# pmgbergen/porepy

Hardware: AMD Instinct MI355X
Metric: cells/sec MPFA assemble+solve, 3D unstructured grid (higher is better)
Workload: dtype f64

## Files before the change

include/porefv.h:

```cpp
#ifndef POREFV_H
#define POREFV_H

#include <stddef.h>
#include <stdint.h>

#ifdef __cplusplus
extern "C" {
#endif

typedef struct pfv_ctx pfv_ctx;

typedef enum {
  PFV_OK = 0,
  PFV_ERR_SINGULAR = 1,
  PFV_ERR_CELL_SHAPE = 2,
  PFV_ERR_HIP = 3,
  PFV_ERR_ARGUMENT = 4,
  PFV_ERR_UNSUPPORTED = 5,
  PFV_ERR_NOT_CONVERGED = 6
} pfv_status;

enum {
  PFV_MAT_FLUX = 0,
  PFV_MAT_BOUND_FLUX = 1,
  PFV_MAT_BOUND_PRESSURE_CELL = 2,
  PFV_MAT_BOUND_PRESSURE_FACE = 3,
  PFV_MAT_VECTOR_SOURCE = 4,
  PFV_MAT_BOUND_PRESSURE_VECTOR_SOURCE = 5,
  PFV_MAT_SYSTEM = 6,
  PFV_MAT_STRESS = 7,
  PFV_MAT_BOUND_STRESS = 8,
  PFV_MAT_BOUND_DISPLACEMENT_CELL = 9,
  PFV_MAT_BOUND_DISPLACEMENT_FACE = 10,
  PFV_MAT_MECH_SYSTEM = 11,
  PFV_MAT_USER_SYSTEM = 12,
  PFV_MAT_FLUX_JACOBIAN = 13,
  PFV_MAT_UPWIND = 14,
  PFV_MAT_UPWIND_RHS_DIR = 15,
  PFV_MAT_UPWIND_RHS_NEU = 16,
  PFV_MAT_TRANSPORT_SYSTEM = 17,
  PFV_MAT_ADVDIFF_SYSTEM = 18,
  PFV_NUM_MATS = 19
};

enum { PFV_BC_DIR = 1, PFV_BC_NEU = 2, PFV_BC_ROB = 4, PFV_BC_INTERNAL = 8 };

enum { PFV_SOLVE_CG = 0, PFV_SOLVE_BICGSTAB = 1, PFV_SOLVE_GMRES = 2 };

enum { PFV_PRECOND_JACOBI = 0, PFV_PRECOND_AMG = 1, PFV_PRECOND_BLOCK = 2,
       PFV_PRECOND_AMG_NNS = 3,
       PFV_PRECOND_SWEEP = 4     };

enum {
  PFV_FLUXFN_LINEAR = 0,
  PFV_FLUXFN_COREY = 1,
  PFV_FLUXFN_TABLE = 2
};

enum {
  PFV_DISCR_REBUILD_TOPOLOGY = 1,
  PFV_DISCR_SKIP_VECTOR_SOURCE = 2
};

typedef struct {
  int32_t iterations;
  int32_t converged;
  double rel_residual;
  double solve_ms;
} pfv_solve_info;

typedef struct {
  double topology_ms;
  double symbolic_ms;
  double node_ms;
  double face_ms;
  double assemble_ms;
  double solve_ms;
  double bytes_written_outputs;
  int64_t num_nodes, num_sub_half_faces, sum_block_sq, max_block;
  double amg_setup_ms;
  double amg_operator_complexity;
  int64_t amg_levels, amg_coarsest_rows;
  double discretize_ms;
  int64_t solve_renumbered;
  double node_flops;
  int64_t node_table_doubles;
  int64_t amg_maps_reused;
  int64_t amg_level0_nnz;
  double amg_filter_theta;
  int64_t win_reused;
  int64_t amg_filter_layout;
  int64_t solve_launches;
  int64_t amg_setup_launches;
  int64_t node_redo;
  int64_t symbolic_reused;
  int64_t amg_stale_rematches;
  int64_t mpsa_contrast_regions;
  double mpsa_max_contrast;
  int64_t assemble_positions_kept;
  int64_t pipeline_runs;
  int64_t amg_nns_modes;
  double face_flux_ms;
  double upwind_ms;
  double transport_assemble_ms;
  double transport_advance_ms;
  int64_t transport_iterations;
  int64_t transport_gmres_retries;
  double advdiff_assemble_ms;
  double advdiff_advance_ms;
  int64_t advdiff_iterations;
  int64_t advdiff_precond_fallbacks;
  int64_t advdiff_gmres_retries;
  int64_t sweep_levels;
  int64_t sweep_core_cells;
  int64_t sweep_launches;
  double sweep_order_ms;
  int64_t sweep_direct_steps;
  int64_t sweep_direct_fallbacks;
  int64_t transport_multi_components;
  int64_t transport_multi_direct_steps;
  int64_t transport_multi_fallback_components;
  double transport_nl_ms;
  int64_t transport_nl_steps;
  int64_t transport_nl_core_iterations;
  int64_t transport_nl_components;
  double transport_react_ms;
  int64_t transport_react_steps;
  int64_t transport_react_core_iterations;
  int64_t transport_react_components;
  double transport_adjoint_ms;
  int64_t transport_adjoint_steps;
  int64_t transport_adjoint_core_iterations;
} pfv_stats;

pfv_status pfv_create(int device, pfv_ctx** out);
void pfv_destroy(pfv_ctx* h);
const char* pfv_last_error(pfv_ctx* h);
int pfv_is_device_build(void);

pfv_status pfv_set_grid(pfv_ctx* h, int nd, int64_t nc, int64_t nf, int64_t nn,
                        const double* nodes, const int32_t* cf_indptr,
                        const int32_t* cf_indices, const int8_t* cf_sign,
                        const int32_t* fn_indptr, const int32_t* fn_indices,
                        const double* face_normals, const double* face_centers,
                        const double* cell_centers, const double* face_areas);

pfv_status pfv_mpfa_set_params(pfv_ctx* h, const double* perm_33n, const uint8_t* bc_flags,
                               const double* robin_weight, double eta,
                               const double* eta_subface);

pfv_status pfv_mpfa_set_permeability(pfv_ctx* h, const double* perm_33n);

#define PFV_AD_WANT_FLUX_JACOBIAN 1u
pfv_status pfv_mpfa_ad_flux_system(pfv_ctx* h, const double* p, const double* dk_dp, const double* bc_values,
                                   const double* vector_source, const double* source, double* flux_out,
                                   uint32_t flags);

pfv_status pfv_mpfa_set_subface_bc(pfv_ctx* h, const uint8_t* bc_flags_sub, const double* robin_weight_sub);

pfv_status pfv_mpfa_discretize(pfv_ctx* h, uint32_t flags);

pfv_status pfv_tpfa_discretize(pfv_ctx* h, int vector_source_dim);

pfv_status pfv_tpfa_transmissibility_ad(pfv_ctx* h, const double* perm_33n, double* t_face, double* dt_dk);

pfv_status pfv_mpfa_discretize_faces(pfv_ctx* h, uint32_t flags, int64_t n_faces,
                                     const int32_t* faces, int keep_other_rows);

pfv_status pfv_matrix_info(pfv_ctx* h, int which, int64_t* nrows, int64_t* ncols,
                           int64_t* nnz);
pfv_status pfv_get_matrix(pfv_ctx* h, int which, int32_t* indptr, int32_t* indices,
                          double* data);
pfv_status pfv_device_memory(pfv_ctx* h, int64_t* free_bytes, int64_t* total_bytes);
pfv_status pfv_host_alloc(size_t bytes, void** out);
void pfv_host_free(void* p);
pfv_status pfv_active_size(pfv_ctx* h, int64_t* n);
pfv_status pfv_get_matrix_rows(pfv_ctx* h, int which, int64_t n_rows, const int32_t* rows, int32_t* out_indptr,
                               int32_t* out_indices, double* out_data);

pfv_status pfv_mpfa_assemble(pfv_ctx* h, const double* bc_values, const double* vector_source,
                             const double* source);
pfv_status pfv_get_rhs(pfv_ctx* h, double* b);

pfv_status pfv_spmv(pfv_ctx* h, int which, const double* x, double* y);

enum {
  PFV_BIOT_SCALAR_GRADIENT = 0,
  PFV_BIOT_DISPLACEMENT_DIVERGENCE = 1,
  PFV_BIOT_BOUNDARY_DISPLACEMENT_DIVERGENCE = 2,
  PFV_BIOT_CONSISTENCY = 3,
  PFV_BIOT_BOUND_DISPLACEMENT_PRESSURE = 4,
  PFV_BIOT_NUM_TERMS = 5
};
pfv_status pfv_biot_set_alphas(pfv_ctx* h, int nalpha, const double* alpha_k33n);
pfv_status pfv_biot_discretize_faces(pfv_ctx* h, uint32_t flags, int64_t n_faces, const int32_t* faces,
                                     int64_t n_cells, const int32_t* cells, int keep_other_rows);

pfv_status pfv_biot_discretize(pfv_ctx* h, uint32_t flags);
pfv_status pfv_biot_matrix_info(pfv_ctx* h, int term, int64_t* nrows, int64_t* ncols, int64_t* nnz);
pfv_status pfv_biot_get_matrix(pfv_ctx* h, int term, int key, int32_t* indptr, int32_t* indices,
                               double* data);

pfv_status pfv_set_system(pfv_ctx* h, int64_t n, const int32_t* indptr, const int32_t* indices,
                          const double* data, const double* rhs);

pfv_status pfv_set_periodic(pfv_ctx* h, const int32_t* native_cell, const double* shift);

pfv_status pfv_set_vectors_on_device(pfv_ctx* h, int on);

pfv_status pfv_set_preconditioner(pfv_ctx* h, int kind);

pfv_status pfv_sweep_info(pfv_ctx* h, int64_t info[4], int32_t* level, int32_t* order);

pfv_status pfv_set_near_null_space(pfv_ctx* h, int bs, int k, const double* B);

pfv_status pfv_amg_nns_level(pfv_ctx* h, int level, int64_t* info, int32_t* agg, double* P, double* B, double* Bc,
                             int32_t* indptr, int32_t* indices, double* val);

pfv_status pfv_amg_level(pfv_ctx* h, int level, int64_t* info, double* params, int32_t* sys_indptr, int32_t* sys_indices,
                         double* sys_val, int32_t* a_indptr, int32_t* a_indices, double* a_val, int32_t* op_indptr,
                         int32_t* op_indices, double* op_val, double* dinv, int32_t* agg, int32_t* mptr, int32_t* mem,
                         double* dense);

pfv_status pfv_set_block_preconditioner(pfv_ctx* h, int64_t n_blocks, const int64_t* block_ptr, int gauss_seidel);

pfv_status pfv_solve(pfv_ctx* h, int method, double rtol, int maxit, int restart,
                     const double* x0, double* x, pfv_solve_info* info);

pfv_status pfv_mpsa_set_params(pfv_ctx* h, const double* stiffness_99n, const double* cell_volumes,
                               const uint8_t* bc_dir_bits, const uint8_t* bc_neu_bits, double eta);
pfv_status pfv_mpsa_set_subface_eta(pfv_ctx* h, const double* eta_subface);
pfv_status pfv_mpsa_set_reconstruction_eta(pfv_ctx* h, int on, double hf_eta);
pfv_status pfv_mpsa_set_reconstruction_eta_subface(pfv_ctx* h, const double* hf_eta_subface);
pfv_status pfv_mpsa_set_robin(pfv_ctx* h, const uint8_t* bc_rob_bits, const double* robin_weight_ddn);
pfv_status pfv_mpsa_set_basis(pfv_ctx* h, const double* basis_ddn);

pfv_status pfv_mpsa_set_subface_bc(pfv_ctx* h, const uint8_t* bc_dir_bits_sub, const uint8_t* bc_neu_bits_sub,
                                   const uint8_t* bc_rob_bits_sub, const double* robin_weight_dds);
pfv_status pfv_mpsa_set_subface_basis(pfv_ctx* h, const double* basis_dds);

pfv_status pfv_mpsa_discretize(pfv_ctx* h, uint32_t flags);

pfv_status pfv_mpsa_discretize_faces(pfv_ctx* h, uint32_t flags, int64_t n_faces,
                                     const int32_t* faces, int keep_other_rows);
pfv_status pfv_mpsa_assemble(pfv_ctx* h, const double* bc_values, const double* source);

pfv_status pfv_mpfa_face_flux(pfv_ctx* h, const double* p, const double* bc_values, const double* vector_source,
                              double* q_out);
pfv_status pfv_upwind_set_bc(pfv_ctx* h, const uint8_t* bc_flags);
pfv_status pfv_upwind_discretize(pfv_ctx* h, const double* q, int num_components);
pfv_status pfv_upwind_assemble(pfv_ctx* h, const double* q, const double* bc_values, const double* accumulation,
                               const double* c_old, const double* source, double* bound_rhs_out);
pfv_status pfv_transport_advance(pfv_ctx* h, int n_steps, int method, double rtol, int maxit, double* c,
                                 int32_t* steps_done, pfv_solve_info* last);
pfv_status pfv_transport_advance_multi(pfv_ctx* h, const double* q, int n_comp, const double* bc_values,
                                       const double* accumulation, const double* source, int n_steps, int method,
                                       double rtol, int maxit, double* c, int32_t* steps_done, pfv_solve_info* last);
pfv_status pfv_transport_advance_nl(pfv_ctx* h, const double* q, int fluxfn_kind, const double* fluxfn_params,
                                    int n_params, const double* bc_values, const double* accumulation,
                                    const double* source, const double* sink, int n_steps, double rtol, int maxit,
                                    double* s, int32_t* steps_done, pfv_solve_info* last);
pfv_status pfv_transport_advance_nl_multi(pfv_ctx* h, const double* q, int fluxfn_kind, const double* fluxfn_params,
                                          int n_params, const double* bc_values, const double* accumulation,
                                          const double* source, const double* sink, int k, const double* c_bc_values,
                                          const double* sorption, const double* c_source, int n_steps, double rtol,
                                          int maxit, double* s, double* c, int32_t* steps_done, pfv_solve_info* last);

pfv_status pfv_transport_advance_react(pfv_ctx* h, const double* q, int k, const double* bc_values,
                                       const double* accumulation, const double* source, const double* mobility,
                                       const double* rate, const double* rate_weight, int n_steps, double rtol,
                                       int maxit, double* c, int32_t* steps_done, pfv_solve_info* last);

pfv_status pfv_transport_adjoint_multi(pfv_ctx* h, const double* q, int n_comp, const double* bc_values,
                                       const double* accumulation, int n_steps, int64_t n_obs, const int32_t* obs_cells,
                                       const double* loads, const double* states, double rtol, int maxit,
                                       double* grad_c0, double* grad_source, double* grad_bc_values,
                                       double* grad_accumulation, double* grad_flux, int32_t* steps_done,
                                       pfv_solve_info* last);

pfv_status pfv_advdiff_assemble(pfv_ctx* h, const double* q, double flux_scale, const double* bc_values,
                                const double* accumulation, const double* c_old, const double* source,
                                double* bound_rhs_out);
pfv_status pfv_advdiff_advance(pfv_ctx* h, int n_steps, int method, double rtol, int maxit, double* c,
                               int32_t* steps_done, pfv_solve_info* last);
pfv_status pfv_advdiff_face_flux(pfv_ctx* h, const double* c, double* out);
// ... 74 lines not shown
```

porepy_amd/_lib.py:

```python
from __future__ import annotations

import ctypes as C
import os

import numpy as np

_HERE = os.path.dirname(os.path.abspath(__file__))
DEFAULT_LIBRARY = os.path.join(_HERE, "csrc", "libporefv_hip.so")

MAT_FLUX, MAT_BOUND_FLUX, MAT_BOUND_PRESSURE_CELL, MAT_BOUND_PRESSURE_FACE = 0, 1, 2, 3
MAT_VECTOR_SOURCE, MAT_BOUND_PRESSURE_VECTOR_SOURCE, MAT_SYSTEM = 4, 5, 6
MAT_STRESS, MAT_BOUND_STRESS, MAT_BOUND_DISPLACEMENT_CELL, MAT_BOUND_DISPLACEMENT_FACE, MAT_MECH_SYSTEM = 7, 8, 9, 10, 11
MAT_USER_SYSTEM = 12
MAT_FLUX_JACOBIAN = 13
MAT_UPWIND, MAT_UPWIND_RHS_DIR, MAT_UPWIND_RHS_NEU, MAT_TRANSPORT_SYSTEM = 14, 15, 16, 17
MAT_ADVDIFF_SYSTEM = 18
BC_DIR, BC_NEU, BC_ROB, BC_INTERNAL = 1, 2, 4, 8
SOLVE_CG, SOLVE_BICGSTAB, SOLVE_GMRES = 0, 1, 2
PRECOND_JACOBI, PRECOND_AMG, PRECOND_BLOCK, PRECOND_AMG_NNS, PRECOND_SWEEP = 0, 1, 2, 3, 4
FLUXFN_LINEAR, FLUXFN_COREY, FLUXFN_TABLE = 0, 1, 2
DISCR_REBUILD_TOPOLOGY, DISCR_SKIP_VECTOR_SOURCE = 1, 2

STATUS_NAMES = {
    0: "ok", 1: "singular local system", 2: "unsupported cell shape", 3: "HIP error",
    4: "bad argument", 5: "unsupported size/feature", 6: "not converged",
}

EXPORTS = [
    "pfv_create", "pfv_destroy", "pfv_last_error", "pfv_is_device_build", "pfv_set_grid",
    "pfv_mpfa_set_params", "pfv_mpfa_discretize", "pfv_matrix_info", "pfv_get_matrix",
    "pfv_mpfa_assemble", "pfv_get_rhs", "pfv_spmv", "pfv_solve", "pfv_spmv_device",
    "pfv_get_device_rhs", "pfv_sync", "pfv_get_stats", "pfv_time_kernel", "pfv_debug_copy",
    "pfv_spmv_device_rows", "pfv_copy_device_vector", "pfv_set_stream",
    "pfv_mpsa_set_params", "pfv_mpsa_discretize", "pfv_mpsa_assemble",
    "pfv_mpfa_discretize_faces", "pfv_set_system", "pfv_tpfa_discretize", "pfv_mpsa_discretize_faces", "pfv_set_preconditioner", "pfv_amg_setup", "pfv_amg_setup_sharded", "pfv_amg_apply_device", "pfv_csr_from_host", "pfv_csr_from_matrix", "pfv_csr_block_diag", "pfv_csr_matmul", "pfv_csr_axpby", "pfv_csr_transpose", "pfv_csr_bmat", "pfv_csr_scale", "pfv_csr_divide", "pfv_csr_spmv", "pfv_csr_spmv_device", "pfv_csr_info", "pfv_csr_get", "pfv_csr_set_system", "pfv_csr_free", "pfv_reset_stream", "pfv_mpsa_set_robin", "pfv_mpsa_set_basis", "pfv_mpfa_set_subface_bc", "pfv_mpsa_set_subface_bc", "pfv_mpsa_set_subface_basis",
    "pfv_biot_set_alphas", "pfv_biot_discretize", "pfv_biot_matrix_info", "pfv_biot_get_matrix",
    "pfv_set_vectors_on_device", "pfv_set_periodic", "pfv_biot_discretize_faces", "pfv_solve_sharded", "pfv_tpfa_transmissibility_ad",
    "pfv_get_matrix_rows", "pfv_active_size", "pfv_device_memory",
    "pfv_rccl_unique_id", "pfv_rccl_comm_create", "pfv_rccl_set_halo_plan", "pfv_rccl_hooks", "pfv_rccl_stats",
    "pfv_rccl_last_error", "pfv_rccl_comm_destroy", "pfv_mpfa_ad_flux_system", "pfv_host_alloc", "pfv_host_free",
    "pfv_mpsa_set_subface_eta", "pfv_mpsa_set_reconstruction_eta", "pfv_mpsa_set_reconstruction_eta_subface", "pfv_get_stats_n", "pfv_set_block_preconditioner",
    "pfv_mpfa_set_permeability", "pfv_set_near_null_space", "pfv_amg_nns_level", "pfv_amg_level",
    "pfv_mpfa_face_flux", "pfv_upwind_set_bc", "pfv_upwind_discretize", "pfv_upwind_assemble", "pfv_transport_advance",
    "pfv_advdiff_assemble", "pfv_advdiff_advance", "pfv_advdiff_face_flux", "pfv_resident_flux",
    "pfv_sweep_info", "pfv_transport_advance_multi", "pfv_transport_advance_nl", "pfv_transport_advance_nl_multi",
    "pfv_transport_advance_react", "pfv_transport_adjoint_multi",
]


class SolveInfo(C.Structure):
    _fields_ = [("iterations", C.c_int32), ("converged", C.c_int32),
                ("rel_residual", C.c_double), ("solve_ms", C.c_double)]


class Stats(C.Structure):
    _fields_ = [("topology_ms", C.c_double), ("symbolic_ms", C.c_double), ("node_ms", C.c_double),
                ("face_ms", C.c_double), ("assemble_ms", C.c_double), ("solve_ms", C.c_double),
                ("bytes_written_outputs", C.c_double), ("num_nodes", C.c_int64),
                ("num_sub_half_faces", C.c_int64), ("sum_block_sq", C.c_int64),
                ("max_block", C.c_int64), ("amg_setup_ms", C.c_double),
                ("amg_operator_complexity", C.c_double), ("amg_levels", C.c_int64),
                ("amg_coarsest_rows", C.c_int64), ("discretize_ms", C.c_double), ("solve_renumbered", C.c_int64),
                ("node_flops", C.c_double), ("node_table_doubles", C.c_int64),
                ("amg_maps_reused", C.c_int64), ("amg_level0_nnz", C.c_int64), ("amg_filter_theta", C.c_double),
                ("win_reused", C.c_int64), ("amg_filter_layout", C.c_int64),
                ("solve_launches", C.c_int64), ("amg_setup_launches", C.c_int64), ("node_redo", C.c_int64),
                ("symbolic_reused", C.c_int64), ("amg_stale_rematches", C.c_int64),
                ("mpsa_contrast_regions", C.c_int64), ("mpsa_max_contrast", C.c_double), ("assemble_positions_kept", C.c_int64),
                ("pipeline_runs", C.c_int64), ("amg_nns_modes", C.c_int64),
                ("face_flux_ms", C.c_double), ("upwind_ms", C.c_double), ("transport_assemble_ms", C.c_double),
                ("transport_advance_ms", C.c_double), ("transport_iterations", C.c_int64),
                ("transport_gmres_retries", C.c_int64),
                ("advdiff_assemble_ms", C.c_double), ("advdiff_advance_ms", C.c_double),
                ("advdiff_iterations", C.c_int64), ("advdiff_precond_fallbacks", C.c_int64),
                ("advdiff_gmres_retries", C.c_int64),
                ("sweep_levels", C.c_int64), ("sweep_core_cells", C.c_int64), ("sweep_launches", C.c_int64),
                ("sweep_order_ms", C.c_double), ("sweep_direct_steps", C.c_int64),
                ("sweep_direct_fallbacks", C.c_int64),
                ("transport_multi_components", C.c_int64), ("transport_multi_direct_steps", C.c_int64),
                ("transport_multi_fallback_components", C.c_int64),
                ("transport_nl_ms", C.c_double), ("transport_nl_steps", C.c_int64),
                ("transport_nl_core_iterations", C.c_int64), ("transport_nl_components", C.c_int64),
                ("transport_react_ms", C.c_double), ("transport_react_steps", C.c_int64),
                ("transport_react_core_iterations", C.c_int64), ("transport_react_components", C.c_int64),
                ("transport_adjoint_ms", C.c_double), ("transport_adjoint_steps", C.c_int64),
                ("transport_adjoint_core_iterations", C.c_int64)]

    def as_dict(self):
        return {n: getattr(self, n) for n, _ in self._fields_}


HALO_FN = C.CFUNCTYPE(C.c_int, C.c_void_p, C.c_void_p, C.c_void_p)
ALLREDUCE_FN = C.CFUNCTYPE(C.c_int, C.c_void_p, C.c_void_p, C.c_int, C.c_void_p)


SENDRECV_FN = C.CFUNCTYPE(C.c_int, C.c_void_p, C.c_int, C.POINTER(C.c_int32), C.c_void_p, C.POINTER(C.c_int64),
                          C.c_void_p, C.POINTER(C.c_int64), C.c_void_p)
ALLGATHER_FN = C.CFUNCTYPE(C.c_int, C.c_void_p, C.c_void_p, C.c_void_p, C.c_int64, C.c_void_p)


class ShardHooks(C.Structure):
    _fields_ = [("exchange_halo", HALO_FN), ("allreduce_sum", ALLREDUCE_FN), ("user", C.c_void_p),
                ("sendrecv", SENDRECV_FN), ("allgather", ALLGATHER_FN)]


class PorefvError(RuntimeError):
    def __init__(self, status: int, message: str):
        super().__init__(f"porefv status {status} ({STATUS_NAMES.get(status, '?')}): {message}")
        self.status = status
        self.message = message


_dp = C.POINTER(C.c_double)
_ip = C.POINTER(C.c_int32)
_bp = C.POINTER(C.c_int8)
_up = C.POINTER(C.c_uint8)
_lp = C.POINTER(C.c_int64)
_h = C.c_void_p


def _bind(lib: C.CDLL) -> C.CDLL:
    lib.pfv_create.argtypes = [C.c_int, C.POINTER(_h)]
    lib.pfv_create.restype = C.c_int
    lib.pfv_destroy.argtypes = [_h]
    lib.pfv_destroy.restype = None
    lib.pfv_last_error.argtypes = [_h]
    lib.pfv_last_error.restype = C.c_char_p
    lib.pfv_is_device_build.argtypes = []
    lib.pfv_is_device_build.restype = C.c_int
    lib.pfv_set_grid.argtypes = [_h, C.c_int, C.c_int64, C.c_int64, C.c_int64, _dp, _ip, _ip, _bp,
                                 _ip, _ip, _dp, _dp, _dp, _dp]
    lib.pfv_set_grid.restype = C.c_int
    lib.pfv_mpfa_set_params.argtypes = [_h, _dp, _up, _dp, C.c_double, _dp]
    lib.pfv_mpfa_set_params.restype = C.c_int
    lib.pfv_mpfa_set_permeability.argtypes = [_h, _dp]
    lib.pfv_mpfa_set_permeability.restype = C.c_int
    lib.pfv_mpfa_discretize.argtypes = [_h, C.c_uint32]
    lib.pfv_mpfa_discretize.restype = C.c_int
    lib.pfv_mpfa_discretize_faces.argtypes = [_h, C.c_uint32, C.c_int64, _ip, C.c_int]
    lib.pfv_mpfa_discretize_faces.restype = C.c_int
    lib.pfv_mpsa_discretize_faces.argtypes = [_h, C.c_uint32, C.c_int64, _ip, C.c_int]
    lib.pfv_mpsa_discretize_faces.restype = C.c_int
    lib.pfv_biot_set_alphas.argtypes = [_h, C.c_int, _dp]
    lib.pfv_biot_set_alphas.restype = C.c_int
    lib.pfv_biot_discretize.argtypes = [_h, C.c_uint32]
    lib.pfv_biot_discretize.restype = C.c_int
    lib.pfv_biot_matrix_info.argtypes = [_h, C.c_int, _lp, _lp, _lp]
    lib.pfv_biot_matrix_info.restype = C.c_int
    lib.pfv_biot_get_matrix.argtypes = [_h, C.c_int, C.c_int, _ip, _ip, _dp]
    lib.pfv_biot_get_matrix.restype = C.c_int
    lib.pfv_mpfa_set_subface_bc.argtypes = [_h, _up, _dp]
    lib.pfv_mpfa_set_subface_bc.restype = C.c_int
    lib.pfv_mpsa_set_basis.argtypes = [_h, _dp]
    lib.pfv_mpsa_set_basis.restype = C.c_int
    lib.pfv_mpsa_set_subface_bc.argtypes = [_h, _up, _up, _up, _dp]
    lib.pfv_mpsa_set_subface_bc.restype = C.c_int
    lib.pfv_mpsa_set_subface_basis.argtypes = [_h, _dp]
    lib.pfv_mpsa_set_subface_basis.restype = C.c_int
    lib.pfv_mpsa_set_robin.argtypes = [_h, _up, _dp]
    lib.pfv_mpsa_set_robin.restype = C.c_int
    lib.pfv_mpsa_set_subface_eta.argtypes = [_h, _dp]
    lib.pfv_mpsa_set_subface_eta.restype = C.c_int
    lib.pfv_mpsa_set_reconstruction_eta.argtypes = [_h, C.c_int, C.c_double]
    lib.pfv_mpsa_set_reconstruction_eta.restype = C.c_int
    lib.pfv_mpsa_set_reconstruction_eta_subface.argtypes = [_h, _dp]
    lib.pfv_mpsa_set_reconstruction_eta_subface.restype = C.c_int
    lib.pfv_reset_stream.argtypes = [_h]
    lib.pfv_reset_stream.restype = C.c_int
    lib.pfv_amg_setup.argtypes = [_h, C.c_int64]
    lib.pfv_amg_setup.restype = C.c_int
    lib.pfv_amg_setup_sharded.argtypes = [_h, C.c_int64, C.POINTER(ShardHooks), C.c_int, C.c_int, C.c_int, _ip, _lp, _ip,
                                          _lp, _ip]
    lib.pfv_amg_setup_sharded.restype = C.c_int
    lib.pfv_csr_from_host.argtypes = [_h, C.c_int64, C.c_int64, _ip, _ip, _dp, C.POINTER(_h)]
    lib.pfv_csr_from_matrix.argtypes = [_h, _h, C.c_int, C.POINTER(_h)]
    lib.pfv_csr_block_diag.argtypes = [_h, C.c_int, C.POINTER(_h), C.POINTER(_h)]
    lib.pfv_csr_matmul.argtypes = [_h, _h, _h, C.POINTER(_h)]
    lib.pfv_csr_axpby.argtypes = [_h, C.c_double, _h, C.c_double, _h, C.POINTER(_h)]
    lib.pfv_csr_transpose.argtypes = [_h, _h, C.POINTER(_h)]
    lib.pfv_csr_bmat.argtypes = [_h, C.c_int, C.c_int, C.POINTER(_h), _lp, _lp, C.POINTER(_h)]
    lib.pfv_csr_scale.argtypes = [_h, _dp, _dp]
    lib.pfv_csr_divide.argtypes = [_h, C.c_double]
    lib.pfv_csr_divide.restype = C.c_int
    lib.pfv_csr_spmv.argtypes = [_h, _dp, _dp]
    lib.pfv_csr_spmv_device.argtypes = [_h, C.c_void_p, C.c_void_p]
    lib.pfv_csr_info.argtypes = [_h, _lp, _lp, _lp]
    lib.pfv_csr_get.argtypes = [_h, _ip, _ip, _dp]
    lib.pfv_csr_set_system.argtypes = [_h, _h, C.c_void_p, C.c_int]
    for name in ("from_host", "from_matrix", "block_diag", "matmul", "axpby", "transpose", "bmat", "scale", "spmv", "spmv_device", "info", "get",
                 "set_system"):
        getattr(lib, "pfv_csr_" + name).restype = C.c_int
    lib.pfv_csr_free.argtypes = [_h]
    lib.pfv_csr_free.restype = None
    lib.pfv_amg_apply_device.argtypes = [_h, C.c_void_p, C.c_void_p]
    lib.pfv_amg_apply_device.restype = C.c_int
    lib.pfv_biot_discretize_faces.argtypes = [_h, C.c_uint32, C.c_int64, _ip, C.c_int64, _ip, C.c_int]
    lib.pfv_biot_discretize_faces.restype = C.c_int
    lib.pfv_set_periodic.argtypes = [_h, C.POINTER(C.c_int32), _dp]
    lib.pfv_set_periodic.restype = C.c_int
    lib.pfv_set_vectors_on_device.argtypes = [_h, C.c_int]
    lib.pfv_set_vectors_on_device.restype = C.c_int
    lib.pfv_set_preconditioner.argtypes = [_h, C.c_int]
    lib.pfv_set_preconditioner.restype = C.c_int
    lib.pfv_tpfa_discretize.argtypes = [_h, C.c_int]
    lib.pfv_tpfa_discretize.restype = C.c_int
    lib.pfv_set_system.argtypes = [_h, C.c_int64, _ip, _ip, _dp, _dp]
    lib.pfv_set_system.restype = C.c_int
    lib.pfv_matrix_info.argtypes = [_h, C.c_int, _lp, _lp, _lp]
    lib.pfv_matrix_info.restype = C.c_int
    lib.pfv_get_matrix.argtypes = [_h, C.c_int, _ip, _ip, _dp]
    lib.pfv_get_matrix.restype = C.c_int
    lib.pfv_mpfa_assemble.argtypes = [_h, _dp, _dp, _dp]
    lib.pfv_mpfa_assemble.restype = C.c_int
    lib.pfv_get_rhs.argtypes = [_h, _dp]
    lib.pfv_get_rhs.restype = C.c_int
    lib.pfv_spmv.argtypes = [_h, C.c_int, _dp, _dp]
    lib.pfv_spmv.restype = C.c_int
    lib.pfv_solve.argtypes = [_h, C.c_int, C.c_double, C.c_int, C.c_int, _dp, _dp, C.POINTER(SolveInfo)]
    lib.pfv_solve.restype = C.c_int
    lib.pfv_spmv_device.argtypes = [_h, C.c_int, C.c_void_p, C.c_void_p]
    lib.pfv_spmv_device.restype = C.c_int
    lib.pfv_get_device_rhs.argtypes = [_h, C.POINTER(C.c_void_p), C.POINTER(C.c_void_p)]
    lib.pfv_get_device_rhs.restype = C.c_int
    lib.pfv_sync.argtypes = [_h]
    lib.pfv_sync.restype = C.c_int
    lib.pfv_get_stats.argtypes = [_h, C.POINTER(Stats)]
    lib.pfv_get_stats.restype = C.c_int
    lib.pfv_set_block_preconditioner.argtypes = [_h, C.c_int64, C.POINTER(C.c_int64), C.c_int]
    lib.pfv_set_block_preconditioner.restype = C.c_int
    lib.pfv_set_near_null_space.argtypes = [_h, C.c_int, C.c_int, _dp]
    lib.pfv_set_near_null_space.restype = C.c_int
    lib.pfv_amg_nns_level.argtypes = [_h, C.c_int, _lp, _ip, _dp, _dp, _dp, _ip, _ip, _dp]
    lib.pfv_amg_nns_level.restype = C.c_int
    lib.pfv_amg_level.argtypes = [_h, C.c_int, _lp, _dp, _ip, _ip, _dp, _ip, _ip, _dp, _ip, _ip, _dp, _dp, _ip, _ip, _ip,
                                  _dp]
    lib.pfv_amg_level.restype = C.c_int
    lib.pfv_get_stats_n.argtypes = [_h, C.c_void_p, C.c_size_t]
    lib.pfv_get_stats_n.restype = C.c_int
    lib.pfv_time_kernel.argtypes = [_h, C.c_int, C.c_int, _dp]
# ... 1343 lines not shown
```

porepy_amd/csrc/amg.inc:

```

namespace pfv {

constexpr int kAmgDenseMax = 1024;
constexpr int kAmgCoarseTargetDefault = 160;
constexpr int kAmgMaxLevels = 14;
constexpr int64_t kAmgWTopRows = 600000;
constexpr int kAmgFilterPermilBlock = 50;
constexpr int kAmgFilterPermil = 30;
constexpr int kAmgRounds = 4;
constexpr int kAmgPasses = 3;
constexpr int kAmgGentleCells = 400000;
constexpr int kGalEpl = 8;
constexpr int kGalMaxMembers = 16;
constexpr int64_t kAmgGatherRowsDefault = 32768;

struct AmgSwitches {
  int bs = 1;
  bool omega_auto = false;
  bool safe_rows = true;
  double omega = 0.95, alpha = 1.5;
  int omega_power_steps = 10;
  double omega_sigma = 1.8;
  int passes = kAmgPasses;
  bool passes_coarse_set = false;
  int passes_coarse_raw = -1;
  int rounds = kAmgRounds, rounds_raw = kAmgRounds;
  int strength_neg = 0;
  bool fp32 = true;
  double filter_theta = 0.0;
  int coarse_target = kAmgCoarseTargetDefault;
  bool gamma_set = false;
  int gamma_raw = 0;
  int gamma_levels = 1;
  int64_t fuse_rows = 30000;
  bool fuse_cycle = true;
  bool restrict_lanes = true;
  bool reuse = true, reuse_dist = true, reuse_rebuilt = true;
  int reuse_dist_min_rows = 500000;
  bool members_reuse = true, sizes_reuse = true;
  bool filter_smooth = true, rowmax_reuse = true, filter_layout_reuse = true, skip_moved_digest = true;
  bool galerkin_batched = true, filter_unroll = true, dense_lds = true;
  int64_t gather_rows = kAmgGatherRowsDefault;
};

static AmgSwitches amg_read_switches(int bs) {
  auto given = [](const char* name, int& v) {
    const char* e = std::getenv(name);
    if (e) v = std::atoi(e);
    return e != nullptr;
  };
  auto on = [](const char* name, int dflt) { return env_int(name, dflt) != 0; };
  AmgSwitches w;
  w.bs = bs;
  w.safe_rows = on("PFV_AMG_SAFE_ROWS", bs == 1 ? 1 : 0);
  int omega_pct = w.safe_rows ? 95 : 80;
  w.omega_auto = !given("PFV_AMG_OMEGA_PCT", omega_pct) && on("PFV_AMG_OMEGA_AUTO", 0);
  w.omega = 0.01 * omega_pct;
  w.alpha = 0.01 * env_int("PFV_AMG_ALPHA_PCT", 150);
  w.omega_power_steps = std::max(2, std::min(30, env_int("PFV_AMG_OMEGA_POWER_STEPS", 10)));
  w.omega_sigma = 0.01 * env_int("PFV_AMG_OMEGA_RHO_PCT", 180);
  w.passes = std::max(1, std::min(6, env_int("PFV_AMG_PASSES", kAmgPasses)));
  w.passes_coarse_set = given("PFV_AMG_PASSES_COARSE", w.passes_coarse_raw);
  w.rounds_raw = env_int("PFV_AMG_ROUNDS", kAmgRounds);
  w.rounds = std::max(1, std::min(12, w.rounds_raw));
  w.strength_neg = env_int("PFV_AMG_STRENGTH_NEG", 0);
  w.fp32 = on("PFV_AMG_FP32", 1);
  w.filter_theta = 0.001 * env_int(bs == 1 ? "PFV_AMG_FILTER_PERMIL" : "PFV_AMG_FILTER_PERMIL_BLOCK",
                                   bs == 1 ? kAmgFilterPermil : kAmgFilterPermilBlock);
  w.coarse_target = std::max(1, std::min(kAmgDenseMax, env_int("PFV_AMG_COARSE_TARGET", kAmgCoarseTargetDefault)));
  w.gamma_set = given("PFV_AMG_GAMMA", w.gamma_raw);
  w.gamma_levels = env_int("PFV_AMG_GAMMA_LEVELS", 1);
  w.fuse_rows = env_int("PFV_AMG_FUSE_ROWS", 30000);
  w.fuse_cycle = on("PFV_AMG_FUSE_CYCLE", 1);
  w.restrict_lanes = on("PFV_AMG_RESTRICT_LANES", bs == 1 ? 1 : 0);
  w.reuse = on("PFV_AMG_REUSE", 1);
  w.reuse_dist = on("PFV_AMG_REUSE_DIST", 1);
  w.reuse_rebuilt = on("PFV_AMG_REUSE_REBUILT", 1);
  w.reuse_dist_min_rows = env_int("PFV_AMG_REUSE_DIST_MIN_ROWS", 500000);
  w.members_reuse = on("PFV_AMG_MEMBERS_REUSE", 1);
  w.sizes_reuse = on("PFV_AMG_SIZES_REUSE", 1);
  w.filter_smooth = on("PFV_AMG_FILTER_SMOOTH", 1);
  w.rowmax_reuse = on("PFV_AMG_ROWMAX_REUSE", 1);
  w.filter_layout_reuse = on("PFV_AMG_FILTER_LAYOUT_REUSE", 1);
  w.skip_moved_digest = on("PFV_AMG_SKIP_MOVED_DIGEST", 1);
  w.galerkin_batched = on("PFV_AMG_GALERKIN_BATCHED", 1);
  w.filter_unroll = on("PFV_AMG_FILTER_UNROLL", 1);
  w.dense_lds = on("PFV_AMG_DENSE_LDS", 1);
  w.gather_rows = std::max<int64_t>(1, env_int("PFV_AMG_GATHER_ROWS", (int)kAmgGatherRowsDefault));
  return w;
}

static int64_t amg_maps_cfg(const AmgSwitches& w) {
  return ((((int64_t)w.passes * 16 + w.rounds_raw) * 16 + w.passes_coarse_raw + 1) * 4 + w.strength_neg) * 65536 +
         w.coarse_target * 8 + w.bs + (int64_t)(1000.0 * w.filter_theta + 0.5) * (int64_t(1) << 40);
}
static int amg_maps_tag(const AmgSwitches& w) { return w.rounds_raw * 64 + w.passes_coarse_raw + 1; }

struct AmgLevel {
  int64_t n = 0;
  int64_t m = 0;
  const CsrPattern* P = nullptr;
  const double* val = nullptr;
  CsrPattern P_own;
  Buf<double> val_own;
  Buf<float> val32;
  const float* v32 = nullptr;
  WinCsr win_own;
  const WinCsr* win = nullptr;
  Buf<double> dinv;
  Buf<int32_t> agg;
  Buf<int32_t> mptr, mem;
  int64_t nc_cells = 0;
  Buf<int32_t> pmap[6];
  int64_t pmap_n[6] = {0, 0, 0, 0, 0, 0};
  int pmap_count = 0;
  Buf<int32_t> pmp[6], pme[6];
  bool members_kept = false;
  Buf<double> x, b, t;
  Buf<double> r2, x2;
  Buf<double> u;
  double omega = 0.8;
  double rho = 0.0;
};

struct AmgWork {
  Buf<int32_t> match, pick, join, lead, a1, mp, me, cap, cnt, tcol, vin;
  Buf<uint32_t> kin, kout;
  Buf<int64_t> pos, tptr, cptr;
  Buf<double> tval, dense_work;
  Buf<int32_t> piv;
  Buf<unsigned long long> csum;
  CsrPattern P[2];
  Buf<double> V[2], D[2];
};

struct AmgPlan {
  int n_peers = 0;
  std::vector<int32_t> peers;
  std::vector<int64_t> send_ptr, recv_ptr;
  std::vector<int32_t> h_send_idx, h_recv_pos;
  Buf<int32_t> send_idx, recv_pos;
  int64_t n_send = 0, n_recv = 0;
  int64_t n_own = 0, n_halo = 0;
  std::vector<int32_t> halo_peer, halo_owner_id;
};
struct Amg;
struct AmgDist {
  ~AmgDist() {
    rows0.indptr.p = nullptr;
    rows0.indices.p = nullptr;
  }
  CsrPattern rows0;
  pfv_shard_hooks hooks{};
  int rank = 0, world = 1;
  std::vector<std::unique_ptr<AmgPlan>> plan;
  size_t kgather = 0;
  Buf<double> sbuf, rbuf, gid;
  Buf<int32_t> aext, itmp, chalo;
  std::unique_ptr<Amg> glob;
  std::vector<int64_t> gn, goff;
  int64_t gN = 0, gnmax = 0;
  Buf<int64_t> gn_d, goff_d, cnt_s, cnt_r;
  Buf<double> gsend, grecv, gb, gx, gV, gval_s, gval_r;
  Buf<int32_t> glen_s, glen_r, gcol_s, gcol_r, hal_gcell;
  CsrPattern gT, gP;
  Buf<double> gTV, gD;
  Buf<int32_t> gagg, gmp, gme;
  int64_t exchanges = 0, allgathers = 0;
  int64_t global_rows0 = 0, global_rows_level = 0;
};

struct Amg {
  Amg();
  ~Amg();
  std::unique_ptr<AmgDist> dist;
  bool no_filter = false;
  int64_t finest_cells_parent = 0;
  std::vector<std::unique_ptr<AmgLevel>> lev;
  size_t nlev = 0;
  AmgWork wk;
  int bs = 1;
  AmgSwitches sw;
  int passes = kAmgPasses;
  double omega = 0.8, alpha = 1.5;
  bool omega_auto = true;
  Buf<double> pw_a, pw_b, pw_zero, pw_part;
  Buf<double> dense;
  unsigned long long filt_layout_for = 0;
  bool filt_layout_stable = false;
  CsrPattern filtP;
  Buf<double> filtV;
  double filter_theta = 0.0;
  int64_t filt_nnz = 0;
  bool filter_level0 = false;
  WinCsr filt_win;
  struct GalSizes { int64_t ncr, annz, nnz; int maxcap; };
  std::vector<GalSizes> gal_sizes;
  unsigned long long gal_for_sum = 0;
  bool gal_use = false;
  size_t gal_k = 0;
  unsigned long long filt_win_sum = 0;
  bool maps_ok = false, reused = false;
  int64_t maps_n = -1, maps_nnz = -1, maps_cfg = 0;
  unsigned long long maps_sum = 0, maps_epoch = 0;
  int maps_tag = 0;
  int iters_fresh = -1;
  int method_fresh = -1;
  double rtol_fresh = 0.0;
  int64_t stale_rematches = 0;
  void note_iterations(int iterations, double rtol, int method, bool converged) {
    if (!valid) return;
    if (!reused) {
      iters_fresh = converged ? iterations : -1;
      rtol_fresh = rtol;
      method_fresh = method;
    } else if (iters_fresh > 0 && rtol == rtol_fresh && method == method_fresh &&
               (!converged || (double)iterations > 1.3 * (double)iters_fresh + 1.0)) {
      maps_ok = false;
      ++stale_rematches;
    }
  }
  bool dense_ok = false;
  bool restrict_lanes = true;
  bool valid = false;
  int gamma = 2, gamma_levels = 1;
  int coarse_target = 0;
  int64_t fuse_rows = 0;
  bool fuse_cycle = true;
  bool fp32 = true;
  double setup_ms = 0.0, op_complexity = 0.0;
  const CsrPattern* sysP = nullptr;
  const double* sysV = nullptr;
};

struct AmgPath {
  bool small = false;
  bool twice = false;
  bool fuse_up = false;
  bool fuse_big = false;
  bool second = false;
};
static AmgPath amg_level_path(const Amg& amg, size_t l) {
  AmgPath p;
  if (l + 1 >= amg.nlev) return p;
  const AmgLevel& L = *amg.lev[l];
  p.small = L.n <= amg.fuse_rows && !(L.win && L.win->ok);
  p.twice = amg.gamma == 2 && l >= 1 && (int)l <= amg.gamma_levels;
  p.fuse_up = p.small && l >= 1 && !p.twice;
  p.fuse_big = amg.fuse_cycle && !p.small && l >= 1;
  p.second = amg.gamma == 2 && (int)l < amg.gamma_levels && l + 2 < amg.nlev;
  return p;
}

inline Amg::Amg() = default;
inline Amg::~Amg() = default;
static bool amg_gal_cached(Amg* amg, int64_t ncr, int64_t annz, int* maxcap, int64_t* nnz) {
  if (!amg || !amg->gal_use || amg->gal_k >= amg->gal_sizes.size()) return false;
  const Amg::GalSizes& g = amg->gal_sizes[amg->gal_k];
  if (g.ncr != ncr || g.annz != annz) {
    amg->gal_use = false;
    amg->gal_sizes.resize(amg->gal_k);
    return false;
  }
  *maxcap = g.maxcap;
  *nnz = g.nnz;
  ++amg->gal_k;
  return true;
}
static void amg_gal_record(Amg* amg, int64_t ncr, int64_t annz, int maxcap, int64_t nnz) {
  if (!amg) return;
  if (amg->gal_k < amg->gal_sizes.size()) amg->gal_sizes.resize(amg->gal_k);
  amg->gal_sizes.push_back(Amg::GalSizes{ncr, annz, nnz, maxcap});
  amg->gal_k = amg->gal_sizes.size();
}

struct AmgGraph {
  const int32_t* ip;
  const int32_t* ix;
  const double* val;
  int bs;
  int neg_only;
  PFV_HD int nblk(int64_t i) const { return (ip[i * bs + 1] - ip[i * bs]) / bs; }
  PFV_HD int col(int64_t i, int k) const { return ix[ip[i * bs] + k * bs] / bs; }
  PFV_HD double w(int64_t i, int k) const {
    double s = 0.0;
    for (int a = 0; a < bs; ++a) {
      const double v = val[ip[i * bs + a] + k * bs + a];
      s += neg_only ? (v < 0.0 ? -v : 0.0) : fabs(v);
    }
    return s;
  }
};

PFV_HD inline uint32_t amg_edge_hash(int64_t i, int64_t j) {
  uint64_t a = (uint64_t)(i < j ? i : j), b = (uint64_t)(i < j ? j : i);
  uint64_t z = a * 0x9E3779B97F4A7C15ull + b + 0x7F4A7C15ull;
  z = (z ^ (z >> 30)) * 0xBF58476D1CE4E5B9ull;
  z = (z ^ (z >> 27)) * 0x94D049BB133111EBull;
  return (uint32_t)(z >> 32);
}

static void amg_pick_pass(pfv_ctx_impl& c, const AmgGraph g, int64_t nb, const int32_t* match, int want_matched,
                          int32_t* out) {
  stream_t s = c.stream;
  const size_t lds_pick = 16 * (8 + 4 + 4) + 16;
  wave_for<16>(s, nb, lds_pick, PFV_LAMBDA(const WaveCtx& w) {
    const int64_t i = w.item;
    if (match[i] >= 0) {
      if (w.lane0()) out[i] = -1;
      return;
    }
    double* cw = reinterpret_cast<double*>(w.lds);
    uint32_t* ch = reinterpret_cast<uint32_t*>(cw + 16);
    int32_t* cj = reinterpret_cast<int32_t*>(ch + 16);
    double bw = 0.0;
    uint32_t bh = 0;
    int best = -1;
    const int m = g.nblk(i);
    PFV_LANES(k, m) {
      const int j = g.col(i, k);
      const bool eligible = (j != i) && j < nb && ((match[j] >= 0) == (want_matched != 0));
      if (eligible) {
        const double wt = g.w(i, k);
        if (wt > 0.0 && !(wt < bw)) {
          const uint32_t h = amg_edge_hash(i, j);
          if (wt > bw || h > bh) { bw = wt; bh = h; best = j; }
        }
      }
    }
    cw[w.lane] = bw;
    ch[w.lane] = bh;
    cj[w.lane] = best;
    w.sync();
    if (w.lane0()) {
      for (int l = 1; l < w.width; ++l) {
        if (cj[l] >= 0 && (cw[l] > bw || (cw[l] == bw && ch[l] > bh))) { bw = cw[l]; bh = ch[l]; best = cj[l]; }
      }
      out[i] = best;
    }
    w.sync();
  });
}

static int64_t amg_pairwise(pfv_ctx_impl& c, const AmgSwitches& sw, AmgWork& wk, const CsrPattern& P, const double* val,
                            int bs, Buf<int32_t>& agg_out) {
  stream_t s = c.stream;
  const int64_t nb = P.nrows / bs;
  AmgGraph g{P.indptr, P.indices, val, bs, sw.strength_neg};
  int32_t* match = wk.match.ensure(nb);
  int32_t* pick = wk.pick.ensure(nb);
  int32_t* join = wk.join.ensure(nb);
  int32_t* lead = wk.lead.ensure(nb + 1);
  int64_t* pos = wk.pos.ensure(nb + 1);
  parallel_for(s, nb, PFV_LAMBDA(int64_t i) { match[i] = -1; });
  for (int round = 0; round < sw.rounds; ++round) {
    amg_pick_pass(c, g, nb, match, 0, pick);
    parallel_for(s, nb, PFV_LAMBDA(int64_t i) {
      const int p = pick[i];
      if (p >= 0 && pick[p] == (int32_t)i) match[i] = p;
    });
  }
  amg_pick_pass(c, g, nb, match, 1, join);
  parallel_for(s, nb, PFV_LAMBDA(int64_t i) {
    lead[i] = (match[i] >= 0) ? ((int32_t)i < match[i] ? 1 : 0) : (join[i] < 0 ? 1 : 0);
  });
  exclusive_scan<int32_t, int64_t>(s, c.scratch, lead, pos, (size_t)nb);
  const int64_t nagg = read_scalar<int64_t>(s, pos + nb);
  int32_t* agg = agg_out.ensure(nb);
  parallel_for(s, nb, PFV_LAMBDA(int64_t i) {
    int l;
    if (match[i] >= 0) l = (int32_t)i < match[i] ? (int32_t)i : match[i];
    else if (join[i] >= 0) l = join[i] < match[join[i]] ? join[i] : match[join[i]];
    else l = (int32_t)i;
    agg[i] = (int32_t)pos[l];
  });
  return nagg;
}

static void amg_members(pfv_ctx_impl& c, AmgWork& wk, const int32_t* agg, int64_t nb, int64_t nagg,
                        Buf<int32_t>& mptr_, Buf<int32_t>& mem_) {
  stream_t s = c.stream;
  uint32_t* k = wk.kin.ensure(nb);
  uint32_t* ko = wk.kout.ensure(nb);
  int32_t* v = wk.vin.ensure(nb);
  int32_t* mem = mem_.ensure(nb);
  int32_t* mptr = mptr_.ensure(nagg + 1);
  parallel_for(s, nb, PFV_LAMBDA(int64_t i) {
    k[i] = (uint32_t)agg[i];
    v[i] = (int32_t)i;
  });
  int bits = 1;
  while ((int64_t(1) << bits) < nagg) ++bits;
  sort_pairs(s, c.scratch, k, ko, v, mem, (size_t)nb, bits);
  parallel_for(s, nagg + 1, PFV_LAMBDA(int64_t I) {
    mptr[I] = (int32_t)lower_bound_idx<uint32_t>(ko, (int)nb, (uint32_t)I);
  });
}

struct Amg;
static bool amg_gal_cached(Amg* amg, int64_t ncr, int64_t annz, int* maxcap, int64_t* nnz);
static void amg_gal_record(Amg* amg, int64_t ncr, int64_t annz, int maxcap, int64_t nnz);
static void amg_galerkin(pfv_ctx_impl& c, const AmgSwitches& sw, AmgWork& wk, const CsrPattern& A, const double* val,
                         int bs, const int32_t* agg, const int32_t* mptr, const int32_t* mem, int64_t nagg, CsrPattern& Ac,
                         Buf<double>& valc, Buf<double>& dinvc, Amg* sizes = nullptr) {
  stream_t s = c.stream;
  const int64_t ncr = nagg * bs;
  const int32_t* ip = A.indptr;
  const int32_t* ix = A.indices;
  int32_t* cap = wk.cap.ensure(ncr + 1);
  int32_t* cnt = wk.cnt.ensure(ncr + 1);
  int64_t* tptr = wk.tptr.ensure(ncr + 1);
  int64_t* cptr = wk.cptr.ensure(ncr + 1);
  int32_t* st = c.status.ensure(16);
  be_memset(st + 8, 0, sizeof(int32_t) * 2, s);
  parallel_for(s, ncr, PFV_LAMBDA(int64_t R) {
    const int64_t I = R / bs;
    const int a = (int)(R - I * bs);
    int m = 0;
    for (int q = mptr[I]; q < mptr[I + 1]; ++q) {
      const int64_t r = (int64_t)mem[q] * bs + a;
      m += ip[r + 1] - ip[r];
    }
    cap[R] = m;
    track_max_i32(st + 8, m);
  });
  exclusive_scan<int32_t, int64_t>(s, c.scratch, cap, tptr, (size_t)ncr);
  int maxcap_c = 0;
  int64_t nnz_c = 0;
  const bool known = amg_gal_cached(sizes, ncr, A.nnz, &maxcap_c, &nnz_c);
  const int maxcap = known ? maxcap_c : read_scalar<int32_t>(s, st + 8);
  const int64_t ttot = A.nnz;
  if (maxcap > 4096) throw Error(PFV_ERR_UNSUPPORTED, "AMG: more than 4096 entries feed one coarse row");
  int32_t* tcol = wk.tcol.ensure(std::max<int64_t>(ttot, 1));
  double* tval = wk.tval.ensure(std::max<int64_t>(ttot, 1));
  double* dinv = dinvc.ensure(std::max<int64_t>(ncr, 1));
  be_memset(dinv, 0, sizeof(double) * (size_t)ncr, s);
  const int capL = std::max(maxcap, 1);
  const int G = capL <= 64 ? 16 : (capL <= 160 ? 32 : 64);
  int capP = 2;
  while (capP < capL) capP <<= 1;
  const int nw = capP / 64 + 1;
  const size_t lds = 8 * (size_t)capP + 8 * (size_t)capL + 8 * (size_t)nw + 4 * (2 * kGalMaxMembers + 1) + 64;
  const bool batched = capL <= kGalEpl * G && sw.galerkin_batched;
  wave_for_g(G, s, ncr, lds, PFV_LAMBDA(const WaveCtx& w) {
    const int64_t R = w.item;
    const int64_t I = R / bs;
    const int a = (int)(R - I * bs);
    unsigned long long* key = reinterpret_cast<unsigned long long*>(w.lds);
    double* v0 = reinterpret_cast<double*>(key + capP);
    unsigned long long* mask = reinterpret_cast<unsigned long long*>(v0 + capL);
    int m = 0;
    const int q0 = mptr[I], nm = mptr[I + 1] - q0;
    if (batched && nm <= kGalMaxMembers && cap[R] <= kGalEpl * w.width) {
      int32_t* mp0 = reinterpret_cast<int32_t*>(mask + nw);
      int32_t* mof = mp0 + kGalMaxMembers;
      PFV_LANES(q, nm) {
        const int64_t r = (int64_t)mem[q0 + q] * bs + a;
        mp0[q] = ip[r];
        mof[q + 1] = ip[r + 1] - ip[r];
      }
      w.sync();
      if (w.lane0()) {
        mof[0] = 0;
        for (int q = 0; q < nm; ++q) mof[q + 1] += mof[q];
      }
      w.sync();
      m = mof[nm];
      int cidx[kGalEpl];
      double vv[kGalEpl];
#pragma unroll
      for (int k = 0; k < kGalEpl; ++k) {
        const int e = w.lane + k * w.width;
        cidx[k] = -1;
        vv[k] = 0.0;
        if (e < m) {
          int q = 0;
          while (q + 1 < nm && e >= mof[q + 1]) ++q;
          const int src = mp0[q] + (e - mof[q]);
          cidx[k] = ix[src];
          vv[k] = val[src];
        }
      }
      int kcs[kGalEpl];
#pragma unroll
      for (int k = 0; k < kGalEpl; ++k) {
        kcs[k] = 0;
        if (cidx[k] >= 0) {
          const int cj = cidx[k] / bs;
          kcs[k] = agg[cj] * bs + (cidx[k] - cj * bs);
        }
      }
#pragma unroll
      for (int k = 0; k < kGalEpl; ++k) {
        const int e = w.lane + k * w.width;
        if (cidx[k] >= 0) {
          key[e] = ((unsigned long long)(unsigned)kcs[k] << 32) | (unsigned)e;
          v0[e] = vv[k];
        }
      }
    } else {
      for (int q = q0; q < q0 + nm; ++q) {
        const int64_t r = (int64_t)mem[q] * bs + a;
        const int p0 = ip[r], len = ip[r + 1] - p0;
        PFV_LANES(t, len) {
          const int cidx = ix[p0 + t];
          const int cj = cidx / bs;
          const unsigned long long kc = (unsigned long long)(unsigned)(agg[cj] * bs + (cidx - cj * bs));
          key[m + t] = (kc << 32) | (unsigned)(m + t);
          v0[m + t] = val[p0 + t];
        }
        m += len;
      }
    }
    int P2 = 2;
    while (P2 < m) P2 <<= 1;
    PFV_LANES(t, P2 - m) key[m + t] = ~0ull;
    PFV_LANES(i, P2 / 64 + 1) mask[i] = 0ull;
    w.sync();
    for (int k = 2; k <= P2; k <<= 1) {
      for (int j = k >> 1; j > 0; j >>= 1) {
        PFV_LANES(t, P2 >> 1) {
          const int lo = ((t & ~(j - 1)) << 1) | (t & (j - 1));
          const int hi = lo | j;
          const bool up = (lo & k) == 0;
          const unsigned long long x = key[lo], y = key[hi];
          if ((x > y) == up) {
            key[lo] = y;
            key[hi] = x;
          }
        }
        w.sync();
      }
    }
    PFV_LANES(e, m) {
      if (e == 0 || (key[e] >> 32) != (key[e - 1] >> 32)) atomic_or_u64(mask + (e >> 6), 1ull << (e & 63));
    }
    w.sync();
    int total = 0;
    for (int i = 0; i < m / 64 + 1; ++i) total += popcount64(mask[i]);
    const int64_t t0 = tptr[R];
    PFV_LANES(e, m) {
      const unsigned long long word = mask[e >> 6];
      if ((word >> (e & 63)) & 1ull) {
        int posn = popcount64(word & ((1ull << (e & 63)) - 1ull));
        for (int i = 0; i < (e >> 6); ++i) posn += popcount64(mask[i]);
        const unsigned long long kc = key[e] >> 32;
        double sum = v0[(unsigned)key[e]];
        for (int t = e + 1; t < m && (key[t] >> 32) == kc; ++t) sum += v0[(unsigned)key[t]];
        tcol[t0 + posn] = (int32_t)kc;
        tval[t0 + posn] = sum;
        if ((int64_t)kc == R) dinv[R] = sum != 0.0 ? 1.0 / sum : 0.0;
      }
    }
    if (w.lane0()) cnt[R] = total;
    w.sync();
  });
  exclusive_scan<int32_t, int64_t>(s, c.scratch, cnt, cptr, (size_t)ncr);
  const int64_t nnz = known ? nnz_c : read_scalar<int64_t>(s, cptr + ncr);
  if (!known) amg_gal_record(sizes, ncr, A.nnz, maxcap, nnz);
  if (nnz >= (int64_t(1) << 31)) throw Error(PFV_ERR_UNSUPPORTED, "AMG: coarse matrix with more than 2^31 entries");
  Ac.nrows = Ac.ncols = ncr;
  Ac.nnz = nnz;
  int32_t* cp = Ac.indptr.ensure(ncr + 1);
  int32_t* cx = Ac.indices.ensure(std::max<int64_t>(nnz, 1));
  double* cv = valc.ensure(std::max<int64_t>(nnz, 1));
  parallel_for(s, ncr + 1, PFV_LAMBDA(int64_t R) { cp[R] = (int32_t)cptr[R]; });
  wave_for<16>(s, ncr, 16, PFV_LAMBDA(const WaveCtx& w) {
    const int64_t R = w.item;
    const int64_t t0 = tptr[R], o = cptr[R];
    PFV_LANES(t, cnt[R]) {
      cx[o + t] = tcol[t0 + t];
      cv[o + t] = tval[t0 + t];
    }
  });
  Ac.max_row = maxcap;
}

static void amg_diag_inverse(pfv_ctx_impl& c, const CsrPattern& P, const double* val, double* dinv) {
  const int32_t* ip = P.indptr;
  const int32_t* ix = P.indices;
  parallel_for(c.stream, P.nrows, PFV_LAMBDA(int64_t r) {
    double d = 0.0;
    for (int e = ip[r]; e < ip[r + 1]; ++e)
      if (ix[e] == r) d += val[e];
    dinv[r] = d != 0.0 ? 1.0 / d : 0.0;
  });
}

static void amg_swap_pattern(CsrPattern& a, CsrPattern& b) {
  std::swap(a.nrows, b.nrows);
  std::swap(a.ncols, b.ncols);
  std::swap(a.nnz, b.nnz);
  std::swap(a.max_row, b.max_row);
  a.indptr.swap(b.indptr);
  a.indices.swap(b.indices);
}

static unsigned long long amg_pattern_checksum(pfv_ctx_impl& c, AmgWork& wk, const CsrPattern& P) {
  if (&P == &c.pat_A && c.pat_A_checksum != 0 && c.have_symbolic) return c.pat_A_checksum;
  return read_scalar<unsigned long long>(c.stream, launch_pattern_checksum(c, wk.csum, P));
}

struct AmgBlockStrength {
  const int32_t* ip;
  const double* val;
  int bs;
  PFV_HD double operator()(int64_t r, int kb) const {
    const int64_t i = r / bs;
    double sw = 0.0;
    for (int a = 0; a < bs; ++a) sw += fabs(val[ip[i * bs + a] + kb * bs + a]);
    return sw;
  }
};

#ifndef PFV_EMULATE
constexpr int kFilterUnroll = 5;

static void amg_filter_count_scalar(stream_t s, int64_t n, const int32_t* ip, const int32_t* ix, const double* val,
                                    const double* rmax, double theta, int32_t* cnt) {
  wave_for<16>(s, n, 16, PFV_LAMBDA(const WaveCtx& w) {
    const int64_t r = w.item;
    const int p0 = ip[r], nb = ip[r + 1] - p0;
    const double mi = rmax[r];
    int kept = 0;
    for (int c0 = 0; c0 < nb; c0 += kFilterUnroll * 16) {
      int cj[kFilterUnroll];
      double v[kFilterUnroll], rm[kFilterUnroll];
#pragma unroll
      for (int u = 0; u < kFilterUnroll; ++u) {
        const int kb = c0 + u * 16 + w.lane;
        const bool live = kb < nb;
        cj[u] = live ? ix[p0 + kb] : -1;
        v[u] = live ? val[p0 + kb] : 0.0;
      }
#pragma unroll
      for (int u = 0; u < kFilterUnroll; ++u) rm[u] = cj[u] >= 0 ? rmax[cj[u]] : 0.0;
#pragma unroll
      for (int u = 0; u < kFilterUnroll; ++u)
        if (cj[u] >= 0 && (cj[u] == (int32_t)r || fabs(v[u]) >= theta * fmin(mi, rm[u]))) ++kept;
    }
    kept += __shfl_xor(kept, 8, 16);
    kept += __shfl_xor(kept, 4, 16);
    kept += __shfl_xor(kept, 2, 16);
    kept += __shfl_xor(kept, 1, 16);
    if (w.lane0()) cnt[r] = kept;
  });
}

static void amg_filter_compact_scalar(stream_t s, int64_t n, const int32_t* ip, const int32_t* ix, const double* val,
                                      const double* rmax, double theta, const int32_t* fp, int32_t* fx, double* fv,
                                      double* dinv_out, bool spec, int32_t* bad) {
  wave_for<16>(s, n, 16 * sizeof(double) + 16, PFV_LAMBDA(const WaveCtx& w) {
    const int64_t r = w.item;
    double* lump = reinterpret_cast<double*>(w.lds);
    const int p0 = ip[r], nb = ip[r + 1] - p0;
    const double mi = rmax[r];
    double mylump = 0.0;
    int base = fp[r];
    const int room = fp[r + 1];
    int od = -1;
    double dv = 0.0;
    const int sh = (int)threadIdx.x & 48;
    for (int c0 = 0; c0 < nb; c0 += kFilterUnroll * 16) {
      int cj[kFilterUnroll];
      double v[kFilterUnroll], rm[kFilterUnroll];
#pragma unroll
      for (int u = 0; u < kFilterUnroll; ++u) {
        const int kb = c0 + u * 16 + w.lane;
        const bool live = kb < nb;
        cj[u] = live ? ix[p0 + kb] : -1;
        v[u] = live ? val[p0 + kb] : 0.0;
      }
#pragma unroll
      for (int u = 0; u < kFilterUnroll; ++u) rm[u] = cj[u] >= 0 ? rmax[cj[u]] : 0.0;
#pragma unroll
      for (int u = 0; u < kFilterUnroll; ++u) {
        if (c0 + u * 16 >= nb) break;
        const bool live = cj[u] >= 0;
        const bool isdiag = cj[u] == (int32_t)r;
        bool keep = live && (isdiag || fabs(v[u]) >= theta * fmin(mi, rm[u]));
        if (live && !keep) mylump += v[u];
        const unsigned long long m = __ballot(keep);
        const unsigned m16 = (unsigned)((m >> sh) & 0xffffu);
        const int before = __popc(m16 & ((1u << w.lane) - 1u));
        const int total = __popc(m16);
        if (keep && spec && base + before + 1 > room) {
          atomic_max_i32(bad, 1);
          keep = false;
        }
        if (keep) {
          const int o = base + before;
          fx[o] = cj[u];
          fv[o] = v[u];
          if (isdiag) { od = o; dv = v[u]; }
        }
        base += total;
      }
    }
    lump[w.lane] = mylump;
    w.lsync();
    if (spec && w.lane0() && base != room) atomic_max_i32(bad, 1);
    const unsigned long long has = __ballot(od >= 0);
    const bool any_diag = ((has >> sh) & 0xffffull) != 0ull;
    if (od >= 0) {
      double sum = 0.0;
      for (int l = 0; l < 16; ++l) sum += lump[l];
      const double d = dv + sum;
      fv[od] = d;
      if (dinv_out) dinv_out[r] = d != 0.0 ? 1.0 / d : 0.0;
    } else if (!any_diag && w.lane0() && dinv_out) {
      dinv_out[r] = 0.0;
    }
    w.lsync();
  });
}
#endif

static void amg_filter(pfv_ctx_impl& c, const AmgSwitches& sw, const CsrPattern& A, const double* val, double theta,
                       CsrPattern& F, Buf<double>& FV, AmgWork& wk, int bs = 1,
// ... 41 lines not shown
#endif
  if (!spec) {
#ifndef PFV_EMULATE
  if (fast) amg_filter_count_scalar(s, n, ip, ix, val, rmax, theta, cnt);
  else
#endif
  wave_for<16>(s, n, 16 * sizeof(int32_t) + 16, PFV_LAMBDA(const WaveCtx& w) {
    const int64_t r = w.item;
    const int64_t i = r / bs;
    int32_t* ct = reinterpret_cast<int32_t*>(w.lds);
    const int p0 = ip[r], nb = (ip[r + 1] - p0) / bs;
    const double mi = rmax[r];
    int kept = 0;
    PFV_LANES(kb, nb) {
      const int cj = ix[p0 + kb * bs] / bs;
      if (cj == (int32_t)i || strength(r, kb) >= theta * fmin(mi, rmax[(int64_t)cj * bs])) ++kept;
    }
#ifndef PFV_EMULATE
    (void)ct;
    kept += __shfl_xor(kept, 8, 16);
    kept += __shfl_xor(kept, 4, 16);
    kept += __shfl_xor(kept, 2, 16);
    kept += __shfl_xor(kept, 1, 16);
    if (w.lane0()) cnt[r] = kept * bs;
#else
    ct[w.lane] = kept;
    w.lsync();
    if (w.lane0()) {
      int tot = 0;
      for (int l = 0; l < w.width; ++l) tot += ct[l];
      cnt[r] = tot * bs;
    }
    w.lsync();
#endif
  });
  exclusive_scan<int32_t, int64_t>(s, c.scratch, cnt, pos, (size_t)n);
  }
  const bool compare = !spec && layout_unchanged != nullptr && F.nrows == n && F.nnz > 0 && F.indptr.p != nullptr;
  if (!spec) {
    be_memset(pos + n + 1, 0, sizeof(int64_t), s);
    if (compare) {
      const int32_t* old = F.indptr.p;
      parallel_for(s, n, PFV_LAMBDA(int64_t r) {
        if (old[r + 1] - old[r] != cnt[r]) pos[n + 1] = 1;
      });
    }
  }
  int64_t tail[2] = {F.nnz, 0};
  if (!spec) be_d2h(tail, pos + n, 2 * sizeof(int64_t), s);
  if (layout_unchanged) *layout_unchanged = spec || (compare && tail[1] == 0 && tail[0] == F.nnz);
  const int64_t nnz = tail[0];
  F.nrows = n;
  F.ncols = A.ncols;
  F.nnz = nnz;
  F.max_row = A.max_row;
  int32_t* fp = F.indptr.ensure(n + 1);
  int32_t* fx = F.indices.ensure(std::max<int64_t>(nnz, 1));
  double* fv = FV.ensure(std::max<int64_t>(nnz, 1));
  if (!spec) parallel_for(s, n + 1, PFV_LAMBDA(int64_t q) { fp[q] = (int32_t)pos[q]; });
#ifndef PFV_EMULATE
  if (fast) amg_filter_compact_scalar(s, n, ip, ix, val, rmax, theta, fp, fx, fv, dinv_out, spec, bad);
  else
#endif
  wave_for<16>(s, n, (16 + 1) * kMaxBs * sizeof(double) + 20 * sizeof(int32_t) + 16, PFV_LAMBDA(const WaveCtx& w) {
    const int64_t r = w.item;
    const int64_t i = r / bs;
    double* lump = reinterpret_cast<double*>(w.lds);
    double* dblk = lump + 16 * kMaxBs;
    int32_t* flag = reinterpret_cast<int32_t*>(dblk + kMaxBs);
    const int p0 = ip[r], nb = (ip[r + 1] - p0) / bs;
    const double mi = rmax[r];
    if (w.lane0()) flag[16] = -1;
    w.lsync();
    double mylump[kMaxBs];
    for (int b = 0; b < kMaxBs; ++b) mylump[b] = 0.0;
    int base = fp[r];
    for (int c0 = 0; c0 < nb; c0 += w.width) {
      const int kb = c0 + w.lane;
      bool keep = false;
      const bool live = kb < nb;
      bool isdiag = false;
      if (live) {
        const int cj = ix[p0 + kb * bs] / bs;
        isdiag = cj == (int32_t)i;
        keep = isdiag || strength(r, kb) >= theta * fmin(mi, rmax[(int64_t)cj * bs]);
        if (!keep)
          for (int b = 0; b < bs; ++b) mylump[b] += val[p0 + kb * bs + b];
      }
      int before = 0, total = 0;
#ifndef PFV_EMULATE
      {
        const unsigned long long m = __ballot(keep);
        const unsigned m16 = (unsigned)((m >> (((int)threadIdx.x & 48))) & 0xffffu);
        before = __popc(m16 & ((1u << w.lane) - 1u));
        total = __popc(m16);
      }
#else
      flag[w.lane] = keep ? 1 : 0;
      w.lsync();
      for (int l = 0; l < w.width; ++l) {
        const int fl = flag[l];
        if (l < w.lane) before += fl;
        total += fl;
      }
#endif
      if (keep && spec && base + (before + 1) * bs > fp[r + 1]) {
        atomic_max_i32(bad, 1);
        keep = false;
      }
      if (keep) {
        const int o = base + before * bs;
        for (int b = 0; b < bs; ++b) {
          fx[o + b] = ix[p0 + kb * bs + b];
          fv[o + b] = val[p0 + kb * bs + b];
        }
        if (isdiag) {
          flag[16] = o;
          for (int b = 0; b < bs; ++b) dblk[b] = val[p0 + kb * bs + b];
        }
      }
      base += total * bs;
      w.lsync();
    }
    for (int b = 0; b < bs; ++b) lump[w.lane * kMaxBs + b] = mylump[b];
    w.lsync();
    if (spec && w.lane0() && base != fp[r + 1]) atomic_max_i32(bad, 1);
    if (w.lane0()) {
      const int od = flag[16];
      if (od >= 0) {
        for (int b = 0; b < bs; ++b) {
          double sum = 0.0;
          for (int l = 0; l < w.width; ++l) sum += lump[l * kMaxBs + b];
          const double dv = dblk[b] + sum;
          fv[od + b] = dv;
          if (dinv_out && b == (int)(r - i * bs)) dinv_out[r] = dv != 0.0 ? 1.0 / dv : 0.0;
        }
      } else if (dinv_out) {
        dinv_out[r] = 0.0;
      }
    }
    w.lsync();
  });
  c.stats.amg_filter_layout = spec ? 1 : 0;
  if (spec && read_scalar<int32_t>(s, bad) != 0) {
    amg_filter(c, sw, A, val, theta, F, FV, wk, bs, fill_halo, rmax_given, dinv_out, false, nullptr);
    c.stats.amg_filter_layout = 2;
    if (layout_unchanged) *layout_unchanged = false;
  }
}

static void amg_estimate_omegas(pfv_ctx_impl& c, Amg& amg);
static void amg_spmv(pfv_ctx_impl& c, const Amg& amg, const AmgLevel& L, const double* x, double* y,
                     const double* smooth_b);
static double* amg_cycle(pfv_ctx_impl& c, Amg& amg, size_t l, const double* b, double* x, bool x_is_presmoothed = false,
                         int visit = 0);
static void amg_setup(pfv_ctx_impl& c, Amg& amg, const CsrPattern& A, const double* val, int bs,
                      const double* diag = nullptr, const WinCsr* win0 = nullptr);
static void amg_restrict(pfv_ctx_impl& c, const Amg& amg, const AmgLevel& L, const AmgLevel& Ln, const double* b,
                         const double* t, bool next_smooths);

static void amg_safeguard_rows(pfv_ctx_impl& c, const CsrPattern& P, const double* val, double* dinv) {
  const int32_t* ip = P.indptr;
  const int32_t* ix = P.indices;
  wave_for<16>(c.stream, P.nrows, 16 * sizeof(double) + 16, PFV_LAMBDA(const WaveCtx& w) {
    const int64_t r = w.item;
    double* sh = reinterpret_cast<double*>(w.lds);
    const int p0 = ip[r], len = ip[r + 1] - p0;
    double off = 0.0;
    PFV_LANES(k, len) {
      if (ix[p0 + k] != (int32_t)r) off += fabs(val[p0 + k]);
    }
    sh[w.lane] = off;
    w.lsync();
    if (w.lane0()) {
      double sum = 0.0;
      for (int l = 0; l < w.width; ++l) sum += sh[l];
      const double di = dinv[r];
      const double ri = sum * fabs(di);
      if (ri > 1.0 && ri < 1.0e300) dinv[r] = di * 2.0 / (1.0 + ri);
    }
    w.lsync();
  });
}

#include "amg_dist.inc"

static bool amg_dense_invert(pfv_ctx_impl& c, const AmgSwitches& sw, AmgWork& wk, const CsrPattern& P, const double* v,
                             Buf<double>& dense) {
  stream_t s = c.stream;
  const int n = (int)P.nrows, ld = n | 1;
  double* D = wk.dense_work.ensure((size_t)n * ld + 3 * (size_t)n);
  double* rsc = D + (size_t)n * ld + 2 * (size_t)n;
  int32_t* ipiv = wk.piv.ensure(n + 4);
  const int32_t* ip = P.indptr;
  const int32_t* ix = P.indices;
  be_memset(D, 0, sizeof(double) * ((size_t)n * ld + 3 * (size_t)n), s);
  parallel_for(s, n, PFV_LAMBDA(int64_t r) {
    double sum = 0.0;
    for (int e = ip[r]; e < ip[r + 1]; ++e) sum += fabs(v[e]);
    const double sc = (sum > 0.0 && sum < 1.0e300) ? 1.0 / sum : 1.0;
    rsc[r] = sc;
    for (int e = ip[r]; e < ip[r + 1]; ++e) D[(size_t)r * ld + ix[e]] += v[e] * sc;
  });
  int32_t* st = c.status.ensure(16);
  be_memset(st, 0, sizeof(int32_t), s);
  auto invert = PFV_LAMBDA(const WaveCtx& w) {
    NodeLds G;
    G.A = D;
    G.rowk = D + (size_t)n * ld;
    G.colk = G.rowk + n;
    G.ipiv = ipiv;
    node_gj_lds(w, G, n, ld, 0, st);
  };
  const size_t lds_need = sizeof(double) * ((size_t)n * ld + 2 * (size_t)n) + 64;
  auto invert_lds = PFV_LAMBDA(const WaveCtx& w) {
    double* A = reinterpret_cast<double*>(w.lds);
    PFV_LANES(q, n * ld) A[q] = D[q];
    w.sync();
    NodeLds G;
    G.A = A;
    G.rowk = A + (size_t)n * ld;
    G.colk = G.rowk + n;
    G.ipiv = ipiv;
    node_gj_lds(w, G, n, ld, 0, st);
    w.sync();
    PFV_LANES(q, n * ld) D[q] = A[q];
    w.sync();
  };
  if (lds_need <= 150 * 1024 && sw.dense_lds) {
    if (n > 128) block_for<1024>(s, 1, lds_need, invert_lds);
    else block_for<256>(s, 1, lds_need, invert_lds);
  } else if (n > 128) block_for<1024>(s, 1, 0, invert);
  else block_for<256>(s, 1, 0, invert);
  if (read_scalar<int32_t>(s, st) == 0) {
    double* inv = dense.ensure((size_t)n * n);
    parallel_for(s, (int64_t)n * n, PFV_LAMBDA(int64_t q) {
      const int64_t r = q / n, cc = q - r * n;
      inv[q] = D[(size_t)r * ld + cc] * rsc[cc];
    });
    return true;
  }
  return false;
}

static void amg_dense_apply(pfv_ctx_impl& c, const double* inv, int64_t n, const double* b, double* x) {
  wave_for(c.stream, n, 64 * sizeof(double) + 16, PFV_LAMBDA(const WaveCtx& w) {
    double* sh = reinterpret_cast<double*>(w.lds);
    const int64_t r = w.item;
    double a = 0.0;
    PFV_LANES(j, (int)n) a += inv[r * n + j] * b[j];
    sh[w.lane] = a;
    w.sync();
    if (w.lane0()) {
      double sum = 0.0;
      for (int j = 0; j < w.width; ++j) sum += sh[j];
      x[r] = sum;
    }
    w.sync();
  });
}


static AmgLevel& amg_level(Amg& amg, size_t l) {
  while (amg.lev.size() <= l) amg.lev.push_back(std::make_unique<AmgLevel>());
  return *amg.lev[l];
}

static bool amg_decide_reuse(pfv_ctx_impl& c, Amg& amg, const CsrPattern& A, unsigned long long& csum) {
  const AmgSwitches& w = amg.sw;
  AmgDist* D = amg.dist.get();
  csum = 0;
  bool mine = false;
  if (w.reuse && (!D || w.reuse_dist)) {
    csum = amg_pattern_checksum(c, amg.wk, A);
    mine = amg.maps_ok && amg.maps_n == A.nrows && amg.maps_nnz == A.nnz && amg.maps_cfg == amg_maps_cfg(w) &&
           amg.maps_sum == csum &&
           (amg.maps_epoch == c.symbolic_epoch || w.reuse_rebuilt) &&
           (!D || (A.nrows >= w.reuse_dist_min_rows && amg.maps_tag == amg_maps_tag(w)));
  }
  return D ? amg_dist_vote(c, *D, A.nrows, mine) : mine;
}

static void amg_check_full_blocks(pfv_ctx_impl& c, const CsrPattern& A, int bs) {
  stream_t s = c.stream;
  const int32_t* ip = A.indptr;
  int32_t* st = c.status.ensure(16);
  be_memset(st + 10, 0, sizeof(int32_t), s);
  parallel_for(s, A.nrows / bs, PFV_LAMBDA(int64_t i) {
    const int len = ip[i * bs + 1] - ip[i * bs];
    bool bad = (len % bs) != 0;
    for (int a = 1; a < bs; ++a) bad = bad || (ip[i * bs + a + 1] - ip[i * bs + a]) != len;
    if (bad) atomic_max_i32(st + 10, 1);
  });
  if (read_scalar<int32_t>(s, st + 10))
    throw Error(PFV_ERR_UNSUPPORTED, "AMG: the matrix is not made of full blocks of the given block size");
}

static unsigned long long amg_setup_level0(pfv_ctx_impl& c, Amg& amg, const CsrPattern& A, const double* val,
                                           const double* diag, const WinCsr* win0, unsigned long long csum) {
  stream_t s = c.stream;
  const AmgSwitches& w = amg.sw;
  AmgDist* D = amg.dist.get();
  const int bs = amg.bs;
  AmgLevel& L0 = amg_level(amg, 0);
  L0.n = A.nrows;
  L0.m = std::max(A.ncols, A.nrows);
  L0.P = &A;
  L0.val = val;
  L0.win = win0;
  amg.filt_nnz = 0;
  amg.filter_level0 = amg.filter_theta > 0.0 && w.filter_smooth;
  if (!amg.filter_level0) {
    double* dv = L0.dinv.ensure(L0.n);
    if (diag) {
      parallel_for(s, L0.n, PFV_LAMBDA(int64_t i) { dv[i] = diag[i] != 0.0 ? 1.0 / diag[i] : 0.0; });
    } else {
      amg_diag_inverse(c, A, val, dv);
    }
    return csum;
  }
  const double* rmax_given = (c.sys_rowmax_for == val && A.nrows == c.nc && w.rowmax_reuse) ? c.sys_rowmax.p : nullptr;
  const bool same_pattern = !D && csum != 0 && amg.filt_layout_for == csum;
  const bool same_layout = same_pattern && amg.filt_layout_stable && w.filter_layout_reuse;
  if (!same_pattern) amg.filtP.nrows = 0;
  bool unchanged = false;
  amg_filter(c, w, A, val, amg.filter_theta, amg.filtP, amg.filtV, amg.wk, bs, amg_fill_halo0(c, D, bs), rmax_given,
             L0.dinv.ensure(L0.n), same_layout, &unchanged);
  amg.filt_layout_stable = unchanged;
  amg.filt_layout_for = D ? 0ull : csum;
  amg.filt_nnz = amg.filtP.nnz;
  L0.P = &amg.filtP;
  L0.val = amg.filtV.p;
  L0.win = nullptr;
  if (amg.filtP.nnz < 200000) return 0ull;
  const bool moved = same_pattern && !unchanged && w.skip_moved_digest;
  const unsigned long long fsum = (env_int("PFV_WIN_REUSE", 1) != 0 && !moved)
                                      ? read_scalar<unsigned long long>(s, launch_pattern_checksum(c, amg.wk.csum, amg.filtP))
                                      : 0ull;
  const bool keep = fsum != 0 && amg.filt_win.ok && amg.filt_win_sum == fsum && amg.filt_win.nrows == amg.filtP.nrows &&
                    amg.filt_win.nnz == amg.filtP.nnz && env_int("PFV_SPMV_WINDOW", 1) != 0;
  if (!keep) {
    if (!(win0 && win_derive(c, amg.filtP, *win0, amg.filt_win))) win_build(c, amg.filtP, amg.filt_win);
    amg.filt_win_sum = amg.filt_win.ok ? fsum : 0ull;
  }
  L0.win = &amg.filt_win;
  return fsum;
}

static void amg_level_buffers(pfv_ctx_impl& c, const Amg& amg, AmgLevel& L, size_t l) {
  if (l > 0) {
    L.x.ensure(L.m);
    L.b.ensure(L.n);
  }
  L.t.ensure(L.m);
  L.v32 = nullptr;
  if (amg.fp32) {
    float* v32 = L.val32.ensure(L.P->nnz);
    const double* v64 = L.val;
    parallel_for(c.stream, L.P->nnz, PFV_LAMBDA(int64_t e) { v32[e] = (float)v64[e]; });
    L.v32 = v32;
  }
  L.nc_cells = 0;
}

static int amg_coarsen_level(pfv_ctx_impl& c, Amg& amg, size_t l, bool reuse) {
  stream_t s = c.stream;
  const AmgSwitches& w = amg.sw;
  AmgWork& wk = amg.wk;
  AmgDist* D = amg.dist.get();
  const int bs = amg.bs;
  AmgLevel& L = *amg.lev[l];
  const int64_t cells = L.n / bs;
  const CsrPattern* curP = L.P;
  const double* curV = L.val;
  if (l == 0 && amg.filter_theta > 0.0 && !amg.filter_level0) {
    amg_filter(c, w, *L.P, L.val, amg.filter_theta, amg.filtP, amg.filtV, wk, bs, amg_fill_halo0(c, D, bs));
    amg.filt_nnz = amg.filtP.nnz;
    curP = &amg.filtP;
    curV = amg.filtV.p;
  }
  int32_t* aggL = L.agg.ensure(cells);
  int64_t cur_cells = cells;
  int slot = -1;
  const int64_t finest_cells = amg.finest_cells_parent > 0 ? amg.finest_cells_parent
                                                            : (D ? D->global_rows0 : amg.lev[0]->n) / bs;
  const int coarse_default = finest_cells >= kAmgGentleCells ? std::min(2, amg.passes) : amg.passes;
  const int passes_here = (l == 0 && amg.finest_cells_parent <= 0)
                              ? amg.passes
                              : std::max(1, std::min(6, w.passes_coarse_set ? w.passes_coarse_raw : coarse_default));
  if (!reuse) L.pmap_count = 0;
  if (!reuse) L.members_kept = false;
  const bool members_reuse = reuse && L.members_kept && w.members_reuse;
  for (int pass = 0; pass < (reuse ? L.pmap_count : passes_here); ++pass) {
    int64_t nagg;
    if (reuse) {
      nagg = L.pmap_n[pass];
    } else {
      nagg = amg_pairwise(c, w, wk, *curP, curV, bs, wk.a1);
      if (nagg >= cur_cells) break;
      be_d2d(L.pmap[pass].ensure(cur_cells), wk.a1.p, sizeof(int32_t) * (size_t)cur_cells, s);
      L.pmap_n[pass] = nagg;
      L.pmap_count = pass + 1;
    }
    const int32_t* a1p = L.pmap[pass].p;
    if (!members_reuse) amg_members(c, wk, a1p, cur_cells, nagg, L.pmp[pass], L.pme[pass]);
    const int nslot = slot < 0 ? 0 : 1 - slot;
    const int32_t* amap = D ? amg_dist_extend_map(c, *D, l, a1p, cur_cells, nagg) : a1p;
    amg_galerkin(c, w, wk, *curP, curV, bs, amap, L.pmp[pass], L.pme[pass], nagg, wk.P[nslot], wk.V[nslot], wk.D[nslot],
                 D ? nullptr : &amg);
    if (D) wk.P[nslot].ncols = (nagg + D->plan[l]->n_halo) * bs;
    if (members_reuse) {
    } else if (slot < 0) {
      parallel_for(s, cells, PFV_LAMBDA(int64_t i) { aggL[i] = a1p[i]; });
    } else {
      parallel_for(s, cells, PFV_LAMBDA(int64_t i) { aggL[i] = a1p[aggL[i]]; });
    }
    slot = nslot;
    curP = &wk.P[slot];
    curV = wk.V[slot].p;
    cur_cells = nagg;
    if (nagg * bs <= w.coarse_target) break;
  }
  if (D && slot < 0) {
    amg_dist_identity_level(c, amg, *D, l, *curP, curV, aggL, cells);
    slot = 0;
  }
  if (!D && (slot < 0 || cur_cells > 0.85 * cells)) return -1;
  L.nc_cells = cur_cells;
  if (!(members_reuse && L.pmap_count > 0)) amg_members(c, wk, aggL, cells, cur_cells, L.mptr, L.mem);
  L.members_kept = L.pmap_count > 0;
  return slot;
}

static void amg_setup_finish(pfv_ctx_impl& c, Amg& amg, const CsrPattern& A, double nnz_sum, unsigned long long csum,
                             unsigned long long level0_sum) {
  const AmgSwitches& w = amg.sw;
  AmgDist* D = amg.dist.get();
  AmgLevel& Lc = *amg.lev[amg.nlev - 1];
  if (D) {
    amg_build_global(c, amg, *D, Lc, *D->plan[amg.nlev - 1]);
  } else if (Lc.n <= kAmgDenseMax) {
    amg.dense_ok = amg_dense_invert(c, w, amg.wk, *Lc.P, Lc.val, amg.dense);
  }
  amg.op_complexity = nnz_sum / (double)A.nnz;
  for (size_t k = 0; k < amg.nlev; ++k) {
    amg.lev[k]->omega = amg.omega;
    amg.lev[k]->rho = 0.0;
  }
  if (w.safe_rows) {
    for (size_t k = 0; k < amg.nlev; ++k) {
      AmgLevel& Lk = *amg.lev[k];
      if (k + 1 < amg.nlev || !amg.dense_ok) amg_safeguard_rows(c, *Lk.P, Lk.val, Lk.dinv);
    }
  }
  if (amg.omega_auto && !D) amg_estimate_omegas(c, amg);
  amg.valid = true;
  if (env_int("PFV_DEBUG_AMG", 0)) {
    std::fprintf(stderr, "amg_setup: filter theta %.3f (nnz %lld -> %lld), levels:", amg.filter_theta, (long long)A.nnz,
                 (long long)amg.filt_nnz);
    for (size_t k = 0; k < amg.nlev; ++k)
      std::fprintf(stderr, " %lld/%lld(w%.3f)", (long long)amg.lev[k]->n, (long long)amg.lev[k]->P->nnz, amg.lev[k]->omega);
    std::fprintf(stderr, " reuse %d\n", (int)amg.reused);
  }
  amg.gal_for_sum = D ? 0ull : level0_sum;
  if (w.reuse && (!D || csum != 0)) {
    amg.maps_ok = true;
    amg.maps_n = A.nrows;
    amg.maps_nnz = A.nnz;
    amg.maps_cfg = amg_maps_cfg(w);
    amg.maps_sum = csum;
    amg.maps_epoch = c.symbolic_epoch;
    amg.maps_tag = amg_maps_tag(w);
  }
}

static void amg_setup(pfv_ctx_impl& c, Amg& amg, const CsrPattern& A, const double* val, int bs,
                      const double* diag, const WinCsr* win0) {
  stream_t s = c.stream;
  Timer tm;
  tm.start(s);
  AmgDist* D = amg.dist.get();
  amg.bs = bs;
  amg.valid = amg.dense_ok = false;
  amg.sysP = &A;
  amg.sysV = val;
  if (A.nrows % bs) throw Error(PFV_ERR_ARGUMENT, "AMG: system size is not a multiple of the block size");
  AmgSwitches& w = amg.sw = amg_read_switches(bs);
  if (amg.no_filter) w.filter_theta = 0.0;
  if (amg.coarse_target > 0) w.coarse_target = std::min(kAmgDenseMax, amg.coarse_target);
  amg.omega_auto = w.omega_auto;
  amg.omega = w.omega;
  amg.alpha = w.alpha;
  amg.passes = w.passes;
  amg.fp32 = w.fp32;
  amg.filter_theta = w.filter_theta;
  amg.gamma_levels = w.gamma_levels;
  amg.fuse_rows = w.fuse_rows;
  amg.fuse_cycle = w.fuse_cycle;
  amg.restrict_lanes = w.restrict_lanes;
  unsigned long long csum = 0;
  const bool reuse = amg_decide_reuse(c, amg, A, csum);
  const int64_t rows_for_shape = D ? D->global_rows0 / D->world : A.nrows;
  amg.gamma = std::max(1, std::min(2, w.gamma_set ? w.gamma_raw : (rows_for_shape >= kAmgWTopRows ? 2 : 1)));
  amg.maps_ok = false;
  amg.reused = reuse;
  if (bs > 1) amg_check_full_blocks(c, A, bs);
  unsigned long long level0_sum = amg_setup_level0(c, amg, A, val, diag, win0, csum);
  amg.gal_use = reuse && !D && level0_sum != 0 && amg.gal_for_sum == level0_sum && w.sizes_reuse;
  amg.gal_k = 0;
  if (!amg.gal_use) amg.gal_sizes.clear();
  double nnz_sum = 0.0;
  size_t l = 0;
  while (true) {
    AmgLevel& L = amg_level(amg, l);
    nnz_sum += (double)L.P->nnz;
    amg_level_buffers(c, amg, L, l);
    if (D ? (l >= 1 && l == D->kgather) : (L.n <= w.coarse_target || (int)l + 1 >= kAmgMaxLevels)) break;
    const int slot = amg_coarsen_level(c, amg, l, reuse);
    if (slot < 0) break;
    AmgLevel& Ln = amg_level(amg, l + 1);
    Ln.n = L.nc_cells * bs;
    amg_swap_pattern(Ln.P_own, amg.wk.P[slot]);
    Ln.val_own.swap(amg.wk.V[slot]);
    Ln.dinv.swap(amg.wk.D[slot]);
    Ln.P = &Ln.P_own;
    Ln.val = Ln.val_own.p;
    Ln.win = nullptr;
    Ln.m = Ln.n;
    if (D) {
      amg_dist_rename_halo(c, *D, l, L.agg, L.nc_cells, bs, Ln);
      amg_dist_decide_gather(c, *D, l, Ln.n, w.gather_rows);
    }
    if (Ln.n > w.coarse_target && Ln.P_own.nnz >= 200000) {
      win_build(c, Ln.P_own, Ln.win_own);
      Ln.win = &Ln.win_own;
    }
    ++l;
  }
  amg.nlev = l + 1;
  amg_setup_finish(c, amg, A, nnz_sum, csum, level0_sum);
  amg.setup_ms = tm.stop(s);
}


#ifndef PFV_EMULATE
template <int L, int U, class VT, int MODE>
__global__ void __launch_bounds__(256) k_amg_spmv(int64_t nrows, const int32_t* __restrict__ indptr,
                                                  const int32_t* __restrict__ indices,
                                                  const VT* __restrict__ val, const double* __restrict__ x,
                                                  double* __restrict__ y, const double* __restrict__ b,
                                                  const double* __restrict__ dinv, double omega, const SpmvFuse F) {
  const int lane = threadIdx.x % L;
  const int64_t row = (int64_t)blockIdx.x * (256 / L) + threadIdx.x / L;
  if (row >= nrows) return;
  const int a = indptr[row], e = indptr[row + 1];
  double sum = 0.0;
  for (int p = a + lane; p < e; p += L * U) {
    int col[U];
    double v[U];
#pragma unroll
    for (int u = 0; u < U; ++u) {
      const int pp = p + u * L;
      const bool ok = pp < e;
      const int pc = ok ? pp : a;
      col[u] = indices[pc];
      const double vv = (double)val[pc];
      v[u] = ok ? vv : 0.0;
    }
#pragma unroll
    for (int u = 0; u < U; ++u) sum += v[u] * (MODE == 4 ? spmv_prolonged(F, x, col[u]) : x[col[u]]);
  }
#pragma unroll
  for (int o = L / 2; o > 0; o >>= 1) sum += __shfl_down(sum, o, L);
  if (lane == 0) {
    if (MODE == 1) y[row] = x[row] + omega * dinv[row] * (b[row] - sum);
    else if (MODE == 4) y[row] = spmv_prolonged(F, x, row) + omega * dinv[row] * (b[row] - sum);
    else if (MODE == 5) {
      const double res = b[row] - sum;
      y[row] = res;
      F.y2[row] = omega * dinv[row] * res;
    } else y[row] = sum;
  }
}
template <int L, class VT, int MODE>
static void launch_amg_spmv(stream_t s, int U, int64_t nrows, const int32_t* ip, const int32_t* ix, const VT* val,
                            const double* x, double* y, const double* b, const double* dinv, double omega,
                            const SpmvFuse& F) {
  const unsigned blocks = (unsigned)((nrows + 256 / L - 1) / (256 / L));
  if (U <= 2)
    PFV_LAUNCH(HIP_KERNEL_NAME(k_amg_spmv<L, 2, VT, MODE>), dim3(blocks), dim3(256), 0, s, nrows, ip, ix,
                       val, x, y, b, dinv, omega, F);
  else if (U <= 4)
    PFV_LAUNCH(HIP_KERNEL_NAME(k_amg_spmv<L, 4, VT, MODE>), dim3(blocks), dim3(256), 0, s, nrows, ip, ix,
                       val, x, y, b, dinv, omega, F);
  else
    PFV_LAUNCH(HIP_KERNEL_NAME(k_amg_spmv<L, 6, VT, MODE>), dim3(blocks), dim3(256), 0, s, nrows, ip, ix,
                       val, x, y, b, dinv, omega, F);
}
#endif

template <class VT, int MODE>
static void amg_spmv_t(pfv_ctx_impl& c, const CsrPattern& P, const VT* val, const double* x, double* y,
                       const double* b, const double* dinv, double omega, const SpmvFuse& F = SpmvFuse{}) {
  stream_t s = c.stream;
  const int64_t nrows = P.nrows;
  if (nrows == 0) return;
  const int32_t* ip = P.indptr;
  const int32_t* ix = P.indices;
#ifdef PFV_EMULATE
  parallel_for(s, nrows, PFV_LAMBDA(int64_t r) {
    double sum = 0.0;
    for (int p = ip[r]; p < ip[r + 1]; ++p) sum += (double)val[p] * (MODE == 4 ? spmv_prolonged(F, x, ix[p]) : x[ix[p]]);
    if (MODE == 1) y[r] = x[r] + omega * dinv[r] * (b[r] - sum);
    else if (MODE == 4) y[r] = spmv_prolonged(F, x, r) + omega * dinv[r] * (b[r] - sum);
    else if (MODE == 5) {
      const double res = b[r] - sum;
      y[r] = res;
      F.y2[r] = omega * dinv[r] * res;
    } else y[r] = sum;
  });
#else
  const double avg = (double)P.nnz / (double)nrows;
  const int L = avg <= 20 ? 8 : (avg <= 160 ? 16 : 32);
  const int U = std::max(1, std::min(6, (int)std::ceil(1.1 * avg / L)));
  if (L == 8) launch_amg_spmv<8, VT, MODE>(s, U, nrows, ip, ix, val, x, y, b, dinv, omega, F);
  else if (L == 16) launch_amg_spmv<16, VT, MODE>(s, U, nrows, ip, ix, val, x, y, b, dinv, omega, F);
  else launch_amg_spmv<32, VT, MODE>(s, U, nrows, ip, ix, val, x, y, b, dinv, omega, F);
  PFV_HIP_CHECK(hipGetLastError());
#endif
}
static void amg_spmv(pfv_ctx_impl& c, const Amg& amg, const AmgLevel& L, const double* x, double* y,
                     const double* smooth_b) {
  const double* dinv = L.dinv;
#ifndef PFV_EMULATE
  if (L.win && L.win->ok) {
    Reduce R{};
    if (L.v32) {
      if (smooth_b) spmv_win<float, 1>(c, *L.P, *L.win, L.v32, x, y, smooth_b, dinv, L.omega, R);
      else spmv_win<float, 0>(c, *L.P, *L.win, L.v32, x, y, nullptr, nullptr, 0.0, R);
    } else {
      if (smooth_b) spmv_win<double, 1>(c, *L.P, *L.win, L.val, x, y, smooth_b, dinv, L.omega, R);
      else spmv_win<double, 0>(c, *L.P, *L.win, L.val, x, y, nullptr, nullptr, 0.0, R);
    }
    return;
  }
#endif
  if (L.v32) {
    if (smooth_b) amg_spmv_t<float, 1>(c, *L.P, L.v32, x, y, smooth_b, dinv, L.omega);
    else amg_spmv_t<float, 0>(c, *L.P, L.v32, x, y, nullptr, nullptr, 0.0);
  } else {
    if (smooth_b) amg_spmv_t<double, 1>(c, *L.P, L.val, x, y, smooth_b, dinv, L.omega);
    else amg_spmv_t<double, 0>(c, *L.P, L.val, x, y, nullptr, nullptr, 0.0);
  }
}
template <int MODE>
static void amg_spmv_fused(pfv_ctx_impl& c, const AmgLevel& L, const double* x, double* y, const double* b,
                           const SpmvFuse& F) {
  const double* dinv = L.dinv;
#ifndef PFV_EMULATE
  if (L.win && L.win->ok) {
    Reduce R{};
    if (L.v32) spmv_win<float, MODE>(c, *L.P, *L.win, L.v32, x, y, b, dinv, L.omega, R, nullptr, 0, F);
// ... 57 lines not shown
        double a = 0.0, b = 0.0;
        for (int j = 0; j < 64; ++j) { a += p1[j]; b += p2[j]; }
        part[w.item] = a;
        part[kChunks + w.item] = b;
      }
      w.sync();
    });
    double* o = out + 2 * nest;
    parallel_for(s, 1, PFV_LAMBDA(int64_t) {
      double a = 0.0, b = 0.0;
      for (int j = 0; j < kChunks; ++j) { a += part[j]; b += part[kChunks + j]; }
      o[0] = a;
      o[1] = b;
    });
    ++nest;
  }
  if (nest == 0) return;
  std::vector<double> h(2 * nest);
  be_d2h(h.data(), out, sizeof(double) * 2 * nest, s);
  size_t k = 0;
  for (size_t l = 0; l < amg.nlev; ++l) {
    AmgLevel& L = *amg.lev[l];
    const bool smooths = l + 1 < amg.nlev || !amg.dense_ok;
    if (!smooths) continue;
    const double a = h[2 * k], b = h[2 * k + 1];
    ++k;
    double rho = (b > 0.0 && a > 0.0 && a < 1.0e300) ? std::sqrt(a / b) + 1.0 : 0.0;
    if (!(rho > 0.5)) rho = 0.0;
    L.rho = rho;
    if (rho > 0.0) L.omega = std::min(1.0, sigma / rho);
  }
}

template <class VT>
static void amg_restrict_residual(pfv_ctx_impl& c, const Amg& amg, const AmgLevel& L, const AmgLevel& Ln, const VT* val,
                                  const double* b, const double* x, bool next_smooths) {
  stream_t s = c.stream;
  const int bs = amg.bs;
  const double omega = Ln.omega;
  const int32_t* ip = L.P->indptr;
  const int32_t* ix = L.P->indices;
  const int32_t* mptr = L.mptr;
  const int32_t* mem = L.mem;
  double* bc = Ln.b;
  double* xn = Ln.x;
  const double* dn = Ln.dinv;
  wave_for<64>(s, Ln.n, 64 * sizeof(double) + 16, PFV_LAMBDA(const WaveCtx& w) {
    double* sh = reinterpret_cast<double*>(w.lds);
    const int64_t R = w.item;
    const int64_t I = R / bs;
    const int a = (int)(R - I * bs);
    const int q0 = mptr[I], nm = mptr[I + 1] - q0;
    constexpr int SUB = 8;
    double part = 0.0;
    for (int t = w.lane; t < nm * SUB; t += w.width) {
      const int q = t / SUB, sl = t - q * SUB;
      const int64_t r = (int64_t)mem[q0 + q] * bs + a;
      double sum = 0.0;
      for (int p = ip[r] + sl; p < ip[r + 1]; p += SUB) sum += (double)val[p] * x[ix[p]];
      part += (sl == 0 ? b[r] : 0.0) - sum;
    }
    sh[w.lane] = part;
    w.lsync();
    if (w.lane0()) {
      double sum = 0.0;
      for (int j = 0; j < w.width; ++j) sum += sh[j];
      bc[R] = sum;
      if (next_smooths) xn[R] = omega * dn[R] * sum;
    }
    w.lsync();
  });
}
template <class VT>
static void amg_prolong_smooth(pfv_ctx_impl& c, const Amg& amg, const AmgLevel& L, const VT* val, const double* b,
                               const double* x, const double* xc, double* y) {
  stream_t s = c.stream;
  const int bs = amg.bs;
  const double omega = L.omega, alpha = amg.alpha;
  const int32_t* ip = L.P->indptr;
  const int32_t* ix = L.P->indices;
  const int32_t* agg = L.agg;
  const double* dinv = L.dinv;
  wave_for<16>(s, L.n, 16 * sizeof(double) + 16, PFV_LAMBDA(const WaveCtx& w) {
    double* sh = reinterpret_cast<double*>(w.lds);
    const int64_t r = w.item;
    const int p0 = ip[r], len = ip[r + 1] - p0;
    double part = 0.0;
    PFV_LANES(k, len) {
      const int cc = ix[p0 + k];
      const int ci = cc / bs;
      part += (double)val[p0 + k] * (x[cc] + alpha * xc[(int64_t)agg[ci] * bs + (cc - ci * bs)]);
    }
    sh[w.lane] = part;
    w.lsync();
    if (w.lane0()) {
      double sum = 0.0;
      for (int j = 0; j < w.width; ++j) sum += sh[j];
      const int64_t i = r / bs;
      const double tr = x[r] + alpha * xc[(int64_t)agg[i] * bs + (r - i * bs)];
      y[r] = tr + omega * dinv[r] * (b[r] - sum);
    }
    w.lsync();
  });
}

static void amg_restrict(pfv_ctx_impl& c, const Amg& amg, const AmgLevel& L, const AmgLevel& Ln, const double* b,
                         const double* t, bool next_smooths) {
  stream_t s = c.stream;
  const int bs = amg.bs;
  const double omega_n = Ln.omega;
  {
    const int32_t* mptr = L.mptr;
    const int32_t* mem = L.mem;
    double* bc = Ln.b;
    double* xn = Ln.x;
    const double* dn = Ln.dinv;
    if (!amg.restrict_lanes) {
      parallel_for(s, Ln.n, PFV_LAMBDA(int64_t R) {
        const int64_t I = R / bs;
        const int a = (int)(R - I * bs);
        double sum = 0.0;
        for (int q = mptr[I]; q < mptr[I + 1]; ++q) {
          const int64_t r = (int64_t)mem[q] * bs + a;
          sum += b[r] - t[r];
        }
        bc[R] = sum;
        if (next_smooths) xn[R] = omega_n * dn[R] * sum;
      });
    } else
    wave_for<8>(s, Ln.n, 8 * sizeof(double) + 16, PFV_LAMBDA(const WaveCtx& w) {
      double* sh = reinterpret_cast<double*>(w.lds);
      const int64_t R = w.item;
      const int64_t I = R / bs;
      const int a = (int)(R - I * bs);
      const int q0 = mptr[I], nm = mptr[I + 1] - q0;
      double part = 0.0;
      PFV_LANES(q, nm) {
        const int64_t r = (int64_t)mem[q0 + q] * bs + a;
        part += b[r] - t[r];
      }
      sh[w.lane] = part;
      w.lsync();
      if (w.lane0()) {
        double sum = 0.0;
        for (int j = 0; j < w.width; ++j) sum += sh[j];
        bc[R] = sum;
        if (next_smooths) xn[R] = omega_n * dn[R] * sum;
      }
      w.lsync();
    });
  }
}

static double* amg_cycle(pfv_ctx_impl& c, Amg& amg, size_t l, const double* b, double* x, bool x_is_presmoothed,
                         int visit) {
  stream_t s = c.stream;
  AmgLevel& L = *amg.lev[l];
  const int64_t n = L.n;
  const double omega = L.omega, alpha = amg.alpha;
  const double* dinv = L.dinv;
  double* t = L.t;
  if (l + 1 == amg.nlev) {
    if (amg.dense_ok) {
      amg_dense_apply(c, amg.dense, n, b, x);
    } else {
      parallel_for(s, n, PFV_LAMBDA(int64_t i) { x[i] = omega * dinv[i] * b[i]; });
      for (int sweep = 0; sweep < 2; ++sweep) {
        amg_spmv(c, amg, L, x, t, b);
        amg_spmv(c, amg, L, t, x, b);
      }
    }
    return x;
  }
  AmgLevel& Ln = *amg.lev[l + 1];
  const int bs = amg.bs;
  const double omega_n = Ln.omega;
  const AmgPath path = amg_level_path(amg, l);
  const bool small = path.small;
  const bool twice = path.twice;
  const bool fuse_up = path.fuse_up;
  const bool fuse_big = path.fuse_big;
  if (!x_is_presmoothed) parallel_for(s, n, PFV_LAMBDA(int64_t i) { x[i] = omega * dinv[i] * b[i]; });
  const bool next_smooths = l + 2 < amg.nlev;
  if (small) {
    if (L.v32) amg_restrict_residual<float>(c, amg, L, Ln, L.v32, b, x, next_smooths);
    else amg_restrict_residual<double>(c, amg, L, Ln, L.val, b, x, next_smooths);
  } else {
    amg_spmv(c, amg, L, x, t, nullptr);
    amg_restrict(c, amg, L, Ln, b, t, next_smooths);
  }
  double* xc = amg_cycle(c, amg, l + 1, Ln.b, Ln.x, next_smooths, 0);
  const double* xc2 = nullptr;
  if (path.second) {
    double* r2 = Ln.r2.ensure(Ln.n);
    double* x2 = Ln.x2.ensure(Ln.n);
    const double* bcn = Ln.b;
    const double* x2r;
    if (amg.fuse_cycle) {
      SpmvFuse F;
      F.y2 = x2;
      amg_spmv_fused<5>(c, Ln, xc, r2, bcn, F);
      x2r = amg_cycle(c, amg, l + 1, r2, x2, true, 1);
    } else {
      double* tn = Ln.t;
      amg_spmv(c, amg, Ln, xc, tn, nullptr);
      parallel_for(s, Ln.n, PFV_LAMBDA(int64_t i) { r2[i] = bcn[i] - tn[i]; });
      x2r = amg_cycle(c, amg, l + 1, r2, x2, false, 1);
    }
    if (amg.fuse_cycle && !fuse_up) xc2 = x2r;
    else parallel_for(s, Ln.n, PFV_LAMBDA(int64_t i) { xc[i] += x2r[i]; });
  }
  if (fuse_up) {
    if (L.v32) amg_prolong_smooth<float>(c, amg, L, L.v32, b, x, xc, t);
    else amg_prolong_smooth<double>(c, amg, L, L.val, b, x, xc, t);
    return t;
  }
  if (fuse_big) {
    double* out = (twice && visit == 0) ? L.u.ensure(n) : t;
    SpmvFuse F;
    F.xc = xc;
    F.xc2 = xc2;
    F.agg = L.agg;
    F.bs = bs;
    F.alpha = alpha;
    amg_spmv_fused<4>(c, L, x, out, b, F);
    return out;
  }
  {
    const int32_t* agg = L.agg;
    parallel_for(s, n, PFV_LAMBDA(int64_t r) {
      const int64_t i = r / bs;
      const int64_t a = (int64_t)agg[i] * bs + (r - i * bs);
      t[r] = x[r] + alpha * (xc2 ? xc[a] + xc2[a] : xc[a]);
    });
  }
  amg_spmv(c, amg, L, t, x, b);
  return x;
}

struct BlockPc {
  struct Blk {
    int64_t p0 = 0, p1 = 0;
    CsrPattern P;
    Buf<double> val, diag;
    std::unique_ptr<Amg> amg;
  };
  std::vector<int64_t> ptr;
  std::vector<std::unique_ptr<Blk>> blk;
  bool gs = true;
  const double* for_val = nullptr;
  Buf<double> tmp;
  double setup_ms = 0.0;
};

static void blockpc_extract(pfv_ctx_impl& c, const CsrPattern& P, const double* val, BlockPc::Blk& B) {
  stream_t s = c.stream;
  const int64_t p0 = B.p0, n = B.p1 - B.p0;
  const int32_t* ip = P.indptr;
  const int32_t* ix = P.indices;
  Buf<int32_t> len;
  Buf<int64_t> pos;
  int32_t* ln = len.ensure(n + 1);
  int64_t* ps = pos.ensure(n + 1);
  const int64_t p1 = B.p1;
  parallel_for(s, n, PFV_LAMBDA(int64_t r) {
    int m = 0;
    for (int e = ip[p0 + r]; e < ip[p0 + r + 1]; ++e) m += (ix[e] >= p0 && ix[e] < p1) ? 1 : 0;
    ln[r] = m;
  });
  exclusive_scan<int32_t, int64_t>(s, c.scratch, ln, ps, (size_t)n);
  const int64_t nnz = read_scalar<int64_t>(s, ps + n);
  if (nnz >= (int64_t(1) << 31)) throw Error(PFV_ERR_UNSUPPORTED, "block with more than 2^31 entries");
  B.P.nrows = B.P.ncols = n;
  B.P.nnz = nnz;
  int32_t* bip = B.P.indptr.ensure(n + 1);
  int32_t* bix = B.P.indices.ensure(std::max<int64_t>(nnz, 1));
  double* bv = B.val.ensure(std::max<int64_t>(nnz, 1));
  double* bd = B.diag.ensure(n);
  int32_t* st = c.status.ensure(16);
  be_memset(st + 11, 0, sizeof(int32_t), s);
  parallel_for(s, n + 1, PFV_LAMBDA(int64_t r) { bip[r] = (int32_t)ps[r]; });
  parallel_for(s, n, PFV_LAMBDA(int64_t r) {
    int64_t o = ps[r];
    double d = 0.0;
    for (int e = ip[p0 + r]; e < ip[p0 + r + 1]; ++e) {
      const int cc = ix[e];
      if (cc >= p0 && cc < p1) {
        bix[o] = (int32_t)(cc - p0);
        bv[o] = val[e];
        if (cc == p0 + r) d = val[e];
        ++o;
      }
    }
    bd[r] = d;
    if (!(d != 0.0)) atomic_max_i32(st + 11, 1);
  });
  if (read_scalar<int32_t>(s, st + 11))
    throw Error(PFV_ERR_ARGUMENT, "block preconditioner: a diagonal entry is zero (permute the rows first: "
                                  "porepy_amd.solvers.match_rows)");
  B.P.max_row = 0;
}

static void blockpc_setup(pfv_ctx_impl& c, BlockPc& M, const CsrPattern& P, const double* val) {
  Timer tm;
  tm.start(c.stream);
  const size_t nb = M.ptr.size() - 1;
  while (M.blk.size() < nb) M.blk.push_back(std::make_unique<BlockPc::Blk>());
  M.blk.resize(nb);
  for (size_t k = 0; k < nb; ++k) {
    BlockPc::Blk& B = *M.blk[k];
    B.p0 = M.ptr[k];
    B.p1 = M.ptr[k + 1];
    blockpc_extract(c, P, val, B);
    if (!B.amg) B.amg = std::make_unique<Amg>();
    B.amg->valid = false;
    B.amg->coarse_target = kAmgDenseMax;
    amg_setup(c, *B.amg, B.P, B.val, 1, B.diag, nullptr);
  }
  M.for_val = val;
  M.setup_ms = tm.stop(c.stream);
}

static void blockpc_apply(pfv_ctx_impl& c, BlockPc& M, const CsrPattern& P, const double* val, int64_t n,
                          const double* in, double* out) {
  stream_t s = c.stream;
  const int32_t* ip = P.indptr;
  const int32_t* ix = P.indices;
  double* t = M.tmp.ensure(n);
  for (size_t k = 0; k < M.blk.size(); ++k) {
    BlockPc::Blk& B = *M.blk[k];
    const int64_t p0 = B.p0, nk = B.p1 - B.p0;
    const double* rhs = in + p0;
    if (M.gs && k > 0) {
      parallel_for(s, nk, PFV_LAMBDA(int64_t r) {
        double sum = 0.0;
        for (int e = ip[p0 + r]; e < ip[p0 + r + 1]; ++e) {
          const int cc = ix[e];
          if (cc >= p0) break;
          sum += val[e] * out[cc];
        }
        t[p0 + r] = in[p0 + r] - sum;
      });
      rhs = t + p0;
    }
    double* z = amg_cycle(c, *B.amg, 0, rhs, out + p0);
    if (z != out + p0) be_d2d(out + p0, z, sizeof(double) * (size_t)nk, s);
  }
}

struct AmgNns;
static void amg_nns_cycle(pfv_ctx_impl& c, AmgNns& H, size_t l, const double* b, double* x);
struct Sweep;
static void sweep_apply(pfv_ctx_impl& c, const Sweep& sw, const CsrPattern& P, const double* val, const double* diag,
                        const double* in, double* out);
struct Precond {
  Amg* amg = nullptr;
  const Sweep* sweep = nullptr;
  AmgNns* nns = nullptr;
  const double* diag = nullptr;
  BlockPc* blocks = nullptr;
  const CsrPattern* P = nullptr;
  const double* val = nullptr;
};
static void precond_apply(pfv_ctx_impl& c, const Precond& M, int64_t n, const double* in, double* out) {
  if (M.sweep) {
    sweep_apply(c, *M.sweep, *M.P, M.val, M.diag, in, out);
  } else if (M.blocks) {
    blockpc_apply(c, *M.blocks, *M.P, M.val, n, in, out);
  } else if (M.nns) {
    amg_nns_cycle(c, *M.nns, 0, in, out);
  } else if (M.amg && M.amg->dist) {
    amg_apply_dist(c, *M.amg, in, out);
  } else if (M.amg) {
    amg_cycle(c, *M.amg, 0, in, out);
  } else {
    const double* d = M.diag;
    parallel_for(c.stream, n, PFV_LAMBDA(int64_t i) { out[i] = in[i] / d[i]; });
  }
}

}
```

porepy_amd/csrc/backend.h:

```cpp
#pragma once

#include <algorithm>
#include <atomic>
#include <chrono>
#include <cmath>
#include <cstdint>
#include <cstdio>
#include <cstdlib>
#include <cstring>
#include <numeric>
#include <stdexcept>
#include <string>
#include <type_traits>
#include <unordered_map>
#include <vector>

#ifdef PFV_EMULATE
#define PFV_HD
#define PFV_FN inline
#define PFV_LAMBDA [=]
#else
#include <hip/hip_runtime.h>
#include <rocprim/rocprim.hpp>
#define PFV_HD __host__ __device__
#define PFV_FN __host__ __device__ __attribute__((always_inline)) inline
#define PFV_LAMBDA [=] __device__
#define PFV_LAUNCH(kernel, ...)                  \
  do {                                           \
    ::pfv::launch_counter().fetch_add(1, std::memory_order_relaxed); \
    hipLaunchKernelGGL((kernel), __VA_ARGS__);   \
  } while (0)
#endif
#define PFV_LANES(i, n) for (int i = w.lane; i < (int)(n); i += w.width)

namespace pfv {

struct Error : std::runtime_error {
  int status;
  Error(int s, const std::string& m) : std::runtime_error(m), status(s) {}
};

constexpr int kWave = 64;

inline std::atomic<long long>& launch_counter() {
  static std::atomic<long long> c{0};
  return c;
}

#ifndef PFV_EMULATE
#define PFV_HIP_CHECK(expr)                                                              \
  do {                                                                                   \
    hipError_t e_ = (expr);                                                              \
    if (e_ != hipSuccess)                                                                \
      throw ::pfv::Error(3, std::string(#expr) + ": " + hipGetErrorString(e_));          \
  } while (0)
using stream_t = hipStream_t;
#else
using stream_t = int;
#endif

inline void* raw_malloc(size_t bytes) {
#ifdef PFV_EMULATE
  void* p = std::malloc(bytes);
  if (!p) throw Error(3, "host emulation: out of memory");
  return p;
#else
  void* p = nullptr;
  PFV_HIP_CHECK(hipMalloc(&p, bytes));
  return p;
#endif
}
inline void raw_free(void* p) {
#ifdef PFV_EMULATE
  std::free(p);
#else
  (void)hipFree(p);
#endif
}

struct MemPool {
  struct Blk { void* p; size_t bytes; };
  std::vector<Blk> free_list;
  std::unordered_map<void*, size_t> live;
  size_t cached = 0;
  static constexpr size_t kMaxCached = size_t(48) << 30;
  void* take(size_t bytes) {
    size_t best = (size_t)-1, best_bytes = (size_t)-1;
    for (size_t i = 0; i < free_list.size(); ++i) {
      const size_t b = free_list[i].bytes;
      if (b >= bytes && b <= 2 * bytes + (size_t(1) << 16) && b < best_bytes) { best = i; best_bytes = b; }
    }
    void* p;
    if (best != (size_t)-1) {
      p = free_list[best].p;
      cached -= best_bytes;
      free_list[best] = free_list.back();
      free_list.pop_back();
      live[p] = best_bytes;
    } else {
      p = raw_malloc(bytes);
      live[p] = bytes;
    }
    return p;
  }
  bool give(void* p) {
    auto it = live.find(p);
    if (it == live.end()) return false;
    const size_t b = it->second;
    live.erase(it);
    if (cached + b > kMaxCached) raw_free(p);
    else { free_list.push_back({p, b}); cached += b; }
    return true;
  }
  void trim() {
    for (auto& b : free_list) raw_free(b.p);
    free_list.clear();
    cached = 0;
  }
  ~MemPool() { trim(); }
};
inline thread_local MemPool* tls_pool = nullptr;
struct PoolScope {
  MemPool* prev;
  explicit PoolScope(MemPool* p) : prev(tls_pool) { tls_pool = p; }
  ~PoolScope() { tls_pool = prev; }
};

inline void* be_malloc(size_t bytes) {
  if (bytes == 0) bytes = 8;
  return tls_pool ? tls_pool->take(bytes) : raw_malloc(bytes);
}
inline void be_free(void* p) {
  if (!p) return;
  if (tls_pool && tls_pool->give(p)) return;
  raw_free(p);
}
#ifndef PFV_EMULATE
inline bool spin_wait_enabled() {
  static const bool on = [] {
    const char* e = std::getenv("PFV_SPIN_WAIT");
    return !(e && std::atoi(e) == 0);
  }();
  return on;
}
inline int env_int_early(const char* name, int dflt) {
  const char* e = std::getenv(name);
  return e ? std::atoi(e) : dflt;
}
inline void wait_stream(stream_t s) {
  if (!spin_wait_enabled()) {
    PFV_HIP_CHECK(hipStreamSynchronize(s));
    return;
  }
  for (;;) {
    const hipError_t e = hipStreamQuery(s);
    if (e == hipSuccess) return;
    if (e != hipErrorNotReady) PFV_HIP_CHECK(e);
  }
}
inline void* pinned_scratch() {
  thread_local void* p = nullptr;
  if (!p) PFV_HIP_CHECK(hipHostMalloc(&p, 4096, hipHostMallocDefault));
  return p;
}
#endif
inline void be_h2d(void* dst, const void* src, size_t bytes, stream_t s) {
  if (!bytes) return;
#ifdef PFV_EMULATE
  (void)s;
  std::memcpy(dst, src, bytes);
#else
  PFV_HIP_CHECK(hipMemcpyAsync(dst, src, bytes, hipMemcpyHostToDevice, s));
  wait_stream(s);
#endif
}
inline void be_d2h(void* dst, const void* src, size_t bytes, stream_t s) {
  if (!bytes) return;
#ifdef PFV_EMULATE
  (void)s;
  std::memcpy(dst, src, bytes);
#else
  if (bytes <= 4096 && spin_wait_enabled()) {
    void* p = pinned_scratch();
    PFV_HIP_CHECK(hipMemcpyAsync(p, src, bytes, hipMemcpyDeviceToHost, s));
    wait_stream(s);
    std::memcpy(dst, p, bytes);
    return;
  }
  if (bytes >= (size_t(8) << 20) && env_int_early("PFV_PINNED_COPIES", 0) != 0) {
    constexpr size_t kChunk = size_t(16) << 20;
    thread_local char* stage[2] = {nullptr, nullptr};
    thread_local hipEvent_t ev[2] = {nullptr, nullptr};
    for (int i = 0; i < 2; ++i) {
      if (!stage[i]) {
        PFV_HIP_CHECK(hipHostMalloc(reinterpret_cast<void**>(&stage[i]), kChunk, hipHostMallocDefault));
        PFV_HIP_CHECK(hipEventCreateWithFlags(&ev[i], hipEventDisableTiming));
      }
    }
    const char* sp = static_cast<const char*>(src);
    char* dp = static_cast<char*>(dst);
    const size_t nchunk = (bytes + kChunk - 1) / kChunk;
    auto issue = [&](size_t k) {
      const size_t off = k * kChunk, len = std::min(kChunk, bytes - off);
      PFV_HIP_CHECK(hipMemcpyAsync(stage[k & 1], sp + off, len, hipMemcpyDeviceToHost, s));
      PFV_HIP_CHECK(hipEventRecord(ev[k & 1], s));
    };
    issue(0);
    for (size_t k = 0; k < nchunk; ++k) {
      if (k + 1 < nchunk) issue(k + 1);
      for (;;) {
        const hipError_t e = hipEventQuery(ev[k & 1]);
        if (e == hipSuccess) break;
        if (e != hipErrorNotReady) PFV_HIP_CHECK(e);
      }
      const size_t off = k * kChunk, len = std::min(kChunk, bytes - off);
      std::memcpy(dp + off, stage[k & 1], len);
    }
    return;
  }
  PFV_HIP_CHECK(hipMemcpyAsync(dst, src, bytes, hipMemcpyDeviceToHost, s));
  wait_stream(s);
#endif
}
inline void be_d2d(void* dst, const void* src, size_t bytes, stream_t s) {
  if (!bytes) return;
#ifdef PFV_EMULATE
  (void)s;
  std::memmove(dst, src, bytes);
#else
  PFV_HIP_CHECK(hipMemcpyAsync(dst, src, bytes, hipMemcpyDeviceToDevice, s));
#endif
}
inline void be_memset(void* dst, int value, size_t bytes, stream_t s) {
  if (!bytes) return;
#ifdef PFV_EMULATE
  (void)s;
  std::memset(dst, value, bytes);
#else
  PFV_HIP_CHECK(hipMemsetAsync(dst, value, bytes, s));
#endif
}
inline void be_sync(stream_t s) {
#ifdef PFV_EMULATE
  (void)s;
#else
  wait_stream(s);
#endif
}

template <class T>
struct Buf {
  T* p = nullptr;
  size_t cap = 0;
  Buf() = default;
  Buf(const Buf&) = delete;
  Buf& operator=(const Buf&) = delete;
  ~Buf() { be_free(p); }
  T* ensure(size_t n) {
    if (n > cap) {
      const size_t room = std::min(cap / 8, (size_t(64) << 20) / sizeof(T));
      size_t want = cap > 0 ? std::max(n, cap + room) : n;
      be_free(p);
      p = nullptr;
      cap = 0;
      if (want > n) {
        try {
          p = static_cast<T*>(be_malloc(want * sizeof(T)));
        } catch (const Error&) {
          p = nullptr;
          want = n;
        }
      }
      if (!p) p = static_cast<T*>(be_malloc(want * sizeof(T)));
      cap = want;
    }
    return p;
  }
  void release() {
    be_free(p);
    p = nullptr;
    cap = 0;
  }
  void swap(Buf& o) {
    std::swap(p, o.p);
    std::swap(cap, o.cap);
  }
  operator T*() const { return p; }
};

struct Timer {
#ifdef PFV_EMULATE
  std::chrono::steady_clock::time_point t0;
  void start(stream_t) { t0 = std::chrono::steady_clock::now(); }
  double stop(stream_t) {
    return std::chrono::duration<double, std::milli>(std::chrono::steady_clock::now() - t0).count();
  }
#else
  hipEvent_t a = nullptr, b = nullptr;
  Timer() {
    (void)hipEventCreate(&a);
    (void)hipEventCreate(&b);
  }
  ~Timer() {
    if (a) (void)hipEventDestroy(a);
    if (b) (void)hipEventDestroy(b);
  }
  Timer(const Timer&) = delete;
  void start(stream_t s) { PFV_HIP_CHECK(hipEventRecord(a, s)); }
  double stop(stream_t s) {
    PFV_HIP_CHECK(hipEventRecord(b, s));
    if (spin_wait_enabled()) {
      for (;;) {
        const hipError_t e = hipEventQuery(b);
        if (e == hipSuccess) break;
        if (e != hipErrorNotReady) PFV_HIP_CHECK(e);
      }
    } else {
      PFV_HIP_CHECK(hipEventSynchronize(b));
    }
    float ms = 0.f;
    PFV_HIP_CHECK(hipEventElapsedTime(&ms, a, b));
    return ms;
  }
  void mark(stream_t s) { PFV_HIP_CHECK(hipEventRecord(b, s)); }
  double elapsed_after_sync() {
    PFV_HIP_CHECK(hipEventSynchronize(b));
    float ms = 0.f;
    PFV_HIP_CHECK(hipEventElapsedTime(&ms, a, b));
    return ms;
  }
#endif
};

#ifndef PFV_EMULATE
struct StreamFork {
  stream_t main, side;
  hipEvent_t e0 = nullptr, e1 = nullptr;
  bool joined = false;
  StreamFork(stream_t m, stream_t sd) : main(m), side(sd) {
    PFV_HIP_CHECK(hipEventCreateWithFlags(&e0, hipEventDisableTiming));
    PFV_HIP_CHECK(hipEventCreateWithFlags(&e1, hipEventDisableTiming));
    PFV_HIP_CHECK(hipEventRecord(e0, main));
    PFV_HIP_CHECK(hipStreamWaitEvent(side, e0, 0));
  }
  void join() {
    PFV_HIP_CHECK(hipEventRecord(e1, side));
    PFV_HIP_CHECK(hipStreamWaitEvent(main, e1, 0));
    joined = true;
  }
  ~StreamFork() {
    if (!joined) (void)hipStreamSynchronize(side);
    if (e0) (void)hipEventDestroy(e0);
    if (e1) (void)hipEventDestroy(e1);
  }
  StreamFork(const StreamFork&) = delete;
};
#endif

struct WaveCtx {
  int64_t item;
  char* lds;
  int lane;
  int width;
  char* red;
#ifdef PFV_EMULATE
  bool lane0() const { return true; }
  void sync() const {}
  void lsync() const {}
  int argmax_abs(const double* base, int stride, int lo, int hi, double* best) const {
    double b = -1.0;
    int p = lo;
    for (int i = lo; i < hi; ++i) {
      const double a = std::fabs(base[(size_t)i * stride]);
      if (a > b) { b = a; p = i; }
    }
    *best = b;
    return p;
  }
#else
  __device__ bool lane0() const { return lane == 0; }
  __device__ void sync() const { __syncthreads(); }
  __device__ void lsync() const {
    if (width > 64) {
      __syncthreads();
    } else {
      __builtin_amdgcn_fence(__ATOMIC_SEQ_CST, "wavefront");
      __builtin_amdgcn_wave_barrier();
    }
  }
  __device__ int argmax_abs(const double* base, int stride, int lo, int hi, double* best) const {
    double b = -1.0;
    int p = 0x7fffffff;
    for (int i = lo + lane; i < hi; i += width) {
      const double a = fabs(base[(size_t)i * stride]);
      if (a > b) { b = a; p = i; }
    }
    const int w = width < 64 ? width : 64;
// ... 137 lines not shown

template <class F>
inline void wave_for_g(int G, stream_t s, int64_t n, size_t lds_bytes, F f) {
  if (G <= 16) wave_for<16>(s, n, lds_bytes, f);
  else if (G <= 32) wave_for<32>(s, n, lds_bytes, f);
  else wave_for<64>(s, n, lds_bytes, f);
}

template <class F>
inline void wave_for_xcd(stream_t s, int64_t n, size_t lds_bytes, F f) {
#ifdef PFV_EMULATE
  wave_for<64>(s, n, lds_bytes, f);
#else
  if (n < 4096) {
    wave_for<64>(s, n, lds_bytes, f);
    return;
  }
  lds_bytes = (lds_bytes + 15) & ~size_t(15);
  if (lds_bytes > 160 * 1024) throw Error(5, "work item needs more than 160 KiB of LDS");
  int64_t blocks = n > 256 * 64 ? 256 * 64 : ((n + 7) & ~int64_t(7));
  if (lds_bytes > 48 * 1024) {
    PFV_HIP_CHECK(hipFuncSetAttribute(reinterpret_cast<const void*>(&k_wave_for_xcd<64, F>),
                                      hipFuncAttributeMaxDynamicSharedMemorySize, (int)lds_bytes));
  }
  PFV_LAUNCH(HIP_KERNEL_NAME(k_wave_for_xcd<64, F>), dim3((unsigned)blocks), dim3(64), lds_bytes, s, n,
                     lds_bytes, f);
  PFV_HIP_CHECK(hipGetLastError());
#endif
}
inline int env_int(const char* name, int dflt) {
  const char* e = std::getenv(name);
  return e ? std::atoi(e) : dflt;
}

#ifndef PFV_EMULATE
template <int T, class F>
__global__ void __launch_bounds__(T) k_block_for(int64_t n, size_t lds_bytes, F f) {
  extern __shared__ __attribute__((aligned(16))) char pfv_lds[];
  for (int64_t b = blockIdx.x; b < n; b += gridDim.x) {
    WaveCtx w{b, pfv_lds, (int)threadIdx.x, T, pfv_lds + lds_bytes};
    f(w);
    __syncthreads();
  }
}
#endif
#ifndef PFV_EMULATE
template <int T, class F>
__global__ void __launch_bounds__(T) k_block_for_global(int64_t n, size_t bytes, char* scratch, F f) {
  extern __shared__ __attribute__((aligned(16))) char pfv_lds[];
  char* mine = scratch + (size_t)blockIdx.x * bytes;
  for (int64_t b = blockIdx.x; b < n; b += gridDim.x) {
    WaveCtx w{b, mine, (int)threadIdx.x, T, pfv_lds};
    f(w);
    __syncthreads();
  }
}
#endif
template <int T = 256, class F>
inline void block_for_global(stream_t s, int64_t n, size_t bytes, Buf<char>& scratch, F f) {
  if (n <= 0) return;
  bytes = (bytes + 255) & ~size_t(255);
#ifdef PFV_EMULATE
  (void)s;
  (void)scratch;
  std::vector<double> mem((bytes + 7) / 8 + 2);
  for (int64_t b = 0; b < n; ++b) {
    WaveCtx w{b, reinterpret_cast<char*>(mem.data()), 0, 1, nullptr};
    f(w);
  }
#else
  const int64_t blocks = n < 256 ? n : 256;
  char* buf = scratch.ensure((size_t)blocks * bytes);
  PFV_LAUNCH(HIP_KERNEL_NAME(k_block_for_global<T, F>), dim3((unsigned)blocks), dim3(T), 256, s, n, bytes, buf, f);
  PFV_HIP_CHECK(hipGetLastError());
#endif
}

template <int T = 256, class F>
inline void block_for(stream_t s, int64_t n, size_t lds_bytes, F f) {
  if (n <= 0) return;
  lds_bytes = (lds_bytes + 15) & ~size_t(15);
#ifdef PFV_EMULATE
  (void)s;
  std::vector<double> lds((lds_bytes + 7) / 8 + 2);
  for (int64_t b = 0; b < n; ++b) {
    WaveCtx w{b, reinterpret_cast<char*>(lds.data()), 0, 1, nullptr};
    f(w);
  }
#else
  const size_t total = lds_bytes + 256;
  if (total > 160 * 1024) throw Error(5, "work item needs more than 160 KiB of LDS");
  int64_t blocks = n < 256 * 8 ? n : 256 * 8;
  if (total > 48 * 1024) {
    PFV_HIP_CHECK(hipFuncSetAttribute(reinterpret_cast<const void*>(&k_block_for<T, F>),
                                      hipFuncAttributeMaxDynamicSharedMemorySize, (int)total));
  }
  PFV_LAUNCH(HIP_KERNEL_NAME(k_block_for<T, F>), dim3((unsigned)blocks), dim3(T), total, s, n, lds_bytes, f);
  PFV_HIP_CHECK(hipGetLastError());
#endif
}

struct Scratch {
  Buf<char> tmp;
};

inline void sort_pairs(stream_t s, Scratch& sc, const uint32_t* kin, uint32_t* kout,
                       const int32_t* vin, int32_t* vout, size_t n, int bits) {
  if (n == 0) return;
#ifdef PFV_EMULATE
  (void)s; (void)sc; (void)bits;
  std::vector<size_t> idx(n);
  std::iota(idx.begin(), idx.end(), size_t(0));
  std::stable_sort(idx.begin(), idx.end(), [&](size_t a, size_t b) { return kin[a] < kin[b]; });
  for (size_t i = 0; i < n; ++i) {
    kout[i] = kin[idx[i]];
    vout[i] = vin[idx[i]];
  }
#else
  size_t bytes = 0;
  PFV_HIP_CHECK(rocprim::radix_sort_pairs(nullptr, bytes, kin, kout, vin, vout, n, 0, bits, s));
  sc.tmp.ensure(bytes);
  PFV_HIP_CHECK(rocprim::radix_sort_pairs(sc.tmp.p, bytes, kin, kout, vin, vout, n, 0, bits, s));
#endif
}

template <class TI, class TO>
inline void exclusive_scan(stream_t s, Scratch& sc, const TI* in, TO* out, size_t n) {
#ifdef PFV_EMULATE
  (void)s; (void)sc;
  TO acc = 0;
  for (size_t i = 0; i < n; ++i) {
    out[i] = acc;
    acc += (TO)in[i];
  }
  out[n] = acc;
#else
  auto it = rocprim::make_transform_iterator(
      rocprim::make_counting_iterator<size_t>(0),
      [in, n] __device__(size_t i) -> TO { return i < n ? (TO)in[i] : TO(0); });
  size_t bytes = 0;
  PFV_HIP_CHECK(rocprim::exclusive_scan(nullptr, bytes, it, out, TO(0), n + 1, rocprim::plus<TO>(), s));
  sc.tmp.ensure(bytes);
  PFV_HIP_CHECK(rocprim::exclusive_scan(sc.tmp.p, bytes, it, out, TO(0), n + 1, rocprim::plus<TO>(), s));
#endif
}

template <class T>
inline T read_scalar(stream_t s, const T* dptr) {
  T v;
  be_d2h(&v, dptr, sizeof(T), s);
  return v;
}

template <class T>
PFV_FN int lower_bound_idx(const T* a, int n, T key) {
  int lo = 0, hi = n;
  while (lo < hi) {
    int mid = (lo + hi) >> 1;
    if (a[mid] < key) lo = mid + 1; else hi = mid;
  }
  return lo;
}

template <class T>
PFV_FN int upper_bound_idx(const T* a, int n, T key) {
  int lo = 0, hi = n;
  while (lo < hi) {
    int mid = (lo + hi) >> 1;
    if (a[mid] <= key) lo = mid + 1; else hi = mid;
  }
  return lo;
}
PFV_HD inline int popcount64(unsigned long long x) { return __builtin_popcountll(x); }
PFV_HD inline void atomic_or_u64(unsigned long long* addr, unsigned long long v) {
#ifdef PFV_EMULATE
  *addr |= v;
#else
#if defined(__HIP_DEVICE_COMPILE__)
  atomicOr(addr, v);
#else
  (void)addr; (void)v;
#endif
#endif
}

PFV_HD inline void atomic_max_i32(int* addr, int v);
PFV_HD inline void track_max_i32(int* addr, int v) {
  if (v > *reinterpret_cast<volatile int*>(addr)) atomic_max_i32(addr, v);
}
PFV_HD inline void atomic_max_i32(int* addr, int v) {
#ifdef PFV_EMULATE
  if (v > *addr) *addr = v;
#else
#if defined(__HIP_DEVICE_COMPILE__)
  atomicMax(addr, v);
#else
  (void)addr; (void)v;
#endif
#endif
}
PFV_HD inline void atomic_min_i32(int* addr, int v) {
#ifdef PFV_EMULATE
  if (v < *addr) *addr = v;
#else
#if defined(__HIP_DEVICE_COMPILE__)
  atomicMin(addr, v);
#else
  (void)addr; (void)v;
#endif
#endif
}
PFV_HD inline int atomic_fetch_add_i32(int* addr, int v) {
#ifdef PFV_EMULATE
  const int old = *addr;
  *addr += v;
  return old;
#else
#if defined(__HIP_DEVICE_COMPILE__)
  return atomicAdd(addr, v);
#else
  (void)addr; (void)v;
  return 0;
#endif
#endif
}
PFV_HD inline void atomic_add_i32(int* addr, int v) {
#ifdef PFV_EMULATE
  *addr += v;
#else
#if defined(__HIP_DEVICE_COMPILE__)
  atomicAdd(addr, v);
#else
  (void)addr; (void)v;
#endif
#endif
}

}
```

porepy_amd/csrc/ctx.h:

```cpp
#pragma once
#include "../../include/porefv.h"
#include "backend.h"

#include <algorithm>
#include <functional>
#include <memory>
#include <vector>

namespace pfv {

constexpr int kMaxFaceNodes = 8;
constexpr int kMaxCellFaces = 16;
constexpr int kMaxBlock = 255;
static const int kClassBounds[] = {4, 8, 12, 16, 24, 32, 40, 48, 64, 96, 128, 192, 255};
constexpr int kNumClasses = 13;

struct alignas(16) SfRec {
  int64_t toff;
  uint8_t n;
  uint8_t ls;
  uint8_t jstar;
  uint8_t deg;
  uint8_t r[3];
  uint8_t pad;
  double om[3];
  double nk[3];
};
static_assert(sizeof(SfRec) == 64, "SfRec is one 64-byte record");

struct alignas(16) FaceRec {
  int32_t f;
  int32_t a;
  int32_t p0;
  int32_t q0;
  uint32_t lens;
  uint32_t nnf;
  int32_t pad[2];
};
static_assert(sizeof(FaceRec) == 32, "FaceRec is one 32-byte record");

struct CsrPattern {
  int64_t nrows = 0, ncols = 0, nnz = 0;
  Buf<int32_t> indptr, indices;
  int max_row = 0;
};

struct WinCsr {
  Buf<int64_t> wptr64buf;
  const int64_t* wptr64 = nullptr;
  const int32_t* wlen = nullptr;
  Buf<int32_t> wcol, cnt;
  Buf<uint16_t> lidx;
  int64_t nblk = 0, nrows = 0, nnz = 0;
  int wmax = 0;
  bool ok = false;
};

struct LinSys {
  const CsrPattern* P = nullptr;
  double* val = nullptr;
  double* diag = nullptr;
  double* rhs = nullptr;
  int64_t n = 0;
  bool valid = false;
  const WinCsr* win = nullptr;
};

struct Amg;
struct BlockPc;
struct AmgNns;
struct Sweep;

struct pfv_ctx_impl {
  MemPool pool;
  pfv_ctx_impl();
  ~pfv_ctx_impl();
  int device = 0;
  stream_t stream{};
  stream_t own_stream{};
  Buf<double> sys_rowmax;
  const double* sys_rowmax_for = nullptr;
  stream_t aux_stream{};
  std::string err;
  Scratch scratch;

  bool have_grid = false;
  int nd = 0;
  int64_t nc = 0, nf = 0, nn = 0, ncf = 0, nsf = 0;
  Buf<double> nodes, fnorm, fcen, ccen, farea;
  bool periodic = false;
  Buf<double> face_shift;
  Buf<int32_t> face_native;
  Buf<int32_t> cf_ptr, cf_idx, fn_ptr, fn_idx;
  Buf<int8_t> cf_sgn;

  bool have_params = false;
  Buf<double> perm;
  Buf<uint8_t> bcflag;
  Buf<double> robin;
  double eta = 0.0;
  bool have_eta_sub = false;
  Buf<double> eta_sub;

  bool have_topology = false;
  int64_t nh = 0;
  Buf<int32_t> node_hptr;
  Buf<int32_t> h_cell;
  Buf<uint8_t> h_lf;
  Buf<int8_t> h_sgn;
  Buf<uint8_t> h_first;
  Buf<int32_t> node_fptr;
  Buf<int32_t> node_sf;
  Buf<int32_t> node_face;
  Buf<int32_t> sf_face;
  Buf<uint8_t> sf_ls;
  Buf<int32_t> face_nsides;
  Buf<int32_t> node_cells;
  Buf<int32_t> node_bptr;
  Buf<int32_t> node_bfaces;
  Buf<uint8_t> node_bls;
  Buf<int64_t> node_tptr;
  Buf<int64_t> node_tbptr;
  Buf<uint8_t> flux_colpairs;
  int64_t cp_stride = 0;
  Buf<uint8_t> node_active;
  Buf<int32_t> face_subset;
  bool biot_rows_complete = false;
  Buf<int32_t> cell_subset;
  Buf<int32_t> face_order;
  double bbox_lo[3] = {0, 0, 0}, bbox_hi[3] = {1, 1, 1};
  Buf<int32_t> node_order;
  std::vector<int64_t> class_begin;
  int max_block = 0, max_deg = 0, max_face_nodes = 0, max_cell_faces = 0, max_bnd_per_node = 0;
  int64_t sum_block_sq = 0;
  int64_t tab_len = 0, tabb_len = 0;

  Buf<double> tab;
  Buf<double> tabb;
  Buf<SfRec> sf_rec;
  Buf<int32_t> face_ctr;
  unsigned face_ctr_next = 0;
  Buf<FaceRec> face_rec;
  Buf<int32_t> status;

  bool have_symbolic = false, have_numeric = false, have_system = false;
  bool have_flow_rhs = false;
  bool rows_complete = false;
  CsrPattern pat_flux, pat_bound, pat_vs, pat_A;
  bool vs_indices_pending = false;
  bool vs_implicit = false;
  Buf<double> val[PFV_NUM_MATS];
  bool filled[PFV_NUM_MATS] = {};
  Buf<double> rhs, diag, xsol, face_tmp, vec_in;
  Buf<double> kry[10];
  Buf<double> red;
  Buf<double> gmres_basis, gmres_small;

  bool have_mpsa_params = false, have_mpsa_numeric = false, have_mpsa_symbolic = false, have_mech_system = false;
  Buf<double> stiff;
  Buf<double> cvol;
  Buf<uint8_t> bc_dirbits, bc_neubits, bc_robbits;
  Buf<double> mpsa_robw;
  bool have_mpsa_robin = false;
  bool have_mpsa_eta_sub = false;
  bool mpsa_hf_on = false;
  double mpsa_hf_eta = 0.0;
  Buf<double> mpsa_hf_eta_sub;
  bool have_mpsa_hf_eta_sub = false;
  Buf<double> Et2, Etb2;
  Buf<double> mpsa_eta_sub;
  Buf<double> mpsa_basis;
  bool have_mpsa_basis = false;
  Buf<double> mpsa_basis_sub;
  bool have_mpsa_basis_sub = false;
  Buf<char> mpsa_scratch;
  bool mpsa_subface_bc = false, have_mpsa_sub_symbolic = false;
  Buf<uint8_t> bc_dirbits_sub, bc_neubits_sub, bc_robbits_sub;
  Buf<double> mpsa_robw_sub;
  bool have_mpsa_robin_sub = false;
  CsrPattern pat_sstress, pat_sbstress, pat_bdf_s, pat_sbdface;
  Buf<uint8_t> bdf_src;
  double mpsa_eta = 0.0;
  Buf<int32_t> cell_nnodes;
  Buf<int64_t> node_eptr, node_ebptr;
  Buf<double> Es, Et, Esb, Etb;
  CsrPattern pat_stress, pat_bstress, pat_Am;
  int biot_nalpha = 0;
  Buf<double> biot_alpha;
  bool have_biot_symbolic = false, have_biot_numeric = false;
  Buf<int32_t> cn_ptr, cn_idx;
  Buf<int64_t> node_dptr, node_dbptr, node_cptr;
  int64_t biot_tot_p = 0, biot_tot_d = 0, biot_tot_db = 0, biot_tot_c = 0;
  Buf<double> bEsp, bEtp, bDD, bBDD, bCONS;
  CsrPattern pat_sg, pat_dd, pat_bdd;
  Buf<double> biot_val[5 * 8];
  CsrPattern pat_user;
  CsrPattern pat_bpf;
  bool rows_complete_m = false;
  bool subface_bc = false;
  Buf<uint8_t> bcflag_s;
  Buf<double> robin_s;
  CsrPattern pat_sflux, pat_sbound;
  bool have_sub_symbolic = false;
  bool tpfa_mode = false;
  Buf<double> rhs_u, diag_u;
  std::vector<int32_t> mpsa_class_lds;
  Buf<double> rhs_m, diag_m;
  bool vectors_on_device = false;
  LinSys active;
  WinCsr win_rows;
  const int32_t* win_rows_for = nullptr;
  int64_t win_rows_n = 0;
  WinCsr win_sys, win_block;
  bool active_is_grid = false;
  bool have_cell_order = false;
  bool cell_order_identity = false;
  Buf<int32_t> cell_perm, cell_iperm;
  CsrPattern pat_perm;
  Buf<double> val_perm, diag_perm, rhs_perm, x_perm;
  const double* perm_for_val = nullptr;
  const int32_t* win_for = nullptr;
  bool win_sys_prebuilt = false;
  bool win_rows_prebuilt = false;
  int active_bs = 1;
  int precond = 0;
  std::unique_ptr<Amg> amg;
  const double* amg_for_val = nullptr;
  Buf<unsigned long long> csum_work;
  unsigned long long pat_A_checksum = 0;
  unsigned long long win_sys_checksum = 0;
  unsigned long long win_rows_checksum = 0;
  unsigned long long symbolic_epoch = 0;
  unsigned long long topo_key = 0;
  Buf<uint8_t> asm_pos, asm_diagpos;
  unsigned long long asm_pos_key = 0;
  int64_t asm_pos_cells = 0;
  Buf<uint8_t> asm_pos_m, asm_diagpos_m;
  unsigned long long asm_pos_m_key = 0;
  int64_t asm_pos_m_rows = 0;
  unsigned long long symb_key = 0;
  std::unique_ptr<BlockPc> block_pc;
  std::unique_ptr<Amg> amg_block;
  int amg_last = 0;
  std::unique_ptr<AmgNns> amg_nns;
  const double* amg_nns_for_val = nullptr;
  unsigned long long amg_nns_key = 0;
  unsigned long long grid_serial = 0;
  bool nns_stale = true;
  std::vector<double> nns_B;
  int nns_k = 0, nns_bs = 0;
  int64_t nns_n = 0;
  unsigned long long nns_key = 0;
  Buf<double> nns_col, nns_row;
  Buf<double> nns_cc;
  unsigned long long amg_nns_cfg = 0;
  CsrPattern pat_block;
  Buf<double> val_block;
  const pfv_shard_hooks* shard = nullptr;
  bool shard_overlap = false;
  Buf<int32_t> shard_blocks;
  int64_t shard_n_interior = 0, shard_n_boundary = 0;
  Buf<int32_t> node_redo;
  std::function<void(stream_t, int64_t)> node_redo_launch;
  int64_t stats_node_redo = 0;
  Buf<int32_t> mpsa_redo;
  Buf<int32_t> mpsa_cell_exp;
  Buf<uint8_t> mpsa_wide_flag;
  Buf<int32_t> mpsa_wide_list;
  Buf<int32_t> mpsa_wide_stat;
  int64_t stats_mpsa_redo = 0;
  Buf<double> red5;
  double* shard_work = nullptr;
  int64_t shard_nloc = 0;

  bool have_q_res = false;
  Buf<double> q_res;
  bool have_upw_bc = false;
  Buf<uint8_t> upw_bc;
  bool have_upwind = false, have_transport = false, have_pat_T = false;
  bool have_upw_cells = false;
  int upw_ncomp = 0;
  Buf<double> upw_q;
  Buf<int32_t> upw_side, upw_cnt;
  Buf<int32_t> upw_up;
  Buf<uint8_t> upw_cls;
  CsrPattern pat_upw, pat_upw_dir, pat_upw_neu, pat_T;
  Buf<double> rhs_t, diag_t, bref_t, acc_t, src_t, c_t, c_keep, q_t, bc_t;
  bool have_acc_t = false, have_src_t = false;
  int64_t transport_zero_diag = -1;
  Buf<double> mc_q, mc_bc, mc_acc, mc_src, mc_c;
  Buf<double> mc_acc_i, mc_src_i, mc_bref_i, mc_x, mc_z, mc_r, mc_nrm, mc_col;
  Buf<double> nl_q, nl_bc, nl_acc, nl_src, nl_sink, nl_s, nl_s2, nl_phi, nl_phi2, nl_bref, nl_rhs, nl_t, nl_cb, nl_ct;
  Buf<double> nl_table, nl_out;
  Buf<double> nlc_cbc, nlc_ads_in, nlc_src_in, nlc_c_in;
  Buf<double> nlc_ads, nlc_src, nlc_bref, nlc_x, nlc_z, nlc_psi, nlc_psi2, nlc_rhs, nlc_t, nlc_cb, nlc_ct;
  Buf<double> rc_q, rc_bc, rc_acc_in, rc_src_in, rc_c_in, rc_rho;
  Buf<double> rc_acc, rc_src, rc_bref, rc_x, rc_z, rc_prev, rc_rhs, rc_g, rc_F, rc_par, rc_out;
  bool have_tpos_T = false;
  Buf<int32_t> tpos_T, aj_slot, aj_obs;
  Buf<double> valT_T;
  Buf<double> aj_loads, aj_state_in, aj_sA, aj_sB, aj_lam, aj_lam2, aj_prev, aj_r, aj_gsrc, aj_gacc, aj_gbc, aj_gq;

  bool have_advdiff = false;
  bool have_adv_bD = false;
  double adv_w = 1.0;
  Buf<double> adv_fb, adv_bD;
  Buf<double> adv_q, adv_bc;
  Buf<double> adv_acc, adv_src, adv_c, adv_keep, adv_rhs, adv_diag, adv_bref;
// ... 52 lines not shown
```

porepy_amd/csrc/linalg.inc:

```

namespace pfv {

static void assemble_system(pfv_ctx_impl& c) {
  stream_t s = c.stream;
  const int64_t nc = c.nc;
  double* Aval = c.val[PFV_MAT_SYSTEM].ensure(c.pat_A.nnz);
  double* diag = c.diag.ensure(nc);
  const int32_t* cf_ptr = c.cf_ptr;
  const int32_t* cf_idx = c.cf_idx;
  const int8_t* cf_sgn = c.cf_sgn;
  const int32_t* ip = c.pat_flux.indptr;
  const int32_t* ix = c.pat_flux.indices;
  const int32_t* ap = c.pat_A.indptr;
  const int32_t* ax = c.pat_A.indices;
  const double* vq = c.val[PFV_MAT_FLUX];
  const int maxrow = std::max(c.pat_A.max_row, 1);
  const size_t lds = (size_t)std::max(maxrow, 64) * 12 + 32;
  double* rowmax = c.sys_rowmax.ensure(nc);
  c.sys_rowmax_for = Aval;
#ifndef PFV_EMULATE
  constexpr int kAsmFaces = 6, kAsmChunks = 4;
  if (c.max_cell_faces <= kAsmFaces && c.pat_flux.max_row <= 16 * kAsmChunks && env_int("PFV_ASM_G", 16) == 16 &&
      env_int("PFV_ASM_PREFETCH", 1) != 0) {
    const int stride_f = 16 * kAsmChunks;
// ... 588 lines not shown
        wc.sync();
      }
      if (wc.lane0()) partial[(int64_t)k * nb + b] = sh[0];
      wc.sync();
    }
  });
  parallel_for(s, 5, PFV_LAMBDA(int64_t k) {
    double a = 0.0;
    for (int i = 0; i < nb; ++i) a += partial[k * nb + i];
    out5[k] = a;
  });
}
PFV_HD inline void apply_merged_omega(double* S, const double* g) {
  const double ts = g[0], tt = g[1], ss = g[2], hs = g[3], ht = g[4];
  const double om = (tt != 0.0) ? ts / tt : 0.0;
  S[S_TS] = ts;
  S[S_TT] = tt;
  S[S_OMEGA] = om;
  const double rr = ss - 2.0 * om * ts + om * om * tt;
  S[S_RR] = rr > 0.0 ? rr : 0.0;
  const double rho_new = hs - om * ht;
  S[S_RHO_OLD] = S[S_RHO];
  S[S_RHO] = rho_new;
  S[S_BETA] = (rho_new / S[S_RHO_OLD]) * (S[S_ALPHA] / om);
}

static void shard_halo(pfv_ctx_impl& c, double* x) {
  if (!c.shard) return;
  if (c.shard->exchange_halo(c.shard->user, x, (void*)(intptr_t)c.stream))
    throw Error(PFV_ERR_ARGUMENT, "exchange_halo hook failed");
}

static void finish_reduction(pfv_ctx_impl& c, int nblocks, const Reduce& R, int mode);
static void spmv_dot(pfv_ctx_impl& c, const CsrPattern& P, const double* val, const double* x, double* y,
                     const double* w, int dot, const Reduce& R, int mode, const WinCsr* W = nullptr);

static void shard_spmv(pfv_ctx_impl& c, const CsrPattern& P, const double* val, double* x, double* y, const double* w,
                       int dot, const Reduce& R, int mode, const WinCsr* W) {
#ifndef PFV_EMULATE
  if (c.shard && c.shard_overlap && W && W->ok && c.aux_stream) {
    {
      StreamFork fork(c.stream, c.aux_stream);
      if (c.shard->exchange_halo(c.shard->user, x, (void*)(intptr_t)c.aux_stream))
        throw Error(PFV_ERR_ARGUMENT, "exchange_halo hook failed");
      const int32_t* li = c.shard_blocks.p;
      if (dot == 0) spmv_win<double, 0>(c, P, *W, val, x, y, nullptr, nullptr, 0.0, R, li, c.shard_n_interior);
      else if (dot == 1) spmv_win<double, 2>(c, P, *W, val, x, y, w, nullptr, 0.0, R, li, c.shard_n_interior);
      else spmv_win<double, 3>(c, P, *W, val, x, y, w, nullptr, 0.0, R, li, c.shard_n_interior);
      fork.join();
    }
    const int32_t* lb = c.shard_blocks.p + c.shard_n_interior;
    if (dot == 0) spmv_win<double, 0>(c, P, *W, val, x, y, nullptr, nullptr, 0.0, R, lb, c.shard_n_boundary);
    else if (dot == 1) spmv_win<double, 2>(c, P, *W, val, x, y, w, nullptr, 0.0, R, lb, c.shard_n_boundary);
    else spmv_win<double, 3>(c, P, *W, val, x, y, w, nullptr, 0.0, R, lb, c.shard_n_boundary);
    if (dot) finish_reduction(c, (int)W->nblk, R, mode);
    return;
  }
#endif
  shard_halo(c, x);
  spmv_dot(c, P, val, x, y, w, dot, R, mode, W);
}

static void finish_reduction(pfv_ctx_impl& c, int nblocks, const Reduce& R, int mode) {
  const int m1 = c.shard ? (int)M_RAW : mode;
#ifdef PFV_EMULATE
  (void)nblocks;
  finalize_scalars(c, R.partial, R.stride, R.S, m1);
#else
  launch_finalize(c.stream, nblocks, R, m1);
#endif
  if (c.shard) {
    double* raw = c.shard_work + 2 * c.shard_nloc;
    double* S = R.S;
    be_d2d(raw, S + S_RAW0, 2 * sizeof(double), c.stream);
    if (c.shard->allreduce_sum(c.shard->user, raw, 2, (void*)(intptr_t)c.stream))
      throw Error(PFV_ERR_ARGUMENT, "allreduce_sum hook failed");
    parallel_for(c.stream, 1, PFV_LAMBDA(int64_t) { apply_scalar_mode(S, raw[0], raw[1], mode); });
  }
}

static void spmv_dot(pfv_ctx_impl& c, const CsrPattern& P, const double* val, const double* x, double* y,
                     const double* w, int dot, const Reduce& R, int mode, const WinCsr* W) {
#ifdef PFV_EMULATE
  (void)W;
  spmv(c, P, val, x, y);
  if (dot == 1) dot_partials(c, P.nrows, w, y, nullptr, nullptr, R.partial, R.stride);
  if (dot == 2) dot_partials(c, P.nrows, y, w, y, y, R.partial, R.stride);
  if (dot) finish_reduction(c, 0, R, mode);
#else
  if (W && W->ok) {
    if (dot == 0) spmv_win<double, 0>(c, P, *W, val, x, y, nullptr, nullptr, 0.0, R);
    else if (dot == 1) spmv_win<double, 2>(c, P, *W, val, x, y, w, nullptr, 0.0, R);
    else spmv_win<double, 3>(c, P, *W, val, x, y, w, nullptr, 0.0, R);
    if (dot) finish_reduction(c, (int)W->nblk, R, mode);
    return;
  }
  if (dot == 0) {
    spmv(c, P, val, x, y);
    return;
  }
  stream_t s = c.stream;
  const int64_t nrows = P.nrows;
  const double avg = (double)P.nnz / (double)nrows;
  const int L = avg <= 20 ? 8 : (avg <= 160 ? 16 : 32);
  int U = (int)std::ceil(1.1 * avg / L);
  U = std::max(1, std::min(6, U));
  const int64_t groups = (nrows + 256 / L - 1) / (256 / L);
  const int blocks = (int)groups;
  if (L == 8) {
    if (dot == 1) launch_spmv_dot_u<8, 1>(s, blocks, U, nrows, P.indptr, P.indices, val, x, y, w, R, mode);
    else launch_spmv_dot_u<8, 2>(s, blocks, U, nrows, P.indptr, P.indices, val, x, y, w, R, mode);
  } else if (L == 16) {
    if (dot == 1) launch_spmv_dot_u<16, 1>(s, blocks, U, nrows, P.indptr, P.indices, val, x, y, w, R, mode);
    else launch_spmv_dot_u<16, 2>(s, blocks, U, nrows, P.indptr, P.indices, val, x, y, w, R, mode);
  } else {
    if (dot == 1) launch_spmv_dot_u<32, 1>(s, blocks, U, nrows, P.indptr, P.indices, val, x, y, w, R, mode);
    else launch_spmv_dot_u<32, 2>(s, blocks, U, nrows, P.indptr, P.indices, val, x, y, w, R, mode);
  }
  finish_reduction(c, blocks, R, mode);
  PFV_HIP_CHECK(hipGetLastError());
#endif
}

static void sys_spmv(pfv_ctx_impl& c, const LinSys& sys, const double* x, double* y) {
#ifndef PFV_EMULATE
  if (sys.win && sys.win->ok) {
    Reduce R{};
    spmv_win<double, 0>(c, *sys.P, *sys.win, sys.val, x, y, nullptr, nullptr, 0.0, R);
    return;
  }
#endif
  spmv(c, *sys.P, sys.val, x, y);
}

static void dot2(pfv_ctx_impl& c, int64_t n, const double* x1, const double* y1, const double* x2,
                 const double* y2, const Reduce& R, int mode) {
#ifdef PFV_EMULATE
  dot_partials(c, n, x1, y1, x2, y2, R.partial, R.stride);
  finish_reduction(c, 0, R, mode);
#else
  const int blocks = (int)std::min<int64_t>((n + 255) / 256, kRedBlocks);
  PFV_LAUNCH(k_dot2, dim3(blocks), dim3(256), 0, c.stream, n, x1, y1, x2, y2, R, mode);
  finish_reduction(c, blocks, R, mode);
  PFV_HIP_CHECK(hipGetLastError());
#endif
}

struct SolveResult {
  int iterations = 0;
  bool converged = false;
  double relres = 0.0;
};

static SolveResult krylov_solve(pfv_ctx_impl& c, const LinSys& sys, int method, double rtol, int maxit,
                                double* d_x, bool x_is_zero, const Precond* M = nullptr) {
  stream_t s = c.stream;
  const int64_t n = sys.n;
  const CsrPattern& P = *sys.P;
  const double* Aval = sys.val;
  const double* diag = sys.diag;
  const double* d_b = sys.rhs;
  double* r = c.kry[0].ensure(n);
  double* rhat = c.kry[1].ensure(n);
  const bool sharded = c.shard != nullptr;
  const bool sh_cg = sharded && method == PFV_SOLVE_CG;
  double* p = sh_cg ? c.shard_work : c.kry[2].ensure(n);
  double* v = c.kry[3].ensure(n);
  double* y = (sharded && !sh_cg) ? c.shard_work : c.kry[4].ensure(n);
  double* z = sharded ? c.shard_work + c.shard_nloc : c.kry[5].ensure(n);
  double* t = c.kry[6].ensure(n);
  Reduce R;
  R.stride = std::max<int64_t>(kRedBlocks, n / 8 + 2);
  double* red = c.red.ensure(2 * R.stride + S_COUNT + 2 * 128);
  R.partial = red;
  R.S = red + 2 * R.stride;
  double* S = R.S;
  const int merged = (sharded && method == PFV_SOLVE_BICGSTAB && env_int("PFV_SHARD_MERGED_DOTS", 1) != 0) ? 1 : 0;
  const int check_every = sharded ? std::max(1, env_int("PFV_SHARD_CHECK_EVERY", 4)) : ((M || n < 200000) ? 1 : 10);
  SolveResult res;

  if (x_is_zero) {
    be_d2d(r, d_b, sizeof(double) * n, s);
  } else {
    if (sharded) throw Error(PFV_ERR_ARGUMENT, "a sharded solve starts from zero");
    sys_spmv(c, sys, d_x, t);
    parallel_for(s, n, PFV_LAMBDA(int64_t i) { r[i] = d_b[i] - t[i]; });
  }
  dot2(c, n, d_b, d_b, nullptr, nullptr, R, M_BB);
  const double bb = read_scalar<double>(s, S + S_BB);
  if (!(bb > 0.0)) {
    be_memset(d_x, 0, sizeof(double) * n, s);
    res.converged = true;
    return res;
  }
  const double tol2 = rtol * rtol * bb;

  if (method == PFV_SOLVE_CG) {
    if (M) {
      precond_apply(c, *M, n, r, z);
      be_d2d(p, z, sizeof(double) * n, s);
    } else {
      parallel_for(s, n, PFV_LAMBDA(int64_t i) {
        const double zi = r[i] / diag[i];
        z[i] = zi;
        p[i] = zi;
      });
    }
    dot2(c, n, r, r, r, z, R, M_START);
    for (int it = 1; it <= maxit; ++it) {
      shard_halo(c, p);
      spmv_dot(c, P, Aval, p, v, p, 1, R, M_CG_ALPHA, sys.win);
      if (M) {
        parallel_for(s, n, PFV_LAMBDA(int64_t i) {
          const double al = S[S_ALPHA];
          d_x[i] += al * p[i];
          r[i] -= al * v[i];
        });
        precond_apply(c, *M, n, r, z);
        dot2(c, n, r, r, r, z, R, M_CG_BETA);
      } else {
#ifdef PFV_EMULATE
      parallel_for(s, n, PFV_LAMBDA(int64_t i) {
        const double al = S[S_ALPHA];
        d_x[i] += al * p[i];
        const double ri = r[i] - al * v[i];
        r[i] = ri;
        z[i] = ri / diag[i];
      });
      dot2(c, n, r, r, r, z, R, M_CG_BETA);
#else
      {
        const int blocks = (int)std::min<int64_t>((n + 255) / 256, kRedBlocks);
        PFV_LAUNCH(k_cg_tail, dim3(blocks), dim3(256), 0, s, n, d_x, r, z, p, v, diag, R, (int)M_CG_BETA);
        finish_reduction(c, blocks, R, M_CG_BETA);
      }
#endif
      }
      parallel_for(s, n, PFV_LAMBDA(int64_t i) { p[i] = z[i] + S[S_BETA] * p[i]; });
      res.iterations = it;
      if (it % check_every == 0 || it == maxit) {
        const double rr = read_scalar<double>(s, S + S_RR);
        res.relres = std::sqrt(rr / bb);
        if (rr <= tol2) { res.converged = true; break; }
        if (!(rr == rr)) break;
      }
    }
    return res;
  }

  constexpr int kTrueResidualRestarts = 3;
  int restarts = 0;
  int it = 1;
restart_bicgstab:
  be_d2d(rhat, r, sizeof(double) * n, s);
  be_memset(p, 0, sizeof(double) * n, s);
  be_memset(v, 0, sizeof(double) * n, s);
  dot2(c, n, r, r, rhat, r, R, M_START);
  for (; it <= maxit; ++it) {
    if (M) {
      parallel_for(s, n, PFV_LAMBDA(int64_t i) { p[i] = r[i] + S[S_BETA] * (p[i] - S[S_OMEGA] * v[i]); });
      precond_apply(c, *M, n, p, y);
    } else {
      parallel_for(s, n, PFV_LAMBDA(int64_t i) {
        const double pi = r[i] + S[S_BETA] * (p[i] - S[S_OMEGA] * v[i]);
        p[i] = pi;
        y[i] = pi / diag[i];
      });
    }
    shard_spmv(c, P, Aval, y, v, rhat, 1, R, M_ALPHA, sys.win);
    if (M) {
      parallel_for(s, n, PFV_LAMBDA(int64_t i) { r[i] -= S[S_ALPHA] * v[i]; });
      precond_apply(c, *M, n, r, z);
    } else {
      parallel_for(s, n, PFV_LAMBDA(int64_t i) {
        const double si = r[i] - S[S_ALPHA] * v[i];
        r[i] = si;
        z[i] = si / diag[i];
      });
    }
    if (merged) {
      shard_spmv(c, P, Aval, z, t, r, 0, R, M_OMEGA, sys.win);
      double* raw = c.shard_work + 2 * c.shard_nloc;
      shard_dot5(c, n, t, r, rhat, c.red5.ensure(5 * kDot5Blocks), raw);
      if (c.shard->allreduce_sum(c.shard->user, raw, 5, (void*)(intptr_t)c.stream))
        throw Error(PFV_ERR_ARGUMENT, "allreduce_sum hook failed");
      parallel_for(s, 1, PFV_LAMBDA(int64_t) { apply_merged_omega(S, raw); });
      parallel_for(s, n, PFV_LAMBDA(int64_t i) {
        const double om = S[S_OMEGA];
        d_x[i] += S[S_ALPHA] * y[i] + om * z[i];
        r[i] -= om * t[i];
      });
    } else {
    shard_halo(c, z);
    spmv_dot(c, P, Aval, z, t, r, 2, R, M_OMEGA, sys.win);
#ifdef PFV_EMULATE
    parallel_for(s, n, PFV_LAMBDA(int64_t i) {
      const double om = S[S_OMEGA];
      d_x[i] += S[S_ALPHA] * y[i] + om * z[i];
      r[i] -= om * t[i];
    });
    dot2(c, n, r, r, rhat, r, R, M_RHO_BETA);
#else
    {
      const int blocks = (int)std::min<int64_t>((n + 255) / 256, kRedBlocks);
      PFV_LAUNCH(k_bicg_tail, dim3(blocks), dim3(256), 0, s, n, d_x, r, y, z, t, rhat, R, (int)M_RHO_BETA);
      finish_reduction(c, blocks, R, M_RHO_BETA);
    }
#endif
    }
    res.iterations = it;
    if (it % check_every == 0 || it == maxit) {
      const double rr = read_scalar<double>(s, S + S_RR);
      res.relres = std::sqrt(rr / bb);
      if (rr <= tol2) { res.converged = true; break; }
      if (!(rr == rr)) break;
    }
  }
  if (res.converged && !sharded && env_int("PFV_TRUE_RESIDUAL", 1) != 0) {
    sys_spmv(c, sys, d_x, t);
    parallel_for(s, n, PFV_LAMBDA(int64_t i) { r[i] = d_b[i] - t[i]; });
    dot2(c, n, r, r, nullptr, nullptr, R, M_RAW);
    const double rr_true = read_scalar<double>(s, S + S_RAW0);
    res.relres = std::sqrt(rr_true / bb);
    if (!(rr_true <= tol2)) {
      res.converged = false;
      if (restarts < kTrueResidualRestarts && it < maxit && rr_true == rr_true) {
        ++restarts;
        ++it;
        goto restart_bicgstab;
      }
    }
  }
  return res;
}

constexpr int kGmresBlocks = 1024;
constexpr int kGmresGroup = 8;

static void gmres_multi_dot(pfv_ctx_impl& c, int64_t n, const double* V, int64_t ld, int nv, const double* w,
                            double* partial, double* out, bool accumulate) {
  stream_t s = c.stream;
  const int nb = (int)std::min<int64_t>(kGmresBlocks, (n + 2047) / 2048);
  block_for<256>(s, nb, 256 * sizeof(double), PFV_LAMBDA(const WaveCtx& wc) {
    double* sh = reinterpret_cast<double*>(wc.lds);
    const int64_t b = wc.item;
    const int64_t lo = n * b / nb, hi = n * (b + 1) / nb;
    for (int k0 = 0; k0 < nv; k0 += kGmresGroup) {
      const int kc = (nv - k0) < kGmresGroup ? (nv - k0) : kGmresGroup;
      double acc[kGmresGroup];
      for (int k = 0; k < kGmresGroup; ++k) acc[k] = 0.0;
      for (int64_t i = lo + wc.lane; i < hi; i += wc.width) {
        const double wi = w[i];
        for (int k = 0; k < kGmresGroup; ++k)
          if (k < kc) acc[k] += V[(int64_t)(k0 + k) * ld + i] * wi;
      }
      for (int k = 0; k < kc; ++k) {
        sh[wc.lane] = acc[k];
        wc.sync();
        for (int o = wc.width >> 1; o > 0; o >>= 1) {
          if (wc.lane < o) sh[wc.lane] += sh[wc.lane + o];
          wc.sync();
        }
        if (wc.lane0()) partial[(int64_t)(k0 + k) * nb + b] = sh[0];
        wc.sync();
      }
    }
  });
  block_for<256>(s, nv, 256 * sizeof(double), PFV_LAMBDA(const WaveCtx& wc) {
    double* sh = reinterpret_cast<double*>(wc.lds);
    const int64_t k = wc.item;
    double a = 0.0;
    for (int i = wc.lane; i < nb; i += wc.width) a += partial[k * nb + i];
    sh[wc.lane] = a;
    wc.sync();
    for (int o = wc.width >> 1; o > 0; o >>= 1) {
      if (wc.lane < o) sh[wc.lane] += sh[wc.lane + o];
      wc.sync();
    }
    if (wc.lane0()) out[k] = accumulate ? out[k] + sh[0] : sh[0];
    wc.sync();
  });
}

static void gmres_multi_axpy(pfv_ctx_impl& c, int64_t n, const double* V, int64_t ld, int nv, const double* coef,
                             double* w) {
  parallel_for(c.stream, n, PFV_LAMBDA(int64_t i) {
    double wi = w[i];
    for (int k = 0; k < nv; ++k) wi -= coef[k] * V[(int64_t)k * ld + i];
    w[i] = wi;
  });
}

static SolveResult gmres_solve(pfv_ctx_impl& c, const LinSys& sys, double rtol, int maxit, int restart,
                               double* d_x, bool x_is_zero, const Precond* Mp = nullptr) {
  Precond Mj;
  Mj.diag = sys.diag;
  const Precond& M = Mp ? *Mp : Mj;
  stream_t s = c.stream;
  const int64_t n = sys.n;
  const CsrPattern& P = *sys.P;
  const double* Aval = sys.val;
  const double* diag = sys.diag;
  const double* d_b = sys.rhs;
  int m = restart > 0 ? std::min(restart, 200) : 30;
  m = std::min(m, std::max(1, maxit));
  double* V = c.gmres_basis.ensure((int64_t)(m + 1) * n);
  double* w = c.kry[0].ensure(n);
  double* y = c.kry[1].ensure(n);
  const int ldh = m + 1;
  double* st = c.gmres_small.ensure((int64_t)ldh * m + 6 * (m + 2) + 8);
  double* Rm = st;
  double* cs = Rm + (int64_t)ldh * m;
  double* sn = cs + m + 2;
  double* g = sn + m + 2;
  double* hcol = g + m + 2;
  double* ysol = hcol + m + 2;
  double* scal = ysol + m + 2;
  double* partial = c.red.ensure((int64_t)(m + 2) * kGmresBlocks + 64);
  SolveResult res;

  gmres_multi_dot(c, n, d_b, n, 1, d_b, partial, scal + 3, false);
  const double bb = read_scalar<double>(s, scal + 3);
  if (!(bb > 0.0)) {
    be_memset(d_x, 0, sizeof(double) * n, s);
    res.converged = true;
    return res;
  }
  if (x_is_zero) be_memset(d_x, 0, sizeof(double) * n, s);
  const double tol2 = rtol * rtol * bb;
  const int check_every = (n < 200000) ? 1 : 5;
  bool first = true;
  while (res.iterations < maxit) {
    double* v0 = V;
    if (first && x_is_zero) {
      be_d2d(v0, d_b, sizeof(double) * n, s);
    } else {
      sys_spmv(c, sys, d_x, w);
      parallel_for(s, n, PFV_LAMBDA(int64_t i) { v0[i] = d_b[i] - w[i]; });
    }
    first = false;
    gmres_multi_dot(c, n, v0, n, 1, v0, partial, scal, false);
    const double rr0 = read_scalar<double>(s, scal);
    res.relres = std::sqrt(rr0 / bb);
    if (rr0 <= tol2) { res.converged = true; break; }
    if (!(rr0 == rr0)) break;
    parallel_for(s, 1, PFV_LAMBDA(int64_t) {
      const double beta = sqrt(scal[0]);
      scal[1] = 1.0 / beta;
      for (int i = 0; i < m + 2; ++i) g[i] = 0.0;
      g[0] = beta;
    });
    parallel_for(s, n, PFV_LAMBDA(int64_t i) { v0[i] *= scal[1]; });
    int j = 0;
    bool stop = false;
    for (; j < m && res.iterations < maxit && !stop; ++j) {
      const double* vj = V + (int64_t)j * n;
      precond_apply(c, M, n, vj, y);
      sys_spmv(c, sys, y, w);
      gmres_multi_dot(c, n, V, n, j + 1, w, partial, hcol, false);
      gmres_multi_axpy(c, n, V, n, j + 1, hcol, w);
      gmres_multi_dot(c, n, V, n, j + 1, w, partial, ysol, false);
      gmres_multi_axpy(c, n, V, n, j + 1, ysol, w);
      gmres_multi_dot(c, n, w, n, 1, w, partial, scal, false);
      parallel_for(s, 1, PFV_LAMBDA(int64_t) {
        for (int i = 0; i <= j; ++i) hcol[i] += ysol[i];
        const double hn = sqrt(scal[0]);
        scal[1] = hn > 0.0 ? 1.0 / hn : 0.0;
        for (int i = 0; i < j; ++i) {
// ... 53 lines not shown
```

porepy_amd/csrc/porefv.hip:

```cpp
#include <cmath>
#include <cstring>

#include "ctx.h"
#include "fluxfn.h"
#include "react.h"
namespace pfv {
static int rccl_exchange_halo(void* user, double* d_x, void* stream);
}
#include "topology.inc"
#include "mpfa_numeric.inc"
#include "linalg.inc"
#include "reorder.inc"
#include "dd.h"
#include "mpsa.inc"
#include "tpfa.inc"
#include "biot.inc"
#include "ad_flux.inc"
#include "upwind.inc"
#include "advdiff.inc"
#include "sweep.inc"

namespace pfv {
#ifndef PFV_EMULATE
__global__ void __launch_bounds__(256) k_triad(int64_t n2, D2* __restrict__ a, const D2* __restrict__ b,
// ... 2939 lines not shown
    const pfv::Amg* ap = h->amg_last == 1 ? h->amg.get() : (h->amg_last == 2 ? h->amg_block.get() : nullptr);
    require(ap && ap->valid, "no AMG hierarchy (pfv_amg_setup or a solve with PFV_PRECOND_AMG first)");
    const pfv::Amg& amg = *ap;
    if (amg.dist) throw pfv::Error(PFV_ERR_UNSUPPORTED, "pfv_amg_level does not read the coupled hierarchy of a sharded solve");
    require(level >= 0 && (size_t)level < amg.nlev, "level out of range");
    const size_t l = (size_t)level;
    const pfv::AmgLevel& L = *amg.lev[l];
    const bool last = l + 1 == amg.nlev;
    const bool filtered = l == 0 && amg.filter_theta > 0.0 && amg.filt_nnz > 0;
    const pfv::CsrPattern* Pa = filtered ? &amg.filtP : L.P;
    const double* Va = filtered ? amg.filtV.p : L.val;
    const pfv::AmgPath path = pfv::amg_level_path(amg, l);
    int maxcap = 0;
    for (const auto& g : amg.gal_sizes) maxcap = std::max(maxcap, g.maxcap);
    info[0] = L.n;
    info[1] = amg.bs;
    info[2] = (int64_t)amg.nlev;
    info[3] = last ? 0 : L.nc_cells;
    info[4] = Pa->nnz;
    info[5] = L.P->nnz;
    info[6] = l == 0 ? amg.sysP->nnz : 0;
    info[7] = L.v32 ? 1 : 0;
    info[8] = (path.small ? 1 : 0) | (path.fuse_up ? 2 : 0) | (path.fuse_big ? 4 : 0) | (path.twice ? 8 : 0) |
              (path.second ? 16 : 0) | (path.second && amg.fuse_cycle ? 32 : 0) | (last && amg.dense_ok ? 64 : 0) |
              (last && !amg.dense_ok ? 128 : 0);
    info[9] = amg.dense_ok ? 1 : 0;
    info[10] = amg.gamma;
    info[11] = amg.gamma_levels;
    info[12] = amg.fuse_rows;
    info[13] = amg.fuse_cycle ? 1 : 0;
    info[14] = amg.reused ? 1 : 0;
    info[15] = amg.filter_level0 ? 1 : 0;
    info[16] = amg.restrict_lanes ? 1 : 0;
    info[17] = (L.win && L.win->ok) ? 1 : 0;
    info[18] = (!last && L.mptr.p && L.mem.p) ? 1 : 0;
    info[19] = maxcap;
    info[20] = pfv::kAmgDenseMax;
    info[21] = pfv::kGalEpl;
    info[22] = pfv::kGalMaxMembers;
    info[23] = pfv::kAmgWTopRows;
    if (params) {
      params[0] = L.omega;
      params[1] = amg.alpha;
      params[2] = amg.filter_theta;
      params[3] = L.rho;
    }
    auto s = h->stream;
    auto csr = [&](const pfv::CsrPattern& P, const double* v, int32_t* ip, int32_t* ix, double* val) {
      if (ip) be_d2h(ip, P.indptr.p, sizeof(int32_t) * (size_t)(P.nrows + 1), s);
      if (ix && P.nnz > 0) be_d2h(ix, P.indices.p, sizeof(int32_t) * (size_t)P.nnz, s);
      if (val && P.nnz > 0) be_d2h(val, v, sizeof(double) * (size_t)P.nnz, s);
    };
    if (l == 0) csr(*amg.sysP, amg.sysV, sys_indptr, sys_indices, sys_val);
    csr(*Pa, Va, a_indptr, a_indices, a_val);
    csr(*L.P, L.val, op_indptr, op_indices, op_val);
    if (dinv) be_d2h(dinv, L.dinv.p, sizeof(double) * (size_t)L.n, s);
    const int64_t cells = L.n / amg.bs;
    if (!last) {
      if (agg) be_d2h(agg, L.agg.p, sizeof(int32_t) * (size_t)cells, s);
      if (mptr) be_d2h(mptr, L.mptr.p, sizeof(int32_t) * (size_t)(L.nc_cells + 1), s);
      if (mem) be_d2h(mem, L.mem.p, sizeof(int32_t) * (size_t)cells, s);
    }
    if (dense && last && amg.dense_ok) be_d2h(dense, amg.dense.p, sizeof(double) * (size_t)(L.n * L.n), s);
    pfv::be_sync(s);
  });
}

static pfv::LinSys solver_system(pfv_ctx* h, bool& permuted) {
  pfv::LinSys sys = h->active;
  const int bs = h->active_bs;
  permuted = false;
  if (h->active_is_grid && sys.n == h->nc * bs && pfv::env_int("PFV_REORDER", 1) != 0 &&
      h->nc >= pfv::env_int("PFV_REORDER_MIN_CELLS", 256)) {
    if (!h->have_cell_order) pfv::build_cell_order(*h);
  }
  if (h->active_is_grid && h->have_cell_order && !h->cell_order_identity && sys.n == h->nc * bs &&
      pfv::env_int("PFV_REORDER", 1) != 0 && h->nc >= pfv::env_int("PFV_REORDER_MIN_CELLS", 256)) {
    if (h->perm_for_val != sys.val) {
      pfv::permute_matrix(*h, sys, bs);
      h->perm_for_val = sys.val;
      values_changed(h, Windows::drop, true);
    }
    pfv::permute_vector(*h, sys.n, bs, sys.rhs, h->rhs_perm.ensure(sys.n), true);
    sys.P = &h->pat_perm;
    sys.val = h->val_perm.p;
    sys.diag = h->diag_perm.p;
    sys.rhs = h->rhs_perm.p;
    permuted = true;
  }
  sys.win = nullptr;
  if (sys.P->nnz >= pfv::env_int("PFV_SPMV_WINDOW_MIN_NNZ", 20000)) {
    if (h->win_for != sys.P->indices.p || !h->win_sys.ok || pfv::env_int("PFV_SPMV_WINDOW", 1) == 0) {
      h->win_sys_checksum = 0;
      pfv::win_build(*h, *sys.P, h->win_sys);
      h->win_for = sys.P->indices.p;
      if (h->win_sys.ok && sys.P == &h->pat_A && h->have_symbolic) h->win_sys_checksum = h->pat_A_checksum;
    }
    sys.win = &h->win_sys;
  }
  return sys;
}

pfv_status pfv_solve(pfv_ctx* h, int method, double rtol, int maxit, int restart, const double* x0,
                     double* x, pfv_solve_info* info) {
  pfv::SolveResult res;
  pfv_status st = guarded(h, [&] {
    require(h->active.valid, "assemble first");
    require(x != nullptr, "x is required");
    require(method == PFV_SOLVE_CG || method == PFV_SOLVE_BICGSTAB || method == PFV_SOLVE_GMRES,
            "method must be PFV_SOLVE_CG, PFV_SOLVE_BICGSTAB or PFV_SOLVE_GMRES");
    require(rtol > 0 && maxit > 0, "rtol and maxit must be positive");
    const bool sweep_transport = h->precond == PFV_PRECOND_SWEEP && transport_is_active(h);
    const bool sweep_advdiff = h->precond == PFV_PRECOND_SWEEP && !sweep_transport && advdiff_is_active(h);
    if (h->precond == PFV_PRECOND_SWEEP && !sweep_transport && !sweep_advdiff)
      throw pfv::Error(PFV_ERR_UNSUPPORTED, "PFV_PRECOND_SWEEP applies to the transport system (pfv_upwind_assemble) and to "
                                            "the advection-diffusion system (pfv_advdiff_assemble) of the handle only: the "
                                            "active system is neither");
    h->stats.sweep_levels = h->stats.sweep_core_cells = h->stats.sweep_launches = 0;
    h->stats.sweep_direct_steps = h->stats.sweep_direct_fallbacks = 0;
    h->stats.sweep_order_ms = 0.0;
    if (h->precond == PFV_PRECOND_SWEEP) {
      const int which = sweep_transport ? PFV_MAT_TRANSPORT_SYSTEM : PFV_MAT_ADVDIFF_SYSTEM;
      if (!h->sweep) h->sweep = std::make_unique<pfv::Sweep>();
      if (!h->sweep->valid || h->sweep->for_system != which) {
        pfv::sweep_build_order(*h, *h->sweep, sweep_transport ? h->transport_q : h->adv_q.p, which);
        h->stats.sweep_order_ms = h->sweep->order_ms;
      }
    }
    if (transport_is_active(h) && h->transport_zero_diag >= 0)
      throw pfv::Error(PFV_ERR_UNSUPPORTED, "zero diagonal entry in row " + std::to_string(h->transport_zero_diag) +
                                                " of the transport system (a cell without outflow and without an "
                                                "accumulation term): the Jacobi-preconditioned solver does not apply");
    if (h->have_advdiff && active_is(h, PFV_MAT_ADVDIFF_SYSTEM) && h->advdiff_zero_diag >= 0)
      throw pfv::Error(PFV_ERR_UNSUPPORTED, "zero diagonal entry in row " + std::to_string(h->advdiff_zero_diag) +
                                                " of the advection-diffusion system: the solver does not apply");
    auto s = h->stream;
    const size_t n = (size_t)h->active.n;
    double* dx = h->xsol.ensure(n);
    if (x0) vec_in(h, dx, x0, n); else pfv::be_memset(dx, 0, n * sizeof(double), s);
    pfv::Timer tm;
    tm.start(s);
    bool permuted = false;
    const pfv::LinSys sys = solver_system(h, permuted);
    h->stats.solve_renumbered = permuted ? 1 : 0;
    double* dxs = dx;
    if (permuted) {
      dxs = h->x_perm.ensure(n);
      if (x0) pfv::permute_vector(*h, (int64_t)n, h->active_bs, dx, dxs, true);
      else pfv::be_memset(dxs, 0, n * sizeof(double), s);
    }
    pfv::Precond M;
    const pfv::Precond* Mp = nullptr;
    const long long launches_before_setup = pfv::launch_counter().load(std::memory_order_relaxed);
    if (h->precond == PFV_PRECOND_AMG) {
      if (!h->amg) h->amg = std::make_unique<pfv::Amg>();
      if (!h->amg->valid || h->amg_for_val != sys.val) {
        pfv::amg_setup(*h, *h->amg, *sys.P, sys.val, h->active_bs, sys.diag, sys.win);
        h->amg_for_val = sys.val;
        h->amg_last = 1;
        amg_setup_stats(h, *h->amg, (int64_t)h->amg->nlev, h->amg->lev[h->amg->nlev - 1]->n, h->amg->reused);
        h->stats.amg_stale_rematches = h->amg->stale_rematches;
        h->stats.amg_level0_nnz = h->amg->lev[0]->P->nnz;
        h->stats.amg_filter_theta = h->amg->filter_level0 ? h->amg->filter_theta : 0.0;
      }
      M.amg = h->amg.get();
      Mp = &M;
    } else if (h->precond == PFV_PRECOND_AMG_NNS) {
      require(h->nns_k > 0 && h->nns_n == (int64_t)n && (!permuted || h->nns_bs == h->active_bs),
              "the near-null space does not fit the active system (pfv_set_near_null_space again)");
      require(!h->nns_B.empty() || h->active_is_grid, "rigid-body modes of the grid need the assembled mechanics system");
      if (!h->amg_nns) h->amg_nns = std::make_unique<pfv::AmgNns>();
      const unsigned long long cfg = pfv::amg_nns_cfg(h->nns_bs);
      if (!h->amg_nns->valid || h->nns_stale || h->amg_nns_for_val != sys.val || h->amg_nns_key != h->nns_key ||
          h->amg_nns_cfg != cfg) {
        const double* B0 = nns_modes(h, permuted);
        pfv::amg_nns_setup(*h, *h->amg_nns, *sys.P, sys.val, h->nns_bs, h->nns_k, B0, nns_centres(h, permuted));
        h->amg_nns_for_val = sys.val;
        h->amg_nns_key = h->nns_key;
        h->amg_nns_cfg = cfg;
        h->nns_stale = false;
        const pfv::AmgNns& H = *h->amg_nns;
        amg_setup_stats(h, H, (int64_t)H.nlev, H.lev[H.nlev - 1]->n, false);
        h->stats.amg_level0_nnz = sys.P->nnz;
        h->stats.amg_filter_theta = 0.0;
        h->stats.amg_nns_modes = H.k;
      }
      M.nns = h->amg_nns.get();
      Mp = &M;
    } else if (h->precond == PFV_PRECOND_BLOCK) {
      require(h->block_pc && !permuted, "pfv_set_block_preconditioner first (user systems only)");
      require(h->block_pc->ptr.back() == (int64_t)n, "the block layout does not cover the system");
      if (h->block_pc->for_val != sys.val) {
        pfv::blockpc_setup(*h, *h->block_pc, *sys.P, sys.val);
        h->stats.amg_setup_ms = h->block_pc->setup_ms;
      }
      M.blocks = h->block_pc.get();
      M.P = sys.P;
      M.val = sys.val;
      M.diag = sys.diag;
      Mp = &M;
    } else if (h->precond == PFV_PRECOND_SWEEP) {
      pfv::Sweep& sw = *h->sweep;
      pfv::sweep_set_numbering(*h, sw, permuted);
      pfv::sweep_make_plan(sw);
      h->stats.sweep_levels = sw.nlev;
      h->stats.sweep_core_cells = sw.n_core;
      h->stats.sweep_launches = (int64_t)sw.plan.size();
      M.sweep = &sw;
      M.P = sys.P;
      M.val = sys.val;
      M.diag = sys.diag;
      Mp = &M;
    }
    const bool sweep_direct = M.sweep && sweep_transport && M.sweep->n_core == 0;
    const long long launches_before_loop = pfv::launch_counter().load(std::memory_order_relaxed);
    h->stats.amg_setup_launches = (int64_t)(launches_before_loop - launches_before_setup);
    if (sweep_direct) {
      bool fell_back = false;
      res = pfv::sweep_direct_solve(*h, sys, M, rtol, maxit, restart, dxs, fell_back);
      h->stats.sweep_direct_steps = 1;
      h->stats.sweep_direct_fallbacks = fell_back ? 1 : 0;
    } else {
    res = method == PFV_SOLVE_GMRES
              ? pfv::gmres_solve(*h, sys, rtol, maxit, restart, dxs, x0 == nullptr, Mp)
              : pfv::krylov_solve(*h, sys, method, rtol, maxit, dxs, x0 == nullptr, Mp);
    }
    if (M.amg && x0 == nullptr) h->amg->note_iterations(res.iterations, rtol, method, res.converged);
    h->stats.solve_launches = (int64_t)(pfv::launch_counter().load(std::memory_order_relaxed) - launches_before_loop);
    if (permuted) pfv::permute_vector(*h, (int64_t)n, h->active_bs, dxs, dx, false);
    h->stats.solve_ms = tm.stop(s);
    vec_out(h, x, dx, n);
  });
  if (info) {
    info->iterations = res.iterations;
    info->converged = res.converged ? 1 : 0;
    info->rel_residual = res.relres;
    info->solve_ms = h ? h->stats.solve_ms : 0.0;
  }
  if (st == PFV_OK && !res.converged) {
    h->err = "Krylov solver did not reach the requested tolerance";
    return PFV_ERR_NOT_CONVERGED;
  }
  return st;
}


pfv_status pfv_solve_sharded(pfv_ctx* h, int method, double rtol, int maxit, int64_t n_own,
                             const pfv_shard_hooks* hooks, double* d_work, double* d_x_owned,
                             pfv_solve_info* info) {
  pfv::SolveResult res;
  pfv_status st = guarded(h, [&] {
    if (h->precond == PFV_PRECOND_AMG_NNS)
      throw pfv::Error(PFV_ERR_UNSUPPORTED, "PFV_PRECOND_AMG_NNS has no sharded form: pfv_set_preconditioner(PFV_PRECOND_AMG) "
                                            "or PFV_PRECOND_JACOBI for sharded solves");
    if (h->precond == PFV_PRECOND_SWEEP)
      throw pfv::Error(PFV_ERR_UNSUPPORTED, "PFV_PRECOND_SWEEP has no AMG hierarchy and no sharded form");
    require(h->active.valid, "assemble first");
    require(hooks && hooks->exchange_halo && hooks->allreduce_sum, "both hooks are required");
    require(d_work && d_x_owned, "work space and x are required");
    require(method == PFV_SOLVE_CG || method == PFV_SOLVE_BICGSTAB, "a sharded solve runs PFV_SOLVE_CG or PFV_SOLVE_BICGSTAB");
    require(rtol > 0 && maxit > 0, "rtol and maxit must be positive");
    const int64_t n_loc = h->active.n;
    require(n_own > 0 && n_own <= n_loc && n_own % h->active_bs == 0, "n_own out of range");
    auto s = h->stream;
    pfv::Timer tm;
    tm.start(s);
    const pfv::CsrPattern& P = *h->active.P;
    RowsView rows(P, n_own);
    pfv::LinSys sys = h->active;
    sys.P = &rows.V;
    sys.n = n_own;
    sys.win = nullptr;
    if (P.nnz >= pfv::env_int("PFV_SPMV_WINDOW_MIN_NNZ", 20000)) {
      if (h->win_rows_for != P.indices.p || h->win_rows_n != n_own) {
        h->win_rows_checksum = 0;
        pfv::win_build(*h, rows.V, h->win_rows);
        h->win_rows_for = P.indices.p;
        if (h->win_rows.ok && &P == &h->pat_A && h->have_symbolic) h->win_rows_checksum = h->pat_A_checksum;
        h->win_rows_n = n_own;
      }
      if (h->win_rows.ok) sys.win = &h->win_rows;
    }
    pfv::Precond M;
    const pfv::Precond* Mp = nullptr;
    if (h->precond == PFV_PRECOND_AMG) {
      require(h->amg_block && h->amg_block->valid && h->amg_block->lev[0]->n == n_own,
              "pfv_amg_setup(n_own) first: the sharded solve preconditions with the hierarchy of the owned block");
      M.amg = h->amg_block.get();
      Mp = &M;
    } else if (h->precond == PFV_PRECOND_BLOCK) {
      require(h->block_pc != nullptr, "pfv_set_block_preconditioner first");
      require(h->block_pc->ptr.back() == n_own, "the block layout must cover exactly the owned unknowns");
      if (h->block_pc->for_val != sys.val) {
        pfv::blockpc_setup(*h, *h->block_pc, rows.V, sys.val);
        h->stats.amg_setup_ms = h->block_pc->setup_ms;
      }
      M.blocks = h->block_pc.get();
      M.P = &rows.V;
      M.val = sys.val;
      M.diag = sys.diag;
      Mp = &M;
    }
    pfv::be_memset(d_x_owned, 0, sizeof(double) * (size_t)n_own, s);
    pfv::be_memset(d_work, 0, sizeof(double) * (size_t)(2 * n_loc + 8), s);
    h->shard_overlap = false;
#ifndef PFV_EMULATE
    {
      const int ov = pfv::env_int("PFV_SHARD_OVERLAP", 0);
      if (ov != 0 && sys.win && sys.win->ok && h->aux_stream && hooks->exchange_halo == &pfv::rccl_exchange_halo) {
        const pfv::WinCsr& W = *sys.win;
        const int64_t nblk = W.nblk;
        int32_t* lst = h->shard_blocks.ensure(2 * nblk + 2);
        int32_t* cnt = h->status.ensure(16);
        pfv::be_memset(cnt + 12, 0, 2 * sizeof(int32_t), s);
        const int64_t* wptr = W.wptr64;
        const int32_t* wlen = W.wlen;
        const int32_t* wcol = W.wcol.p;
        int32_t* tmp_b = lst + nblk;
        pfv::parallel_for(s, nblk, PFV_LAMBDA(int64_t b) {
          const int64_t w0 = wptr[b];
          const int wn = wlen ? wlen[b] : (int)(wptr[b + 1] - w0);
          const bool bnd = ov == 2 ? (b & 1) != 0 : (wn > 0 && wcol[w0 + wn - 1] >= n_own);
          if (bnd) tmp_b[atomicAdd(cnt + 13, 1)] = (int32_t)b;
          else lst[atomicAdd(cnt + 12, 1)] = (int32_t)b;
        });
        int32_t hc[2];
        be_d2h(hc, cnt + 12, sizeof(hc), s);
        h->shard_n_interior = hc[0];
        h->shard_n_boundary = hc[1];
        pfv::be_d2d(lst + hc[0], tmp_b, sizeof(int32_t) * (size_t)hc[1], s);
        h->shard_overlap = true;
      }
    }
#endif
    h->shard = hooks;
    h->shard_work = d_work;
    h->shard_nloc = n_loc;
    try {
      res = pfv::krylov_solve(*h, sys, method, rtol, maxit, d_x_owned, true, Mp);
    } catch (...) {
      h->shard = nullptr;
      throw;
    }
    h->shard = nullptr;
    if (M.amg) h->amg_block->note_iterations(res.iterations, rtol, method, res.converged);
    h->stats.solve_ms = tm.stop(s);
  });
  if (info) {
    info->iterations = res.iterations;
    info->converged = res.converged ? 1 : 0;
    info->rel_residual = res.relres;
    info->solve_ms = h ? h->stats.solve_ms : 0.0;
  }
  if (st == PFV_OK && !res.converged) {
    h->err = "Krylov solver did not reach the requested tolerance";
    return PFV_ERR_NOT_CONVERGED;
  }
  return st;
}

pfv_status pfv_sweep_info(pfv_ctx* h, int64_t info[4], int32_t* level, int32_t* order) {
  return guarded(h, [&] {
    require(h->sweep && h->sweep->valid, "no flow order on the handle (a solve with PFV_PRECOND_SWEEP builds it)");
    const pfv::Sweep& sw = *h->sweep;
    if (info) {
      info[0] = sw.nc;
      info[1] = sw.nlev;
      info[2] = sw.n_core;
      info[3] = sw.core_level;
    }
    if (level) be_d2h(level, sw.level.p, sizeof(int32_t) * (size_t)sw.nc, h->stream);
    if (order) be_d2h(order, sw.order.p, sizeof(int32_t) * (size_t)sw.nc, h->stream);
  });
}

pfv_status pfv_get_stats(pfv_ctx* h, pfv_stats* out) {
  return guarded(h, [&] {
    require(out != nullptr, "null output");
    *out = h->stats;
  });
}
// ... 113 lines not shown
```

Before: 32.69 million.

## Speculate Galerkin sizes in AMG setup and overlap BiCGSTAB residual read with next preconditioner head

AMG setup reuse now guesses the Galerkin coarse-row capacity and nnz from the previous setup instead of reading them from the device after each pass. All passes run with one deferred readback, and the work is redone if any row exceeds the guessed capacity. In BiCGSTAB, the convergence-check residual read is issued asynchronously through a pinned buffer and an event. The next iteration's p-update and the first AMG smoothing/spmv are enqueued before the host waits, so the GPU keeps working during the host round-trip. This adds complexity, host-wait counters, possible wasted work when a guess misses or the solve converges, and speculative nnz sizing that uses A.nnz as an upper bound.

```diff
diff --git a/include/porefv.h b/include/porefv.h
--- a/include/porefv.h
+++ b/include/porefv.h
@@ -131,6 +131,9 @@
   double transport_adjoint_ms;
   int64_t transport_adjoint_steps;
   int64_t transport_adjoint_core_iterations;
+  int64_t solve_host_waits;
+  int64_t amg_setup_host_waits;
+  int64_t amg_gal_redo;
 } pfv_stats;
 
 pfv_status pfv_create(int device, pfv_ctx** out);
diff --git a/porepy_amd/_lib.py b/porepy_amd/_lib.py
--- a/porepy_amd/_lib.py
+++ b/porepy_amd/_lib.py
@@ -84,7 +84,8 @@
                 ("transport_react_ms", C.c_double), ("transport_react_steps", C.c_int64),
                 ("transport_react_core_iterations", C.c_int64), ("transport_react_components", C.c_int64),
                 ("transport_adjoint_ms", C.c_double), ("transport_adjoint_steps", C.c_int64),
-                ("transport_adjoint_core_iterations", C.c_int64)]
+                ("transport_adjoint_core_iterations", C.c_int64),
+                ("solve_host_waits", C.c_int64), ("amg_setup_host_waits", C.c_int64), ("amg_gal_redo", C.c_int64)]
 
     def as_dict(self):
         return {n: getattr(self, n) for n, _ in self._fields_}
diff --git a/porepy_amd/csrc/amg.inc b/porepy_amd/csrc/amg.inc
--- a/porepy_amd/csrc/amg.inc
+++ b/porepy_amd/csrc/amg.inc
@@ -38,6 +38,7 @@
   bool reuse = true, reuse_dist = true, reuse_rebuilt = true;
   int reuse_dist_min_rows = 500000;
   bool members_reuse = true, sizes_reuse = true;
+  bool gal_spec = true;
   bool filter_smooth = true, rowmax_reuse = true, filter_layout_reuse = true, skip_moved_digest = true;
   bool galerkin_batched = true, filter_unroll = true, dense_lds = true;
   int64_t gather_rows = kAmgGatherRowsDefault;
@@ -79,6 +80,7 @@
   w.reuse_dist_min_rows = env_int("PFV_AMG_REUSE_DIST_MIN_ROWS", 500000);
   w.members_reuse = on("PFV_AMG_MEMBERS_REUSE", 1);
   w.sizes_reuse = on("PFV_AMG_SIZES_REUSE", 1);
+  w.gal_spec = on("PFV_AMG_GAL_SPEC", 1);
   w.filter_smooth = on("PFV_AMG_FILTER_SMOOTH", 1);
   w.rowmax_reuse = on("PFV_AMG_ROWMAX_REUSE", 1);
   w.filter_layout_reuse = on("PFV_AMG_FILTER_LAYOUT_REUSE", 1);
@@ -130,6 +132,7 @@
   Buf<double> tval, dense_work;
   Buf<int32_t> piv;
   Buf<unsigned long long> csum;
+  Buf<int64_t> gal_true;
   CsrPattern P[2];
   Buf<double> V[2], D[2];
 };
@@ -199,6 +202,10 @@
   unsigned long long gal_for_sum = 0;
   bool gal_use = false;
   size_t gal_k = 0;
+  std::vector<GalSizes> gal_pred;
+  size_t gal_pred_k = 0;
+  bool gal_spec = false;
+  int64_t gal_redo = 0;
   unsigned long long filt_win_sum = 0;
   bool maps_ok = false, reused = false;
   int64_t maps_n = -1, maps_nnz = -1, maps_cfg = 0;
@@ -400,9 +407,18 @@
 struct Amg;
 static bool amg_gal_cached(Amg* amg, int64_t ncr, int64_t annz, int* maxcap, int64_t* nnz);
 static void amg_gal_record(Amg* amg, int64_t ncr, int64_t annz, int maxcap, int64_t nnz);
+struct GalSpec {
+  int cap_used = 0;
+  int cap_pred = 0;
+  int32_t* d_maxcap = nullptr;
+  int64_t* d_nnz = nullptr;
+  int32_t* d_flag = nullptr;
+};
+static int amg_gal_spec_capacity(int prev) { return std::min(4096, prev + prev / 4 + 8); }
+
 static void amg_galerkin(pfv_ctx_impl& c, const AmgSwitches& sw, AmgWork& wk, const CsrPattern& A, const double* val,
                          int bs, const int32_t* agg, const int32_t* mptr, const int32_t* mem, int64_t nagg, CsrPattern& Ac,
-                         Buf<double>& valc, Buf<double>& dinvc, Amg* sizes = nullptr) {
+                         Buf<double>& valc, Buf<double>& dinvc, Amg* sizes = nullptr, const GalSpec* spec = nullptr) {
   stream_t s = c.stream;
   const int64_t ncr = nagg * bs;
   const int32_t* ip = A.indptr;
@@ -413,6 +429,7 @@
   int64_t* cptr = wk.cptr.ensure(ncr + 1);
   int32_t* st = c.status.ensure(16);
   be_memset(st + 8, 0, sizeof(int32_t) * 2, s);
+  int32_t* capmax = spec ? spec->d_maxcap : st + 8;
   parallel_for(s, ncr, PFV_LAMBDA(int64_t R) {
     const int64_t I = R / bs;
     const int a = (int)(R - I * bs);
@@ -422,13 +439,15 @@
       m += ip[r + 1] - ip[r];
     }
     cap[R] = m;
-    track_max_i32(st + 8, m);
+    track_max_i32(capmax, m);
   });
   exclusive_scan<int32_t, int64_t>(s, c.scratch, cap, tptr, (size_t)ncr);
   int maxcap_c = 0;
   int64_t nnz_c = 0;
-  const bool known = amg_gal_cached(sizes, ncr, A.nnz, &maxcap_c, &nnz_c);
-  const int maxcap = known ? maxcap_c : read_scalar<int32_t>(s, st + 8);
+  const bool known = !spec && amg_gal_cached(sizes, ncr, A.nnz, &maxcap_c, &nnz_c);
+  const int maxcap = spec ? spec->cap_used : (known ? maxcap_c : read_scalar<int32_t>(s, st + 8));
+  const int cap_limit = spec ? spec->cap_used : 0x7fffffff;
+  int32_t* flag = spec ? spec->d_flag : nullptr;
   const int64_t ttot = A.nnz;
   if (maxcap > 4096) throw Error(PFV_ERR_UNSUPPORTED, "AMG: more than 4096 entries feed one coarse row");
   int32_t* tcol = wk.tcol.ensure(std::max<int64_t>(ttot, 1));
@@ -436,14 +455,22 @@
   double* dinv = dinvc.ensure(std::max<int64_t>(ncr, 1));
   be_memset(dinv, 0, sizeof(double) * (size_t)ncr, s);
   const int capL = std::max(maxcap, 1);
-  const int G = capL <= 64 ? 16 : (capL <= 160 ? 32 : 64);
+  const int capG = spec ? std::max(spec->cap_pred, 1) : capL;
+  const int G = capG <= 64 ? 16 : (capG <= 160 ? 32 : 64);
   int capP = 2;
   while (capP < capL) capP <<= 1;
   const int nw = capP / 64 + 1;
   const size_t lds = 8 * (size_t)capP + 8 * (size_t)capL + 8 * (size_t)nw + 4 * (2 * kGalMaxMembers + 1) + 64;
-  const bool batched = capL <= kGalEpl * G && sw.galerkin_batched;
+  const bool batched = capG <= kGalEpl * G && sw.galerkin_batched;
   wave_for_g(G, s, ncr, lds, PFV_LAMBDA(const WaveCtx& w) {
     const int64_t R = w.item;
+    if (cap[R] > cap_limit) {
+      if (w.lane0()) {
+        atomic_max_i32(flag, 1);
+        cnt[R] = 0;
+      }
+      return;
+    }
     const int64_t I = R / bs;
     const int a = (int)(R - I * bs);
     unsigned long long* key = reinterpret_cast<unsigned long long*>(w.lds);
@@ -556,15 +583,24 @@
     w.sync();
   });
   exclusive_scan<int32_t, int64_t>(s, c.scratch, cnt, cptr, (size_t)ncr);
-  const int64_t nnz = known ? nnz_c : read_scalar<int64_t>(s, cptr + ncr);
-  if (!known) amg_gal_record(sizes, ncr, A.nnz, maxcap, nnz);
+  int64_t nnz;
+  int64_t* true_nnz = spec ? spec->d_nnz : nullptr;
+  if (spec) {
+    nnz = A.nnz;
+  } else {
+    nnz = known ? nnz_c : read_scalar<int64_t>(s, cptr + ncr);
+    if (!known) amg_gal_record(sizes, ncr, A.nnz, maxcap, nnz);
+  }
   if (nnz >= (int64_t(1) << 31)) throw Error(PFV_ERR_UNSUPPORTED, "AMG: coarse matrix with more than 2^31 entries");
   Ac.nrows = Ac.ncols = ncr;
   Ac.nnz = nnz;
   int32_t* cp = Ac.indptr.ensure(ncr + 1);
   int32_t* cx = Ac.indices.ensure(std::max<int64_t>(nnz, 1));
   double* cv = valc.ensure(std::max<int64_t>(nnz, 1));
-  parallel_for(s, ncr + 1, PFV_LAMBDA(int64_t R) { cp[R] = (int32_t)cptr[R]; });
+  parallel_for(s, ncr + 1, PFV_LAMBDA(int64_t R) {
+    cp[R] = (int32_t)cptr[R];
+    if (true_nnz && R == ncr) true_nnz[0] = cptr[ncr];
+  });
   wave_for<16>(s, ncr, 16, PFV_LAMBDA(const WaveCtx& w) {
     const int64_t R = w.item;
     const int64_t t0 = tptr[R], o = cptr[R];
@@ -912,8 +948,9 @@
 static void amg_estimate_omegas(pfv_ctx_impl& c, Amg& amg);
 static void amg_spmv(pfv_ctx_impl& c, const Amg& amg, const AmgLevel& L, const double* x, double* y,
                      const double* smooth_b);
+enum AmgCyclePart { kCycleWhole = 0, kCycleHead, kCycleRest };
 static double* amg_cycle(pfv_ctx_impl& c, Amg& amg, size_t l, const double* b, double* x, bool x_is_presmoothed = false,
-                         int visit = 0);
+                         int visit = 0, AmgCyclePart part = kCycleWhole);
 static void amg_setup(pfv_ctx_impl& c, Amg& amg, const CsrPattern& A, const double* val, int bs,
                       const double* diag = nullptr, const WinCsr* win0 = nullptr);
 static void amg_restrict(pfv_ctx_impl& c, const Amg& amg, const AmgLevel& L, const AmgLevel& Ln, const double* b,
@@ -1151,6 +1188,23 @@
   if (!reuse) L.pmap_count = 0;
   if (!reuse) L.members_kept = false;
   const bool members_reuse = reuse && L.members_kept && w.members_reuse;
+  const CsrPattern* const P0 = curP;
+  const double* const V0 = curV;
+  const size_t pred0 = amg.gal_pred_k;
+  bool spec = reuse && !D && amg.gal_spec && L.pmap_count > 0 && L.pmap_count <= 8;
+  for (int pass = 0; spec && pass < L.pmap_count; ++pass) {
+    if (pred0 + pass >= amg.gal_pred.size() || amg.gal_pred[pred0 + pass].ncr != L.pmap_n[pass] * bs) spec = amg.gal_spec = false;
+    if (L.pmap_n[pass] * bs <= w.coarse_target) break;
+  }
+  int64_t* gal_true = spec ? wk.gal_true.ensure(17) : nullptr;
+  int npass = 0;
+again:
+  curP = P0;
+  curV = V0;
+  cur_cells = cells;
+  slot = -1;
+  npass = 0;
+  if (spec) be_memset(gal_true, 0, sizeof(int64_t) * 17, s);
   for (int pass = 0; pass < (reuse ? L.pmap_count : passes_here); ++pass) {
     int64_t nagg;
     if (reuse) {
@@ -1166,8 +1220,17 @@
     if (!members_reuse) amg_members(c, wk, a1p, cur_cells, nagg, L.pmp[pass], L.pme[pass]);
     const int nslot = slot < 0 ? 0 : 1 - slot;
     const int32_t* amap = D ? amg_dist_extend_map(c, *D, l, a1p, cur_cells, nagg) : a1p;
+    GalSpec gs;
+    if (spec) {
+      gs.cap_pred = amg.gal_pred[pred0 + pass].maxcap;
+      gs.cap_used = amg_gal_spec_capacity(gs.cap_pred);
+      gs.d_nnz = gal_true + pass;
+      gs.d_maxcap = reinterpret_cast<int32_t*>(gal_true + 8 + pass);
+      gs.d_flag = reinterpret_cast<int32_t*>(gal_true + 16);
+    }
     amg_galerkin(c, w, wk, *curP, curV, bs, amap, L.pmp[pass], L.pme[pass], nagg, wk.P[nslot], wk.V[nslot], wk.D[nslot],
-                 D ? nullptr : &amg);
+                 D ? nullptr : &amg, spec ? &gs : nullptr);
+    ++npass;
     if (D) wk.P[nslot].ncols = (nagg + D->plan[l]->n_halo) * bs;
     if (members_reuse) {
     } else if (slot < 0) {
@@ -1180,6 +1243,26 @@
     curV = wk.V[slot].p;
     cur_cells = nagg;
     if (nagg * bs <= w.coarse_target) break;
+  }
+  if (spec) {
+    int64_t got[17];
+    be_d2h(got, gal_true, sizeof(got), s);
+    if (got[16] != 0) {
+      ++amg.gal_redo;
+      spec = false;
+      goto again;
+    }
+    int64_t annz = P0->nnz;
+    for (int pass = 0; pass < npass; ++pass) {
+      if (got[pass] >= (int64_t(1) << 31)) throw Error(PFV_ERR_UNSUPPORTED, "AMG: coarse matrix with more than 2^31 entries");
+      amg_gal_record(&amg, L.pmap_n[pass] * bs, annz, (int)got[8 + pass], got[pass]);
+      annz = got[pass];
+    }
+    wk.P[slot].nnz = got[npass - 1];
+    wk.P[slot].max_row = (int)got[8 + npass - 1];
+    amg.gal_pred_k = pred0 + (size_t)npass;
+  } else if (amg.gal_spec) {
+    amg.gal_pred_k = pred0 + (size_t)npass;
   }
   if (D && slot < 0) {
     amg_dist_identity_level(c, amg, *D, l, *curP, curV, aggL, cells);
@@ -1268,6 +1351,11 @@
   unsigned long long level0_sum = amg_setup_level0(c, amg, A, val, diag, win0, csum);
   amg.gal_use = reuse && !D && level0_sum != 0 && amg.gal_for_sum == level0_sum && w.sizes_reuse;
   amg.gal_k = 0;
+  amg.gal_spec = reuse && !D && !amg.gal_use && w.gal_spec && !amg.gal_sizes.empty();
+  amg.gal_pred.clear();
+  if (amg.gal_spec) amg.gal_pred.swap(amg.gal_sizes);
+  amg.gal_pred_k = 0;
+  amg.gal_redo = 0;
   if (!amg.gal_use) amg.gal_sizes.clear();
   double nnz_sum = 0.0;
   size_t l = 0;
@@ -1631,9 +1719,13 @@
   }
 }
 
+static bool amg_cycle_has_head(const Amg& amg) { return amg.nlev > 1 && !amg_level_path(amg, 0).small; }
+
 static double* amg_cycle(pfv_ctx_impl& c, Amg& amg, size_t l, const double* b, double* x, bool x_is_presmoothed,
-                         int visit) {
+                         int visit, AmgCyclePart part) {
   stream_t s = c.stream;
+  const bool head_done = part == kCycleRest && l == 0 && amg_cycle_has_head(amg);
+  if (part == kCycleHead && !(l == 0 && amg_cycle_has_head(amg))) return x;
   AmgLevel& L = *amg.lev[l];
   const int64_t n = L.n;
   const double omega = L.omega, alpha = amg.alpha;
@@ -1659,13 +1751,14 @@
   const bool twice = path.twice;
   const bool fuse_up = path.fuse_up;
   const bool fuse_big = path.fuse_big;
-  if (!x_is_presmoothed) parallel_for(s, n, PFV_LAMBDA(int64_t i) { x[i] = omega * dinv[i] * b[i]; });
+  if (!x_is_presmoothed && !head_done) parallel_for(s, n, PFV_LAMBDA(int64_t i) { x[i] = omega * dinv[i] * b[i]; });
   const bool next_smooths = l + 2 < amg.nlev;
   if (small) {
     if (L.v32) amg_restrict_residual<float>(c, amg, L, Ln, L.v32, b, x, next_smooths);
     else amg_restrict_residual<double>(c, amg, L, Ln, L.val, b, x, next_smooths);
   } else {
-    amg_spmv(c, amg, L, x, t, nullptr);
+    if (!head_done) amg_spmv(c, amg, L, x, t, nullptr);
+    if (part == kCycleHead) return x;
     amg_restrict(c, amg, L, Ln, b, t, next_smooths);
   }
   double* xc = amg_cycle(c, amg, l + 1, Ln.b, Ln.x, next_smooths, 0);
@@ -1857,5 +1950,16 @@
     parallel_for(c.stream, n, PFV_LAMBDA(int64_t i) { out[i] = in[i] / d[i]; });
   }
 }
-
-}
+static bool precond_has_head(const Precond& M) {
+  return !M.sweep && !M.blocks && !M.nns && M.amg && !M.amg->dist && amg_cycle_has_head(*M.amg);
+}
+static void precond_begin(pfv_ctx_impl& c, const Precond& M, int64_t n, const double* in, double* out) {
+  (void)n;
+  if (precond_has_head(M)) amg_cycle(c, *M.amg, 0, in, out, false, 0, kCycleHead);
+}
+static void precond_finish(pfv_ctx_impl& c, const Precond& M, int64_t n, const double* in, double* out) {
+  if (precond_has_head(M)) amg_cycle(c, *M.amg, 0, in, out, false, 0, kCycleRest);
+  else precond_apply(c, M, n, in, out);
+}
+
+}
diff --git a/porepy_amd/csrc/backend.h b/porepy_amd/csrc/backend.h
--- a/porepy_amd/csrc/backend.h
+++ b/porepy_amd/csrc/backend.h
@@ -47,6 +47,12 @@
   return c;
 }
 
+inline std::atomic<long long>& host_wait_counter() {
+  static std::atomic<long long> c{0};
+  return c;
+}
+inline void note_host_wait() { host_wait_counter().fetch_add(1, std::memory_order_relaxed); }
+
 #ifndef PFV_EMULATE
 #define PFV_HIP_CHECK(expr)                                                              \
   do {                                                                                   \
@@ -148,6 +154,7 @@
   return e ? std::atoi(e) : dflt;
 }
 inline void wait_stream(stream_t s) {
+  note_host_wait();
   if (!spin_wait_enabled()) {
     PFV_HIP_CHECK(hipStreamSynchronize(s));
     return;
@@ -168,6 +175,7 @@
   if (!bytes) return;
 #ifdef PFV_EMULATE
   (void)s;
+  note_host_wait();
   std::memcpy(dst, src, bytes);
 #else
   PFV_HIP_CHECK(hipMemcpyAsync(dst, src, bytes, hipMemcpyHostToDevice, s));
@@ -178,6 +186,7 @@
   if (!bytes) return;
 #ifdef PFV_EMULATE
   (void)s;
+  note_host_wait();
   std::memcpy(dst, src, bytes);
 #else
   if (bytes <= 4096 && spin_wait_enabled()) {
@@ -243,6 +252,7 @@
 inline void be_sync(stream_t s) {
 #ifdef PFV_EMULATE
   (void)s;
+  note_host_wait();
 #else
   wait_stream(s);
 #endif
@@ -686,6 +696,57 @@
   return v;
 }
 
+struct SmallRead {
+  static constexpr size_t kBytes = 64;
+#ifdef PFV_EMULATE
+  alignas(8) char slot[kBytes] = {};
+#else
+  void* slot = nullptr;
+  hipEvent_t ev = nullptr;
+#endif
+  SmallRead() = default;
+  SmallRead(const SmallRead&) = delete;
+  SmallRead& operator=(const SmallRead&) = delete;
+  ~SmallRead() {
+#ifndef PFV_EMULATE
+    if (ev) (void)hipEventDestroy(ev);
+    if (slot) (void)hipHostFree(slot);
+#endif
+  }
+  void begin(const void* src, size_t bytes, stream_t s) {
+    if (bytes > kBytes) throw Error(1, "SmallRead: more than 64 bytes");
+#ifdef PFV_EMULATE
+    (void)s;
+    std::memcpy(slot, src, bytes);
+#else
+    if (!slot) PFV_HIP_CHECK(hipHostMalloc(&slot, kBytes, hipHostMallocDefault));
+    if (!ev) PFV_HIP_CHECK(hipEventCreateWithFlags(&ev, hipEventDisableTiming));
+    PFV_HIP_CHECK(hipMemcpyAsync(slot, src, bytes, hipMemcpyDeviceToHost, s));
+    PFV_HIP_CHECK(hipEventRecord(ev, s));
+#endif
+  }
+  void wait() {
+    note_host_wait();
+#ifndef PFV_EMULATE
+    if (!spin_wait_enabled()) {
+      PFV_HIP_CHECK(hipEventSynchronize(ev));
+      return;
+    }
+    for (;;) {
+      const hipError_t e = hipEventQuery(ev);
+      if (e == hipSuccess) return;
+      if (e != hipErrorNotReady) PFV_HIP_CHECK(e);
+    }
+#endif
+  }
+  template <class T>
+  T get() const {
+    T v;
+    std::memcpy(&v, slot, sizeof(T));
+    return v;
+  }
+};
+
 template <class T>
 PFV_FN int lower_bound_idx(const T* a, int n, T key) {
   int lo = 0, hi = n;
diff --git a/porepy_amd/csrc/ctx.h b/porepy_amd/csrc/ctx.h
--- a/porepy_amd/csrc/ctx.h
+++ b/porepy_amd/csrc/ctx.h
@@ -154,6 +154,7 @@
   Buf<double> rhs, diag, xsol, face_tmp, vec_in;
   Buf<double> kry[10];
   Buf<double> red;
+  SmallRead kry_read;
   Buf<double> gmres_basis, gmres_small;
 
   bool have_mpsa_params = false, have_mpsa_numeric = false, have_mpsa_symbolic = false, have_mech_system = false;
diff --git a/porepy_amd/csrc/linalg.inc b/porepy_amd/csrc/linalg.inc
--- a/porepy_amd/csrc/linalg.inc
+++ b/porepy_amd/csrc/linalg.inc
@@ -764,6 +764,20 @@
   double relres = 0.0;
 };
 
+static void bicg_head(pfv_ctx_impl& c, const Precond* M, int64_t n, const double* diag, const double* S, const double* r,
+                      const double* v, double* p, double* y) {
+  if (M) {
+    parallel_for(c.stream, n, PFV_LAMBDA(int64_t i) { p[i] = r[i] + S[S_BETA] * (p[i] - S[S_OMEGA] * v[i]); });
+    precond_begin(c, *M, n, p, y);
+  } else {
+    parallel_for(c.stream, n, PFV_LAMBDA(int64_t i) {
+      const double pi = r[i] + S[S_BETA] * (p[i] - S[S_OMEGA] * v[i]);
+      p[i] = pi;
+      y[i] = pi / diag[i];
+    });
+  }
+}
+
 static SolveResult krylov_solve(pfv_ctx_impl& c, const LinSys& sys, int method, double rtol, int maxit,
                                 double* d_x, bool x_is_zero, const Precond* M = nullptr) {
   stream_t s = c.stream;
@@ -863,22 +877,18 @@
   constexpr int kTrueResidualRestarts = 3;
   int restarts = 0;
   int it = 1;
+  const bool early_read = !sharded && env_int("PFV_KRYLOV_EARLY_READ", 1) != 0;
+  bool head_enqueued = false;
 restart_bicgstab:
+  head_enqueued = false;
   be_d2d(rhat, r, sizeof(double) * n, s);
   be_memset(p, 0, sizeof(double) * n, s);
   be_memset(v, 0, sizeof(double) * n, s);
   dot2(c, n, r, r, rhat, r, R, M_START);
   for (; it <= maxit; ++it) {
-    if (M) {
-      parallel_for(s, n, PFV_LAMBDA(int64_t i) { p[i] = r[i] + S[S_BETA] * (p[i] - S[S_OMEGA] * v[i]); });
-      precond_apply(c, *M, n, p, y);
-    } else {
-      parallel_for(s, n, PFV_LAMBDA(int64_t i) {
-        const double pi = r[i] + S[S_BETA] * (p[i] - S[S_OMEGA] * v[i]);
-        p[i] = pi;
-        y[i] = pi / diag[i];
-      });
-    }
+    if (!head_enqueued) bicg_head(c, M, n, diag, S, r, v, p, y);
+    if (M) precond_finish(c, *M, n, p, y);
+    head_enqueued = false;
     shard_spmv(c, P, Aval, y, v, rhat, 1, R, M_ALPHA, sys.win);
     if (M) {
       parallel_for(s, n, PFV_LAMBDA(int64_t i) { r[i] -= S[S_ALPHA] * v[i]; });
@@ -922,10 +932,27 @@
     }
     res.iterations = it;
     if (it % check_every == 0 || it == maxit) {
-      const double rr = read_scalar<double>(s, S + S_RR);
+      double rr;
+      long long head_launches = 0;
+      if (early_read && it < maxit) {
+        c.kry_read.begin(S + S_RR, sizeof(double), s);
+        const long long before = launch_counter().load(std::memory_order_relaxed);
+        bicg_head(c, M, n, diag, S, r, v, p, y);
+        head_launches = launch_counter().load(std::memory_order_relaxed) - before;
+        head_enqueued = true;
+        c.kry_read.wait();
+        rr = c.kry_read.get<double>();
+      } else {
+        rr = read_scalar<double>(s, S + S_RR);
+      }
       res.relres = std::sqrt(rr / bb);
-      if (rr <= tol2) { res.converged = true; break; }
-      if (!(rr == rr)) break;
+      const bool stop = rr <= tol2 || !(rr == rr);
+      if (stop) {
+        if (head_enqueued) launch_counter().fetch_sub(head_launches, std::memory_order_relaxed);
+        head_enqueued = false;
+        if (rr <= tol2) res.converged = true;
+        break;
+      }
     }
   }
   if (res.converged && !sharded && env_int("PFV_TRUE_RESIDUAL", 1) != 0) {
diff --git a/porepy_amd/csrc/porefv.hip b/porepy_amd/csrc/porefv.hip
--- a/porepy_amd/csrc/porefv.hip
+++ b/porepy_amd/csrc/porefv.hip
@@ -3115,6 +3115,7 @@
     pfv::Precond M;
     const pfv::Precond* Mp = nullptr;
     const long long launches_before_setup = pfv::launch_counter().load(std::memory_order_relaxed);
+    const long long waits_before_setup = pfv::host_wait_counter().load(std::memory_order_relaxed);
     if (h->precond == PFV_PRECOND_AMG) {
       if (!h->amg) h->amg = std::make_unique<pfv::Amg>();
       if (!h->amg->valid || h->amg_for_val != sys.val) {
@@ -3123,6 +3124,7 @@
         h->amg_last = 1;
         amg_setup_stats(h, *h->amg, (int64_t)h->amg->nlev, h->amg->lev[h->amg->nlev - 1]->n, h->amg->reused);
         h->stats.amg_stale_rematches = h->amg->stale_rematches;
+        h->stats.amg_gal_redo = h->amg->gal_redo;
         h->stats.amg_level0_nnz = h->amg->lev[0]->P->nnz;
         h->stats.amg_filter_theta = h->amg->filter_level0 ? h->amg->filter_theta : 0.0;
       }
@@ -3178,6 +3180,8 @@
     const bool sweep_direct = M.sweep && sweep_transport && M.sweep->n_core == 0;
     const long long launches_before_loop = pfv::launch_counter().load(std::memory_order_relaxed);
     h->stats.amg_setup_launches = (int64_t)(launches_before_loop - launches_before_setup);
+    const long long waits_before_loop = pfv::host_wait_counter().load(std::memory_order_relaxed);
+    h->stats.amg_setup_host_waits = (int64_t)(waits_before_loop - waits_before_setup);
     if (sweep_direct) {
       bool fell_back = false;
       res = pfv::sweep_direct_solve(*h, sys, M, rtol, maxit, restart, dxs, fell_back);
@@ -3190,6 +3194,7 @@
     }
     if (M.amg && x0 == nullptr) h->amg->note_iterations(res.iterations, rtol, method, res.converged);
     h->stats.solve_launches = (int64_t)(pfv::launch_counter().load(std::memory_order_relaxed) - launches_before_loop);
+    h->stats.solve_host_waits = (int64_t)(pfv::host_wait_counter().load(std::memory_order_relaxed) - waits_before_loop);
     if (permuted) pfv::permute_vector(*h, (int64_t)n, h->active_bs, dxs, dx, false);
     h->stats.solve_ms = tm.stop(s);
     vec_out(h, x, dx, n);
```

New measurement: 32.86 million, median of 6. About the same (+0.5%).
